# zhuye98/ICL

Hardware: AMD Instinct MI355X
Metric: 3D volumes/sec/node (fwd+bwd, 96^3 patch) (higher is better)
Workload: dtype f32; 1 GPU; 3D U-Net ICL BraTS-shape synthetic 96x96x96, num_classes=2, batch=2 per GPU (1 labeled + 1 unlabeled), full ICL step incl. SGD; global_batch=2, parallelism=dp1, launch=hipGraph replay

## Files before the change

icl_amd/_lib.py:

```python
from __future__ import annotations

import ctypes
import os
from ctypes import c_char_p, c_double, c_float, c_int, c_int64, c_void_p

import torch

_HERE = os.path.dirname(os.path.abspath(__file__))
DEFAULT_LIB = os.path.join(_HERE, "libicl_hip.so")

_lib = None
_lib_path = None
_host_pointers_ok = False

P, I, L, F = c_void_p, c_int, c_int64, c_float
D = c_double

_SIGNATURES = {
    "icl_abi_version": (c_int, []),
    "icl_last_error": (c_char_p, []),
    "icl_last_kernel_name": (c_char_p, []),
    "icl_conv3d_packed_elems": (c_int64, [I, I, I, I]),
    "icl_conv3d_pack_weights": (c_int, [P, P, I, I, I, I, P]),
    "icl_conv3d_pack_weights_both": (c_int, [P, P, P, I, I, I, P]),
    "icl_conv3d_pack_weights_multi": (c_int, [P, P, P, P, P, P, I, P]),
    "icl_conv3d_fwd_ws_bytes": (c_int64, [I, I, I, I, I, I, I]),
    "icl_conv3d_fwd": (c_int, [P, P, P, P, P, I, I, I, I, I, I, I, L, L, P]),
    "icl_scalar_combine": (c_int, [P, P, I, I, P, P]),
    "icl_conv3d_split_ws_bytes": (c_int64, [I, I]),
    "icl_conv3d_split_weights_multi": (c_int, [P, P, P, P, I, P]),
    "icl_conv3d_fwd_presplit": (c_int, [P, P, P, P, I, I, I, I, I, I, L, L, P]),
    "icl_conv3d_fwd_presplit_ws_bytes": (c_int64, [I, I, I, I, I, I]),
    "icl_conv3d_fwd_presplit_ws": (c_int, [P, P, P, P, P, I, I, I, I, I, I, L, L, P]),
    "icl_conv3d_fwd_stats_slots": (c_int, [I, I, I, I, I, I]),
    "icl_conv3d_fwd_presplit_stats": (c_int, [P, P, P, P, P, I, I, I, I, I, I, L, L, P]),
    "icl_norm_fwd_given_stats": (c_int, [P, P, P, P, P, P, P, P, P, I, I, L, I, I, F, F, P, I, P]),
    "icl_conv3d_wgrad_ws_bytes": (c_int64, [I, I, I, I]),
    "icl_conv3d_wgrad": (c_int, [P, P, P, P, P, I, I, I, I, I, I, I, L, L, P]),
    "icl_conv3d_wgrad_slabs": (c_int, [P, P, P, I, I, I, I, I, I, I, L, L, P, P]),
    "icl_conv3d_wgrad_reduce_multi": (c_int, [P, P, P, P, P, P, I, P]),
    "icl_norm_ws_bytes": (c_int64, [I, I, L]),
    "icl_norm_fwd": (c_int, [P, P, P, P, P, P, P, P, I, I, L, I, I, I, F, F, P, P]),
    "icl_norm_bwd": (c_int, [P, P, P, P, P, P, P, P, P, I, I, L, I, I, I, P, P]),
    "icl_norm_res_fwd": (c_int, [P, P, P, P, P, P, P, P, P, I, I, L, I, I, I, F, F, P, P]),
    "icl_norm_res_bwd": (c_int, [P, P, P, P, P, P, P, P, P, P, P, I, I, L, I, I, I, P, P]),
    "icl_rstd_from_var": (c_int, [P, P, I, F, P]),
    "icl_norm_finalize_stats": (c_int, [P, I, I, I, F, P, P, P, P]),
    "icl_norm_apply": (c_int, [P, P, P, I, I, L, P]),
    "icl_maxpool2_fwd_norm": (c_int, [P, P, P, P, L, I, I, I, I, P]),
    "icl_upsample2x_concat_norm": (c_int, [P, P, P, P, P, I, I, I, I, I, I, P]),
    "icl_conv1x1_dropout_norm": (c_int, [P, P, P, P, P, I, I, I, L, I, I, ctypes.c_uint32, F, P, P]),
    "icl_conv1x1_wgrad_dropout_norm": (c_int, [P, P, P, P, P, P, I, I, I, L, L, ctypes.c_uint32, F, P, P]),
    "icl_maxpool2_fwd": (c_int, [P, P, P, L, I, I, I, I, P]),
    "icl_maxpool2_bwd": (c_int, [P, P, P, L, I, I, I, I, P]),
    "icl_maxpool2_bwd_add": (c_int, [P, P, P, P, I, I, I, I, I, I, L, P]),
    "icl_trilinear_fwd": (c_int, [P, P, I, I, I, I, I, I, I, I, L, I, P]),
    "icl_trilinear_bwd_ws_bytes": (c_int64, [I, I, I, I, I, I, I, I]),
    "icl_trilinear_bwd": (c_int, [P, P, P, I, I, I, I, I, I, I, I, L, I, P]),
    "icl_copy_rows": (c_int, [P, P, L, L, L, L, P]),
    "icl_concat2": (c_int, [P, L, P, L, P, P]),
    "icl_dwconv3_fwd": (c_int, [P, P, P, I, I, I, I, I, I, P]),
    "icl_dwconv3_wgrad_ws_bytes": (c_int64, [I, I, I, I, I]),
    "icl_dwconv3_wgrad": (c_int, [P, P, P, P, I, I, I, I, I, P]),
    "icl_conv1x1_small": (c_int, [P, P, P, P, I, I, I, L, I, I, P]),
    "icl_conv1x1_dropout": (c_int, [P, P, P, P, I, I, I, L, I, I, I, ctypes.c_uint32, F, P, P]),
    "icl_conv1x1_wgrad_dropout": (c_int, [P, P, P, P, P, I, I, I, L, L, ctypes.c_uint32, F, P, P]),
    "icl_dropout": (c_int, [P, P, L, ctypes.c_uint32, F, P, P]),
    "icl_drop_path": (c_int, [P, P, L, L, ctypes.c_uint32, F, P, P]),
    "icl_drop_path_add": (c_int, [P, P, P, L, L, ctypes.c_uint32, F, P, P]),
    "icl_loss_fwd": (c_int, [P, P, P, P, P, P, I, I, L, I, I, P]),
    "icl_window_attn_bias_elems": (c_int64, [I, I]),
    "icl_depth_to_space2": (c_int, [P, P, I, I, I, I, I, L, P]),
    "icl_space_to_depth2": (c_int, [P, P, I, I, I, I, I, L, P]),
    "icl_colsum_multi": (c_int, [P, P, P, P, I, P]),
    "icl_gather_rows": (c_int, [P, P, P, L, L, L, I, P]),
    "icl_gather_rows_sum2": (c_int, [P, P, P, L, L, L, I, P]),
    "icl_im2col3": (c_int, [P, P, I, I, I, I, I, P]),
    "icl_im2col3_planes": (c_int, [P, P, I, I, I, I, I, P]),
    "icl_conv3d_cin1_fwd": (c_int, [P, P, P, P, I, I, I, I, I, L, L, P]),
    "icl_conv3d_cin1_wgrad_ws_bytes": (c_int64, [I, I, I]),
    "icl_conv3d_cin1_wgrad": (c_int, [P, P, P, P, I, I, I, I, I, L, L, P]),
    "icl_col2im3": (c_int, [P, P, I, I, I, I, I, P]),
    "icl_linear_ws_bytes": (c_int64, [L, I, I, I]),
    "icl_linear_fwd": (c_int, [P, P, P, P, P, L, I, I, I, P]),
    "icl_linear_dgrad": (c_int, [P, P, P, P, L, I, I, P]),
    "icl_linear_bwd_small": (c_int, [P, P, P, P, P, P, L, I, I, P]),
    "icl_linear_wgrad_small": (c_int, [P, P, P, P, L, I, I, P]),
    "icl_linear_dgrad_sgd": (c_int, [P, P, P, P, P, P, L, I, I, F, F, F, I, P, P]),
    "icl_gemm_ws_bytes": (c_int64, [L, I, I, I]),
    "icl_gemm": (c_int, [P, P, P, P, P, L, I, I, L, L, L, I, I, I, I, L, L, L, P]),
    "icl_linear_wgrad_ws_bytes": (c_int64, [L, I, I]),
    "icl_linear_wgrad": (c_int, [P, P, P, P, P, L, I, I, P]),
    "icl_conv1x1_wgrad_ws_bytes": (c_int64, [I, L, I, I]),
    "icl_conv1x1_wgrad": (c_int, [P, P, P, P, P, I, I, I, L, L, L, P]),
    "icl_relpos_bias_fwd": (c_int, [P, P, P, I, I, I, P]),
    "icl_window_attn_fwd": (c_int, [P, P, P, P, P, I, I, I, I, I, F, P]),
    "icl_window_attn_bwd": (c_int, [P, P, P, P, P, P, P, P, I, I, I, I, I, F, P]),
    "icl_window_attn_bwd_chunks": (c_int, [I, I, I, I, I]),
    "icl_window_attn_fwd_drop": (c_int, [P, P, P, P, P, I, I, I, I, I, F, ctypes.c_uint32, F, P, P]),
    "icl_window_attn_keep_probe": (c_int, [P, c_int64, I, ctypes.c_uint32, F, P, P]),
    "icl_window_attn_bwd_drop": (c_int, [P, P, P, P, P, P, P, P, I, I, I, I, I, F, ctypes.c_uint32, F, P, P]),
    "icl_relpos_bias_bwd_sum": (c_int, [P, I, P, P, P, L, I, I, P]),
    "icl_layernorm_fwd": (c_int, [P, P, P, P, P, P, L, I, F, P]),
    "icl_layernorm_bwd_ws_bytes": (c_int64, [L, I]),
    "icl_layernorm_bwd": (c_int, [P, P, P, P, P, P, P, P, P, L, I, P]),
    "icl_gelu_fwd": (c_int, [P, P, L, P]),
    "icl_gelu_bwd": (c_int, [P, P, P, L, P]),
    "icl_attn_fwd": (c_int, [P, P, P, P, P, I, I, I, I, I, F, P]),
    "icl_attn_bwd": (c_int, [P, P, P, P, P, P, P, P, P, I, I, I, I, I, F, P]),
    "icl_attn_bwd_ws_bytes": (c_int64, [I, I, I, I, I]),
    "icl_attn_bwd_ws": (c_int, [P, P, P, P, P, P, P, P, P, P, I, I, I, I, I, F, P]),
    "icl_crop_rotflip": (c_int, [P, P, P, I, P, P, I, I, I, P]),
    "icl_volume_feed": (c_int, [P, P, P, P, I, P, P, I, I, I, P]),
    "icl_rank_tile": (c_int, []),
    "icl_rank_index_build": (c_int, [P, P, I, I, I, F, P, P, P]),
    "icl_rank_select": (c_int, [P, P, P, P, P, F, I, P, P]),
    "icl_volume_feed_origins": (c_int, [P, P, P, P, I, P, P, P, I, I, I, P]),
    "icl_prefix_box": (c_int, [P, I, I, I, P, I, P, P, P]),
    "icl_prefix_resample": (c_int, [P, P, P, P, P, I, P, P, P]),
    "icl_prefix_restore": (c_int, [P, I, P, P, P, P]),
    "icl_slice_augment": (c_int, [P, P, P, P, I, P, P, I, I, P]),
    "icl_slice_resize": (c_int, [P, P, L, I, I, I, I, I, P]),
    "icl_sgd_step": (c_int, [P, P, P, L, F, F, F, I, P, P]),
    "icl_sgd_step_factored": (c_int, [P, P, P, P, I, I, I, F, F, F, I, P, P]),
    "icl_sgd_step_factored_narrow": (c_int, [P, P, P, P, I, I, I, F, F, F, I, P, I, P]),
    "icl_sgd_factored_split_ws_bytes": (c_int64, [I, I, I]),
    "icl_sgd_step_factored_split": (c_int, [P, P, P, P, P, I, I, I, F, F, F, I, P, P]),
    "icl_sgd_step_multi": (c_int, [P, P, P, P, I, F, F, F, I, P, P]),
    "icl_loss_bwd": (c_int, [P, P, P, P, P, P, P, P, I, I, L, I, I, P]),
    "icl_loss_fwd_multi": (c_int, [P, I, P]),
    "icl_loss_bwd_multi": (c_int, [P, I, P]),
    "icl_qchain_stage": (c_int, [P, P]),
    "icl_qchain_wgrad": (c_int, [P, P, P, P, P, P, P, P, I, P]),
    "icl_seg_metrics_ws_bytes": (c_int64, [I, I, I, I]),
    "icl_seg_metrics": (c_int, [P, I, P, I, I, I, I, I, I, P, P, P]),
    "icl_seg_surface_ws_bytes": (c_int64, [I, I, I, I]),
    "icl_seg_surface_metrics": (c_int, [P, I, P, I, I, I, I, I, D, D, D, D, P, P, P, P]),
    "icl_seg_components_ws_bytes": (c_int64, [I, I, I, I]),
    "icl_seg_components": (c_int, [P, I, I, I, I, I, I, P, P, P, P]),
    "icl_seg_filter_components": (c_int, [P, I, I, I, I, I, I, I, c_int64, P, P, P, P]),
    "icl_window_gather": (c_int, [P, P, P, I, I, I, I, I, I, I, I, I, I, I, I, I, I, P]),
    "icl_window_accumulate": (c_int, [P, P, P, P, P, I, I, I, I, I, I, I, I, I, P]),
    "icl_window_finalize": (c_int, [P, P, P, P, I, I, I, I, I, I, I, I, I, I, P]),
    "icl_window_gather_flipped": (c_int, [P, P, P, P, I, I, I, I, I, I, I, I, I, I, I, I, I, I, P]),
    "icl_window_accumulate_flipped": (c_int, [P, P, P, P, P, P, I, I, I, I, I, I, I, I, I, P]),
    "icl_last_live_fwd_kernel_name": (c_char_p, []),
    "icl_last_wgrad_grid": (None, [P, P]),
    "icl_conv3d_fwd_live_ok": (c_int, [I, I, I, I, I, I, I]),
    "icl_conv3d_fwd_presplit_live": (c_int, [P, P, P, P, I, I, I, I, I, I, I, L, L, P]),
    "icl_conv3d_fwd_presplit_ws_live": (c_int, [P, P, P, P, P, I, I, I, I, I, I, I, L, L, P]),
    "icl_conv3d_fwd_live": (c_int, [P, P, P, P, P, I, I, I, I, I, I, I, I, L, L, P]),
    "icl_conv3d_wgrad_ws_bytes_live": (c_int64, [I, I, I, I, I]),
    "icl_conv3d_wgrad_live": (c_int, [P, P, P, P, P, I, I, I, I, I, I, I, I, L, L, P]),
    "icl_conv3d_wgrad_slabs_live": (c_int, [P, P, P, I, I, I, I, I, I, I, I, L, L, P, P]),
    "icl_norm_bwd_live": (c_int, [P, P, P, P, P, P, P, P, P, I, I, I, L, I, I, I, P, P]),
    "icl_maxpool2_bwd_add_live": (c_int, [P, P, P, P, I, I, I, I, I, I, I, L, P]),
    "icl_trilinear_bwd_live": (c_int, [P, P, P, I, I, I, I, I, I, I, I, I, L, I, P]),
    "icl_conv1x1_small_live": (c_int, [P, P, P, P, I, I, I, I, L, I, I, P]),
    "icl_conv1x1_dropout_live": (c_int, [P, P, P, P, I, I, I, I, L, I, I, I, ctypes.c_uint32, F, P, P]),
    "icl_conv1x1_wgrad_live": (c_int, [P, P, P, P, P, I, I, I, I, L, L, L, P]),
    "icl_conv1x1_wgrad_dropout_live": (c_int, [P, P, P, P, P, I, I, I, I, L, L, ctypes.c_uint32, F, P, P]),
    "icl_conv1x1_wgrad_dropout_norm_live": (c_int, [P, P, P, P, P, P, I, I, I, I, L, L, ctypes.c_uint32, F, P, P]),
}

EXPORTS = tuple(_SIGNATURES)


def _load(path: str):
    if not os.path.exists(path):
        raise RuntimeError(
            f"icl_amd: HIP library {path} not found — build it with `python -m icl_amd.build` "
            "(hipcc --offload-arch=gfx950). There is no CPU fallback.")
    lib = ctypes.CDLL(path)
    for name, (res, args) in _SIGNATURES.items():
        fn = getattr(lib, name)
        fn.restype = res
        fn.argtypes = args
    return lib


def lib():
    global _lib, _lib_path
    if _lib is None:
        _lib_path = os.environ.get("ICL_HIP_LIB", DEFAULT_LIB)
        _lib = _load(_lib_path)
    return _lib


def lib_path():
    lib()
    return _lib_path


def host_pointers_ok() -> bool:
    return _host_pointers_ok


def _use_library_for_tests(path: str | None, host_pointers: bool = True):
    global _lib, _lib_path, _host_pointers_ok
    if path is None:
        _lib, _lib_path, _host_pointers_ok = None, None, False
        return
    _lib, _lib_path, _host_pointers_ok = _load(path), path, host_pointers


def check(rc: int, what: str = ""):
    if rc != 0:
        msg = lib().icl_last_error()
        raise RuntimeError(f"icl_hip {what} failed ({rc}): {msg.decode() if msg else ''}")
```

icl_amd/csrc/icl_abi.inc:

```

#include "kernels/common.h"
#include "kernels/norm.h"
#include "kernels/pool_resize.h"
#include "kernels/reduce.h"
#include "kernels/conv_mfma.h"
#include "kernels/conv_mfma_static.h"
#include "kernels/conv_mfma_flat.h"
#include "kernels/conv_bf16x3.h"
#include "kernels/conv_bf16x3_ws.h"
#include "kernels/conv_wgrad_tr.h"
#include "kernels/conv_wgrad_zs.h"
#include "kernels/conv_cin1.h"
#include "kernels/misc.h"
#include "kernels/loss.h"
#include "kernels/optim.h"
#include "kernels/winattn.h"
#include "kernels/linear_wgrad.h"
#include "kernels/token.h"
#include "kernels/gemm.h"
#include "kernels/datafeed.h"
#include "kernels/rankindex.h"
#include "kernels/prefix.h"
#include "kernels/qchain.h"
#include "kernels/metrics.h"
// ... 1181 lines not shown
  hipStream_t st = (hipStream_t)stream;
  const int R = n * c;
  const int nch = (int)((s + icl::kNormChunk - 1) / icl::kNormChunk);
  float* part = (float*)ws;
  if (mode == 0 && nch == 1) {
    part = nullptr;
  } else {
    ICL_LAUNCH(icl::norm_act_bwd_partial_kernel, dim3(nch, R), dim3(icl::kNormThreads), 0, st, gy, x, mean, rstd, gamma, beta, part,
               (long)s, c, nch, mode, act, res);
    if (int rc = check_launch("norm_bwd_partial")) return rc;
  }
  const float inv_count = 1.0f / (float)((mode ? (int64_t)n : 1) * s);
  ICL_LAUNCH(icl::norm_act_bwd_apply_kernel, dim3(nch, R), dim3(icl::kNormThreads), 0, st, gy, x, mean, rstd, gamma, beta,
             (const float*)part, gx, (long)s, c, mode, act, inv_count, use_batch_stats, res, gres, R, nch, dgamma, dbeta);
  return check_launch("norm_bwd_apply");
}

int icl_rstd_from_var(const float* var, float* rstd, int c, float eps, void* stream) {
  if (!var || !rstd || c < 1) return fail(-1, "rstd_from_var: bad argument");
  ICL_LAUNCH(icl::rstd_from_var_kernel, dim3((c + 63) / 64), dim3(64), 0, (hipStream_t)stream, var, rstd, c, eps);
  return check_launch("rstd_from_var");
}

namespace {
int maxpool2_fwd_run(const float* x, const float* ss, float* y, uint8_t* idx, int64_t nc, int dout, int hout, int wout, int pool_depth,
                     hipStream_t st, const char* what) {
  const long total = nc * dout * hout * wout;
  const char* e_x2 = getenv("ICL_MAXPOOL_BWD_X2");
  if ((wout & 1) == 0 && aligned16(x) && ((uintptr_t)y & 7) == 0 && (e_x2 ? atoi(e_x2) : 1)) {
    ICL_LAUNCH(icl::maxpool2_fwd_x2_kernel, dim3(grid_for(total / 2, 256)), dim3(256), 0, st, x, y, idx, (long)nc, dout, hout, wout, pool_depth, ss);
  } else {
    ICL_LAUNCH(icl::maxpool2_fwd_kernel, dim3(grid_for(total, 256)), dim3(256), 0, st, x, y, idx, (long)nc, dout, hout, wout, pool_depth, ss);
  }
  return check_launch(what);
}
}

int icl_maxpool2_fwd(const float* x, float* y, uint8_t* idx, int64_t nc, int dout, int hout, int wout, int pool_depth, void* stream) {
  if (!x || !y || !idx || nc < 1 || dout < 1 || hout < 1 || wout < 1 || (pool_depth != 1 && pool_depth != 2)) return fail(-1, "maxpool2_fwd: bad argument");
  return maxpool2_fwd_run(x, nullptr, y, idx, nc, dout, hout, wout, pool_depth, (hipStream_t)stream, "maxpool2_fwd");
}

int icl_norm_finalize_stats(const float* part, int n, int c, int nslots, float eps, float* mean, float* rstd, float* ss, void* stream) {
  if (!part || !mean || !rstd || !ss || n < 1 || c < 1 || nslots < 1) return fail(-1, "norm_finalize_stats: bad argument");
  ICL_LAUNCH(icl::norm_finalize_stats_kernel, dim3(n * c), dim3(64), 0, (hipStream_t)stream, part, n * c, c, nslots, eps, mean, rstd, ss);
  return check_launch("norm_finalize_stats");
}

int icl_norm_apply(const float* x, const float* ss, float* y, int n, int c, int64_t s, void* stream) {
  if (!x || !ss || !y || n < 1 || c < 1 || s < 4 || (s & 3) || !aligned16(x) || !aligned16(y)) return fail(-1, "norm_apply: bad argument (s %% 4 == 0)");
  ICL_LAUNCH(icl::copy_rows_norm_kernel, dim3(grid_for((long)n * c * (s >> 2), 256, 1 << 16)), dim3(256), 0, (hipStream_t)stream, x, y, n, c, (long)s,
             (long)c * s, ss);
  return check_launch("norm_apply");
}

int icl_maxpool2_fwd_norm(const float* x, const float* ss, float* y, uint8_t* idx, int64_t nc, int dout, int hout, int wout, int pool_depth,
                          void* stream) {
  if (!x || !ss || !y || !idx || nc < 1 || dout < 1 || hout < 1 || wout < 1 || (pool_depth != 1 && pool_depth != 2))
    return fail(-1, "maxpool2_fwd_norm: bad argument");
  return maxpool2_fwd_run(x, ss, y, idx, nc, dout, hout, wout, pool_depth, (hipStream_t)stream, "maxpool2_fwd_norm");
}

int icl_upsample2x_concat_norm(const float* skip, const float* skip_ss, const float* deep, const float* deep_ss, float* out, int n, int cs,
                               int cd, int d, int h, int w, void* stream) {
  if (!skip || !deep || !out || n < 1 || cs < 1 || cd < 1 || d < 2 || h < 2 || w < 4 || (d & 1) || (h & 1) || (w & 3))
    return fail(-1, "upsample2x_concat_norm: bad argument (even depth / height, width a multiple of 4)");
  if (!aligned16(skip) || !aligned16(deep) || !aligned16(out)) return fail(-1, "upsample2x_concat_norm: 16-byte alignment");
  hipStream_t st = (hipStream_t)stream;
  const long s = (long)d * h * w, obs = (long)(cs + cd) * s;
  if (skip_ss) {
    ICL_LAUNCH(icl::copy_rows_norm_kernel, dim3(grid_for((long)n * cs * (s >> 2), 256, 1 << 16)), dim3(256), 0, st, skip, out, n, cs, s, obs, skip_ss);
  } else {
    ICL_LAUNCH(icl::copy_rows_kernel, dim3(grid_for((long)n * cs * s, 256)), dim3(256), 0, st, skip, out, (long)n, (long)cs * s, (long)cs * s, obs);
  }
  if (int rc = check_launch("upsample2x_concat_norm: skip")) return rc;
  const long total = (long)n * cd * s;
  const int di = d / 2, hi = h / 2, wi = w / 2;
  if (wi % 4 == 0)
    ICL_LAUNCH(icl::upsample2x_fwd_x4_kernel, dim3(grid_for(total / 32, 256, 1 << 16)), dim3(256), 0, st, deep, out + (long)cs * s, n, cd, di, hi, wi, obs,
               deep_ss);
  else
    ICL_LAUNCH(icl::upsample2x_fwd_kernel, dim3(grid_for(total / 16, 256, 1 << 16)), dim3(256), 0, st, deep, out + (long)cs * s, n, cd, di, hi, wi, obs,
               deep_ss);
  return check_launch("upsample2x_concat_norm: deep");
}

int icl_maxpool2_bwd(const float* gy, const uint8_t* idx, float* gx, int64_t nc, int dout, int hout, int wout, int pool_depth, void* stream) {
  if (!gy || !gx || !idx || nc < 1 || dout < 1 || hout < 1 || wout < 1 || (pool_depth != 1 && pool_depth != 2)) return fail(-1, "maxpool2_bwd: bad argument");
  const long total = nc * dout * hout * wout;
  ICL_LAUNCH(icl::maxpool2_bwd_kernel, dim3(grid_for(total, 256)), dim3(256), 0, (hipStream_t)stream, gy, idx, gx, (long)nc, dout, hout, wout,
             pool_depth);
  return check_launch("maxpool2_bwd");
}

int icl_maxpool2_bwd_add(const float* gy, const uint8_t* idx, const float* add, float* gx, int n, int c, int dout, int hout, int wout,
                         int pool_depth, int64_t add_bstride, void* stream) {
  return icl_maxpool2_bwd_add_live(gy, idx, add, gx, n, n, c, dout, hout, wout, pool_depth, add_bstride, stream);
}

int icl_maxpool2_bwd_add_live(const float* gy, const uint8_t* idx, const float* add, float* gx, int n, int skip_live, int c, int dout, int hout,
                              int wout, int pool_depth, int64_t add_bstride, void* stream) {
  if (!gy || !gx || !idx || !add || n < 1 || c < 1 || dout < 1 || hout < 1 || wout < 1 || (pool_depth != 1 && pool_depth != 2) || (add_bstride & 1) ||
      ((uintptr_t)add & 7) || skip_live < 1 || skip_live > n)
    return fail(-1, "maxpool2_bwd_add: bad argument");
  const long ncskip = (long)skip_live * c;
  const long total = (long)n * c * dout * hout * wout;
  const char* e_x2 = getenv("ICL_MAXPOOL_BWD_X2");
  if ((wout & 1) == 0 && aligned16(add) && aligned16(gx) && ((uintptr_t)gy & 7) == 0 && (add_bstride & 3) == 0 && (e_x2 ? atoi(e_x2) : 1)) {
    ICL_LAUNCH(icl::maxpool2_bwd_add_x2_kernel, dim3(grid_for(total / 2, 256)), dim3(256), 0, (hipStream_t)stream, gy, idx, add, gx, (long)n * c, c,
               dout, hout, wout, pool_depth, (long)add_bstride, ncskip);
    return check_launch("maxpool2_bwd_add_x2");
  }
  ICL_LAUNCH(icl::maxpool2_bwd_add_kernel, dim3(grid_for(total, 256)), dim3(256), 0, (hipStream_t)stream, gy, idx, add, gx, (long)n * c, c, dout,
             hout, wout, pool_depth, (long)add_bstride, ncskip);
  return check_launch("maxpool2_bwd_add");
}

namespace {
inline float resize_scale(int in, int out, int align) {
  if (align) return out > 1 ? (float)(in - 1) / (float)(out - 1) : 0.f;
  return (float)in / (float)out;
}
}

int icl_trilinear_fwd(const float* x, float* y, int n, int c, int di, int hi, int wi, int dout, int hout, int wout,
                      int64_t y_bstride, int align_corners, void* stream) {
  if (!x || !y || n < 1 || c < 1 || di < 1 || hi < 1 || wi < 1 || dout < 1 || hout < 1 || wout < 1) return fail(-1, "trilinear_fwd: bad argument");
  const long total = (long)n * c * dout * hout * wout;
  const float rz = resize_scale(di, dout, align_corners), ry = resize_scale(hi, hout, align_corners), rx = resize_scale(wi, wout, align_corners);
  if (!align_corners && dout == 2 * di && hout == 2 * hi && wout == 2 * wi && wi % 2 == 0 && y_bstride % 4 == 0 && aligned16(y) &&
      total / 16 < (1L << 31)) {
    constexpr int x4 = 1;
    if (x4 && wi % 4 == 0 && aligned16(x))
      ICL_LAUNCH(icl::upsample2x_fwd_x4_kernel, dim3(grid_for(total / 32, 256, 1 << 16)), dim3(256), 0, (hipStream_t)stream, x, y, n, c, di, hi,
                 wi, (long)y_bstride, (const float*)nullptr);
    else
      ICL_LAUNCH(icl::upsample2x_fwd_kernel, dim3(grid_for(total / 16, 256, 1 << 16)), dim3(256), 0, (hipStream_t)stream, x, y, n, c, di, hi, wi,
                 (long)y_bstride, (const float*)nullptr);
  } else if (wout % 4 == 0 && y_bstride % 4 == 0 && aligned16(y) && total / 4 < (1L << 31)) {
    ICL_LAUNCH(icl::trilinear_fwd_quad_kernel, dim3(grid_for(total / 4, 256, 1 << 16)), dim3(256), 0, (hipStream_t)stream, x, y, n, c, di, hi,
               wi, dout, hout, wout, rz, ry, rx, (long)y_bstride, align_corners);
  } else {
    ICL_LAUNCH(icl::trilinear_fwd_kernel, dim3(grid_for(total, 256)), dim3(256), 0, (hipStream_t)stream, x, y, n, c, di, hi, wi, dout, hout,
               wout, rz, ry, rx, (long)y_bstride, align_corners);
  }
  return check_launch("trilinear_fwd");
}

int64_t icl_trilinear_bwd_ws_bytes(int n, int c, int di, int hi, int wi, int dout, int hout, int wout) {
  (void)di;
  return ((int64_t)n * c * dout * hout * wi + (int64_t)n * c * dout * hi * wi) * 4;
}

int icl_trilinear_bwd(const float* gy, float* gx, void* ws, int n, int c, int di, int hi, int wi, int dout, int hout, int wout,
                      int64_t gy_bstride, int align_corners, void* stream) {
  if (!gy || !gx || !ws || n < 1 || c < 1 || di < 1 || hi < 1 || wi < 1 || dout < 1 || hout < 1 || wout < 1) return fail(-1, "trilinear_bwd: bad argument");
  hipStream_t st = (hipStream_t)stream;
  const int al = align_corners;
  const float rz = resize_scale(di, dout, al), ry = resize_scale(hi, hout, al), rx = resize_scale(wi, wout, al);
  float* t1 = (float*)ws;
  float* t2 = t1 + (size_t)n * c * dout * hout * wi;
  int rc;
  if (!al && dout == 2 * di && hout == 2 * hi && wout == 2 * wi && wi % 4 == 0 && gy_bstride % 4 == 0 && aligned16(gy) && aligned16(gx) &&
      (long)n * c * di * hi * wi / 4 < (1L << 31)) {
    ICL_LAUNCH(icl::upsample2x_bwd_kernel, dim3(grid_for((long)n * c * ((di + icl::kUpSeg - 1) / icl::kUpSeg) * hi * wi / 4, 256, 1 << 16)),
               dim3(256), 0, st, gy, gx, n, c, di, hi,
               wi, (long)gy_bstride);
    return check_launch("upsample2x_bwd");
  }
  auto axis = [&](const float* src, float* dst, long rows, int li, int lo, long inner, float rs, long sbs, const char* what) -> int {
    const long total = (long)n * rows * li * inner;
    const bool small = total / 4 < (1L << 31) && rows < (1L << 31);
    if (small && inner % 4 == 0 && sbs % 4 == 0 && aligned16(src) && aligned16(dst)) {
      ICL_LAUNCH(icl::resize_bwd_axis_t4_kernel, dim3(grid_for(total / 4, 256, 1 << 16)), dim3(256), 0, st, src, dst, n, (unsigned)rows, li, lo,
                 (unsigned)(inner / 4), rs, sbs, al);
    } else if (inner == 1 && lo >= 4 * li && lo % 4 == 0 && lo <= 1024 && sbs % 4 == 0 && aligned16(src) && rows * li >= 4096) {
      const long nrows = (long)n * rows;
      ICL_LAUNCH(icl::resize_bwd_axis_x_lds_kernel, dim3((unsigned)cdivl(nrows, icl::kRbxRows)), dim3(256),
                 (size_t)icl::kRbxRows * (lo + 4) * 4, st, src, dst, n, rows, li, lo, rs, sbs, al);
    } else if (small && inner == 1 && li % 4 == 0 && aligned16(dst)) {
      ICL_LAUNCH(icl::resize_bwd_axis_i4_kernel, dim3(grid_for(total / 4, 256, 1 << 16)), dim3(256), 0, st, src, dst, n, (unsigned)rows, li, lo,
                 rs, sbs, al);
    } else {
      ICL_LAUNCH(icl::resize_bwd_axis_kernel, dim3(grid_for(total, 256)), dim3(256), 0, st, src, dst, n, rows, li, lo, inner, rs, sbs, al);
    }
    return check_launch(what);
  };
  if ((rc = axis(gy, t1, (long)c * dout * hout, wi, wout, 1L, rx, (long)gy_bstride, "resize_bwd_x"))) return rc;
  if ((rc = axis(t1, t2, (long)c * dout, hi, hout, (long)wi, ry, (long)c * dout * hout * wi, "resize_bwd_y"))) return rc;
  if ((rc = axis(t2, gx, (long)c, di, dout, (long)hi * wi, rz, (long)c * dout * hi * wi, "resize_bwd_z"))) return rc;
  return 0;
}

int icl_copy_rows(const float* src, float* dst, int64_t rows, int64_t row_elems, int64_t src_stride, int64_t dst_stride,
                  void* stream) {
  if (!src || !dst || rows < 1 || row_elems < 1) return fail(-1, "copy_rows: bad argument");
  ICL_LAUNCH(icl::copy_rows_kernel, dim3(grid_for(rows * row_elems, 256)), dim3(256), 0, (hipStream_t)stream, src, dst, (long)rows,
             (long)row_elems, (long)src_stride, (long)dst_stride);
  return check_launch("copy_rows");
}

int icl_concat2(const float* a, int64_t na, const float* b, int64_t nb, float* out, void* stream) {
  if (!out || na < 0 || nb < 0 || na + nb < 4 || (na & 3) || (nb & 3) || (!a && !b)) return fail(-1, "concat2: bad argument (float counts are multiples of 4)");
  if ((a && !aligned16(a)) || (b && !aligned16(b)) || !aligned16(out)) return fail(-1, "concat2: 16-byte alignment");
  ICL_LAUNCH(icl::concat2_kernel, dim3(grid_for((na + nb) >> 2, 256)), dim3(256), 0, (hipStream_t)stream, a, (long)na, b, (long)nb, out);
  return check_launch("concat2");
}

int icl_depth_to_space2(const float* yt, float* out, int n, int d, int h, int w, int cout, int64_t out_bstride, void* stream) {
  if (!yt || !out || n < 1 || d < 1 || h < 1 || w < 1 || cout < 1) return fail(-1, "depth_to_space2: bad argument");
  const size_t lds = (size_t)w * (cout * 8 + 2) * 4;
  if (lds > (size_t)kMaxDynLdsBig) return fail(-1, "depth_to_space2: token row does not fit LDS (w * cout too large)");
  if (lds > (size_t)kMaxDynLds) ICL_SET_MAX_DYN_LDS(icl::depth_to_space2_kernel, kMaxDynLdsBig);
  ICL_LAUNCH(icl::depth_to_space2_kernel, dim3(h, d, n), dim3(256), lds, (hipStream_t)stream, yt, out, d, h, w, cout, (long)out_bstride);
  return check_launch("depth_to_space2");
}

int icl_space_to_depth2(const float* g, float* gt, int n, int d, int h, int w, int cout, int64_t g_bstride, void* stream) {
  if (!g || !gt || n < 1 || d < 1 || h < 1 || w < 1 || cout < 1) return fail(-1, "space_to_depth2: bad argument");
  const size_t lds = (size_t)w * (cout * 8 + 2) * 4;
  if (lds > (size_t)kMaxDynLdsBig) return fail(-1, "space_to_depth2: token row does not fit LDS (w * cout too large)");
  if (lds > (size_t)kMaxDynLds) ICL_SET_MAX_DYN_LDS(icl::space_to_depth2_kernel, kMaxDynLdsBig);
  ICL_LAUNCH(icl::space_to_depth2_kernel, dim3(h, d, n), dim3(256), lds, (hipStream_t)stream, g, gt, d, h, w, cout, (long)g_bstride);
  return check_launch("space_to_depth2");
}

int icl_dwconv3_fwd(const float* x, const float* w, float* y, int n, int c, int d, int h, int wd, int flip, void* stream) {
  if (!x || !w || !y || n < 1 || c < 1 || d < 1 || h < 1 || wd < 1) return fail(-1, "dwconv3_fwd: bad argument");
  const long total = (long)n * c * d * h * wd;
  ICL_LAUNCH(icl::dwconv3_fwd_kernel, dim3(grid_for(total, 256)), dim3(256), 0, (hipStream_t)stream, x, w, y, (long)n * c, c, d, h, wd, flip);
  return check_launch("dwconv3_fwd");
}

static long dwconv3_wgrad_chunks(long total) {
  long chunks = cdivl(total, 1024);
  return chunks > 512 ? 512 : chunks;
}

int64_t icl_dwconv3_wgrad_ws_bytes(int n, int c, int d, int h, int wd) {
  return dwconv3_wgrad_chunks((long)n * d * h * wd) * c * 27 * 4;
}

int icl_dwconv3_wgrad(const float* x, const float* gy, float* gw, void* ws, int n, int c, int d, int h, int wd, void* stream) {
  if (!x || !gy || !gw || !ws || n < 1 || c < 1 || d < 1 || h < 1 || wd < 1) return fail(-1, "dwconv3_wgrad: bad argument");
  hipStream_t s = (hipStream_t)stream;
  const long total = (long)n * d * h * wd;
  const long chunks = dwconv3_wgrad_chunks(total);
  const long chunk = cdivl(total, chunks);
  ICL_LAUNCH(icl::dwconv3_wgrad_kernel, dim3((unsigned)chunks, c), dim3(256), 0, s, x, gy, (float*)ws, n, c, d, h, wd, chunk);
  if (int rc = check_launch("dwconv3_wgrad")) return rc;
  ICL_LAUNCH(icl::dwconv3_wgrad_reduce_kernel, dim3((unsigned)cdivl((long)c * 27, 16)), dim3(256), 0, s, (const float*)ws, gw, c * 27, (int)chunks);
  return check_launch("dwconv3_wgrad_reduce");
}

namespace {
icl::DropSpec drop_spec(int mode, uint32_t seed, float p, const uint32_t* seed_dev) {
  icl::DropSpec d{};
  d.mode = mode;
  d.seed = (unsigned)seed;
  d.thresh = (unsigned)((double)p * 4294967296.0);
  d.scale = 1.0f / (1.0f - p);
  d.seed_dev = (const unsigned*)seed_dev;
  return d;
}

int conv1x1_small_run(const float* x, const float* w, const float* bias, float* y, int n, int cin, int cout, int64_t s, int w_ostride,
                      int w_istride, const icl::DropSpec& dr, hipStream_t st, int n_plan = 0) {
  if ((long)(n_plan > n ? n_plan : n) * s >= 65536) {
    const long quads = (long)n * (s >> 2);
    const int ob = cout <= 1 ? 1 : cout <= 2 ? 2 : cout <= 4 ? 4 : cout <= 8 ? 8 : 16;
    const dim3 grid(grid_for(quads, 256, 1 << 16), (cout + ob - 1) / ob);
    switch (ob) {
      case 1: ICL_LAUNCH(icl::conv1x1_stream_kernel<1>, grid, dim3(256), 0, st, x, w, bias, y, n, cin, cout, (long)s, w_ostride, w_istride, dr); break;
      case 2: ICL_LAUNCH(icl::conv1x1_stream_kernel<2>, grid, dim3(256), 0, st, x, w, bias, y, n, cin, cout, (long)s, w_ostride, w_istride, dr); break;
      case 4: ICL_LAUNCH(icl::conv1x1_stream_kernel<4>, grid, dim3(256), 0, st, x, w, bias, y, n, cin, cout, (long)s, w_ostride, w_istride, dr); break;
      case 8: ICL_LAUNCH(icl::conv1x1_stream_kernel<8>, grid, dim3(256), 0, st, x, w, bias, y, n, cin, cout, (long)s, w_ostride, w_istride, dr); break;
      default: ICL_LAUNCH(icl::conv1x1_stream_kernel<16>, grid, dim3(256), 0, st, x, w, bias, y, n, cin, cout, (long)s, w_ostride, w_istride, dr); break;
    }
    return check_launch("conv1x1_stream");
  }
  if (dr.mode) return 1;
  const long total = (long)n * cout * (s >> 2);
  ICL_LAUNCH(icl::conv1x1_small_kernel, dim3(grid_for(total, 256)), dim3(256), 0, st, x, w, bias, y, n, cin, cout, (long)s,
             w_ostride, w_istride);
  return check_launch("conv1x1_small");
}
}

int icl_conv1x1_small(const float* x, const float* w, const float* bias, float* y, int n, int cin, int cout, int64_t s, int w_ostride,
                      int w_istride, void* stream) {
  if (!x || !w || !y || n < 1 || cin < 1 || cout < 1 || s < 4 || (s & 3)) return fail(-1, "conv1x1_small: bad argument (s %% 4 == 0)");
  return conv1x1_small_run(x, w, bias, y, n, cin, cout, s, w_ostride, w_istride, icl::DropSpec{}, (hipStream_t)stream);
}

int icl_conv1x1_dropout(const float* x, const float* w, const float* bias, float* y, int n, int cin, int cout, int64_t s, int w_ostride,
                        int w_istride, int mask_mode, uint32_t seed, float p, const uint32_t* seed_dev, void* stream) {
  if (!x || !w || !y || n < 1 || cin < 1 || cout < 1 || s < 4 || (s & 3) || (mask_mode != 1 && mask_mode != 2) || !(p >= 0.f && p < 1.f))
    return fail(-1, "conv1x1_dropout: bad argument");
  return conv1x1_small_run(x, w, bias, y, n, cin, cout, s, w_ostride, w_istride, drop_spec(mask_mode, seed, p, seed_dev), (hipStream_t)stream);
}

int icl_conv1x1_dropout_norm(const float* x, const float* ss, const float* w, const float* bias, float* y, int n, int cin, int cout, int64_t s,
                             int w_ostride, int w_istride, uint32_t seed, float p, const uint32_t* seed_dev, void* stream) {
  if (!x || !ss || !w || !y || n < 1 || cin < 1 || cout < 1 || s < 4 || (s & 3) || !(p >= 0.f && p < 1.f) || (long)n * s < 65536)
    return fail(-1, "conv1x1_dropout_norm: bad argument (big volumes only: n * s >= 65536)");
  icl::DropSpec dr = p > 0.f ? drop_spec(1, seed, p, seed_dev) : icl::DropSpec{};
  dr.ss = ss;
  return conv1x1_small_run(x, w, bias, y, n, cin, cout, s, w_ostride, w_istride, dr, (hipStream_t)stream);
}

int icl_scalar_combine(const void* const* in, const float* w, int n_in, int n_out, float* out, void* stream) {
  if (!in || !w || !out || n_in < 1 || n_out < 1 || n_in > icl::kScalarCombine || n_out > icl::kScalarCombine)
    return fail(-1, "scalar_combine: bad argument (<= %d scalars in and out)", icl::kScalarCombine);
  icl::ScalarCombine s{};
  s.n_in = n_in; s.n_out = n_out;
  for (int i = 0; i < n_in; ++i) {
    if (!in[i]) return fail(-1, "scalar_combine: null input %d", i);
    s.in[i] = (const float*)in[i];
  }
  for (int j = 0; j < n_out; ++j)
    for (int i = 0; i < n_in; ++i) s.w[j][i] = w[j * n_in + i];
  ICL_LAUNCH(icl::scalar_combine_kernel, dim3(1), dim3(64), 0, (hipStream_t)stream, s, out);
  return check_launch("scalar_combine");
}

int icl_colsum_multi(const void* const* g, void* const* out, const int32_t* rows, const int32_t* cols, int count, void* stream) {
  if (!g || !out || !rows || !cols || count < 1) return fail(-1, "colsum_multi: bad argument");
  for (int base = 0; base < count; base += icl::kColsumMulti) {
    icl::ColsumMulti m{};
    const int k = count - base < icl::kColsumMulti ? count - base : icl::kColsumMulti;
    int cmax = 1;
    for (int i = 0; i < k; ++i) {
      const int j = base + i;
      if (!g[j] || !out[j] || rows[j] < 1 || cols[j] < 1) return fail(-1, "colsum_multi: bad tensor %d", j);
      m.g[i] = (const float*)g[j]; m.out[i] = (float*)out[j]; m.rows[i] = rows[j]; m.cols[i] = cols[j];
      if (cols[j] > cmax) cmax = cols[j];
    }
    ICL_LAUNCH(icl::colsum_multi_kernel, dim3(grid_for(cmax, 16, 128), k), dim3(256), 0, (hipStream_t)stream, m);
    const int rc = check_launch("colsum_multi");
    if (rc) return rc;
  }
  return 0;
}

int icl_gather_rows(const float* src, const int32_t* idx, float* out, int64_t b, int64_t s, int64_t m, int c, void* stream) {
  if (!src || !idx || !out || b < 1 || s < 1 || m < 1 || c < 4 || (c & 3)) return fail(-1, "gather_rows: bad argument (c %% 4 == 0)");
  ICL_LAUNCH(icl::gather_rows_kernel, dim3(grid_for(b * m * (c / 4), 256)), dim3(256), 0, (hipStream_t)stream, src, (const int*)idx, out,
             (long)b, (long)s, (long)m, c / 4);
  return check_launch("gather_rows");
}

int icl_gather_rows_sum2(const float* src, const int32_t* idx2, float* out, int64_t b, int64_t s, int64_t m, int c, void* stream) {
  if (!src || !idx2 || !out || b < 1 || s < 1 || m < 1 || c < 4 || (c & 3)) return fail(-1, "gather_rows_sum2: bad argument (c %% 4 == 0)");
  ICL_LAUNCH(icl::gather_rows_sum2_kernel, dim3(grid_for(b * m * (c / 4), 256)), dim3(256), 0, (hipStream_t)stream, src, (const int*)idx2, out,
             (long)b, (long)s, (long)m, c / 4);
  return check_launch("gather_rows_sum2");
}

int icl_im2col3(const float* x, float* cols, int n, int c, int d, int h, int w, void* stream) {
  if (!x || !cols || n < 1 || c < 1 || d < 1 || h < 1 || w < 1) return fail(-1, "im2col3: bad argument");
  ICL_LAUNCH(icl::im2col3_kernel, dim3(grid_for((long)n * c * 27 * d * h * w, 256)), dim3(256), 0, (hipStream_t)stream, x, cols, n, c, d, h, w);
  return check_launch("im2col3");
}

int icl_im2col3_planes(const float* x, float* planes, int n, int c, int d, int h, int w, void* stream) {
  if (!x || !planes || n < 1 || c < 1 || d < 1 || h < 1 || w < 4 || (w & 3)) return fail(-1, "im2col3_planes: bad argument (w %% 4 == 0)");
  ICL_LAUNCH(icl::im2col3_planes_kernel, dim3(grid_for((long)n * c * 27 * d * h * (w / 4), 256, 1 << 16)), dim3(256), 0, (hipStream_t)stream, x,
             planes, n, c, d, h, w);
  return check_launch("im2col3_planes");
}

int icl_col2im3(const float* g, float* dx, int n, int c, int d, int h, int w, void* stream) {
  if (!g || !dx || n < 1 || c < 1 || d < 1 || h < 1 || w < 1) return fail(-1, "col2im3: bad argument");
  ICL_LAUNCH(icl::col2im3_kernel, dim3(grid_for((long)n * c * d * h * w, 256)), dim3(256), 0, (hipStream_t)stream, g, dx, n, c, d, h, w);
  return check_launch("col2im3");
}

int icl_drop_path_add(const float* x, const float* res, float* y, int64_t n, int64_t group, uint32_t seed, float p,
                      const uint32_t* seed_dev, void* stream) {
  if (!x || !y || n < 1 || group < 1 || !(p >= 0.f && p < 1.f)) return fail(-1, "dropout: bad argument");
  const unsigned thresh = (unsigned)((double)p * 4294967296.0);
  ICL_LAUNCH(icl::dropout_kernel, dim3(grid_for(n, 256)), dim3(256), 0, (hipStream_t)stream, x, res, y, (long)n, (unsigned)seed, thresh,
             1.0f / (1.0f - p), (const unsigned*)seed_dev, (long)group);
  return check_launch("dropout");
}

int icl_drop_path(const float* x, float* y, int64_t n, int64_t group, uint32_t seed, float p, const uint32_t* seed_dev, void* stream) {
  return icl_drop_path_add(x, nullptr, y, n, group, seed, p, seed_dev, stream);
}

int icl_dropout(const float* x, float* y, int64_t n, uint32_t seed, float p, const uint32_t* seed_dev, void* stream) {
  return icl_drop_path(x, y, n, 1, seed, p, seed_dev, stream);
}

static bool loss_force_generic() {
  const char* e = getenv("ICL_LOSS_GENERIC");
  return e && atoi(e) == 1;
}
static int loss_class_group(int nc) { return nc <= 4 ? 0 : (nc <= 16 ? 1 : 2); }

int icl_loss_fwd(const float* a, const float* b, const int64_t* labels, const float* weight, float* stats, float* out,
                 int batch, int nc, int64_t s, int mode, int a_is_prob, void* stream) {
  if (nc < 1 || nc > icl::kLossMaxNc) return fail(-1, "loss_fwd: %d classes (1 .. %d)", nc, icl::kLossMaxNc);
  if (!a || !stats || !out || batch < 1 || s < 1 || mode < 0 || mode > 3) return fail(-1, "loss_fwd: bad argument");
  if ((mode <= 1) != (labels != nullptr) || (mode >= 2) != (b != nullptr)) return fail(-1, "loss_fwd: target does not match mode");
  hipStream_t st = (hipStream_t)stream;
  const long total = (long)batch * s;
  const int nblk = grid_for(total, 256, ICL_LOSS_MAX_BLOCKS);
  float* part = stats + (3 * nc + 1);
  const dim3 grid(nblk), block(256);
  const long long* lab = (const long long*)labels;
  if (nc > 16 || loss_force_generic()) {
    ICL_LAUNCH(icl::loss_stats_generic_kernel, grid, block, 0, st, a, b, lab, part, batch, nc, (long)s, a_is_prob);
  } else if (nc <= 4) {
    ICL_LAUNCH((icl::loss_stats_kernel<4>), grid, block, 0, st, a, b, lab, part, batch, nc, (long)s, a_is_prob);
  } else {
    ICL_LAUNCH((icl::loss_stats_kernel<16>), grid, block, 0, st, a, b, lab, part, batch, nc, (long)s, a_is_prob);
  }
  int rc = check_launch("loss_stats");
  if (rc) return rc;
  ICL_LAUNCH(icl::loss_finalize_kernel, dim3(1), dim3(256), 0, st, (const float*)part, nblk, stats, weight, out, nc, 1.0f / (float)total,
             1.0f / ((float)total * (float)nc), mode);
  return check_launch("loss_finalize");
}

static int loss_multi_fill(const IclLossJob* jobs, int count, bool bwd, icl::LossMulti& m, int& most, int& group) {
  if (!jobs || count < 1 || count > icl::kLossMulti) return fail(-1, "loss_multi: 1 .. %d jobs", icl::kLossMulti);
  most = 1;
  group = loss_class_group(jobs[0].nc);
  for (int j = 0; j < count; ++j) {
    const IclLossJob& q = jobs[j];
    if (q.nc < 1 || q.nc > icl::kLossMaxNc) return fail(-1, "loss_multi: job %d has %d classes (1 .. %d)", j, q.nc, icl::kLossMaxNc);
    if (!q.a || !q.stats || q.batch < 1 || q.s < 1 || q.mode < 0 || q.mode > 3 || loss_class_group(q.nc) != group)
      return fail(-1, "loss_multi: bad job %d (all jobs of a call need nc <= 4, or all 5 .. 16, or all 17 .. %d)", j, icl::kLossMaxNc);
    if ((q.mode <= 1) != (q.labels != nullptr) || (q.mode >= 2) != (q.b != nullptr)) return fail(-1, "loss_multi: target of job %d does not match its mode", j);
    if (bwd ? !q.ga : !q.out) return fail(-1, "loss_multi: job %d has no output", j);
    const long total = (long)q.batch * q.s;
    m.a[j] = q.a; m.b[j] = q.b; m.lab[j] = (const long long*)q.labels; m.weight[j] = q.weight; m.stats[j] = q.stats; m.out[j] = q.out;
    m.g0[j] = q.gout0; m.g1[j] = q.gout1; m.ga[j] = q.ga;
    m.S[j] = (long)q.s; m.B[j] = q.batch; m.nc[j] = q.nc; m.mode[j] = q.mode; m.aip[j] = q.a_is_prob;
    m.nblk[j] = bwd ? grid_for(total, 256, 4096) : grid_for(total, 256, ICL_LOSS_MAX_BLOCKS);
    if (m.nblk[j] > most) most = m.nblk[j];
  }
  if (loss_force_generic()) group = 2;
  return 0;
}

int icl_loss_fwd_multi(const IclLossJob* jobs, int count, void* stream) {
  icl::LossMulti m{};
  int most = 1, group = 0;
  int rc = loss_multi_fill(jobs, count, false, m, most, group);
  if (rc) return rc;
  hipStream_t st = (hipStream_t)stream;
  if (group == 2) {
    ICL_LAUNCH(icl::loss_stats_generic_multi_kernel, dim3(most, count), dim3(256), 0, st, m);
  } else if (group == 0) {
    ICL_LAUNCH((icl::loss_stats_multi_kernel<4>), dim3(most, count), dim3(256), 0, st, m);
  } else {
    ICL_LAUNCH((icl::loss_stats_multi_kernel<16>), dim3(most, count), dim3(256), 0, st, m);
  }
  rc = check_launch("loss_stats_multi");
  if (rc) return rc;
  ICL_LAUNCH(icl::loss_finalize_multi_kernel, dim3(count), dim3(256), 0, st, m);
  return check_launch("loss_finalize_multi");
}

int icl_loss_bwd_multi(const IclLossJob* jobs, int count, void* stream) {
  icl::LossMulti m{};
  int most = 1, group = 0;
  int rc = loss_multi_fill(jobs, count, true, m, most, group);
  if (rc) return rc;
  if (group == 2) {
    ICL_LAUNCH(icl::loss_grad_generic_multi_kernel, dim3(most, count), dim3(256), 0, (hipStream_t)stream, m);
  } else if (group == 0) {
    ICL_LAUNCH((icl::loss_grad_multi_kernel<4>), dim3(most, count), dim3(256), 0, (hipStream_t)stream, m);
  } else {
    ICL_LAUNCH((icl::loss_grad_multi_kernel<16>), dim3(most, count), dim3(256), 0, (hipStream_t)stream, m);
  }
  return check_launch("loss_grad_multi");
}

int icl_loss_bwd(const float* a, const float* b, const int64_t* labels, const float* weight, const float* stats,
                 const float* gout0, const float* gout1, float* ga, int batch, int nc, int64_t s, int mode, int a_is_prob,
                 void* stream) {
  if (nc < 1 || nc > icl::kLossMaxNc) return fail(-1, "loss_bwd: %d classes (1 .. %d)", nc, icl::kLossMaxNc);
  if (!a || !stats || !ga || batch < 1 || s < 1) return fail(-1, "loss_bwd: bad argument");
  hipStream_t st = (hipStream_t)stream;
  const long total = (long)batch * s;
  const float inv_vox = 1.0f / (float)total, inv_elems = 1.0f / ((float)total * (float)nc);
  const dim3 grid(grid_for(total, 256, 4096)), block(256);
  const long long* lab = (const long long*)labels;
  if (nc > 16 || loss_force_generic()) {
    ICL_LAUNCH(icl::loss_grad_generic_kernel, grid, block, 0, st, a, b, lab, stats, weight, gout0, gout1, ga, batch, nc, (long)s, mode, inv_vox,
               inv_elems, a_is_prob);
  } else if (nc <= 4) {
    ICL_LAUNCH((icl::loss_grad_kernel<4>), grid, block, 0, st, a, b, lab, stats, weight, gout0, gout1, ga, batch, nc, (long)s, mode, inv_vox,
               inv_elems, a_is_prob);
  } else {
    ICL_LAUNCH((icl::loss_grad_kernel<16>), grid, block, 0, st, a, b, lab, stats, weight, gout0, gout1, ga, batch, nc, (long)s, mode, inv_vox,
               inv_elems, a_is_prob);
  }
  return check_launch("loss_grad");
}

int icl_layernorm_fwd(const float* x, const float* gamma, const float* beta, float* y, float* mean, float* rstd, int64_t rows,
                      int c, float eps, void* stream) {
  if (!x || (!gamma != !beta) || !y || !mean || !rstd || rows < 1 || c < 1) return fail(-1, "layernorm_fwd: bad argument");
  constexpr int longrow = 1;
  if (c >= 1024 && c <= 256 * 64 && longrow) {
    if (c <= 256 * 16) ICL_LAUNCH((icl::layernorm_fwd_longrow_kernel<16>), dim3((unsigned)rows), dim3(256), 0, (hipStream_t)stream, x, gamma, beta, y, mean, rstd, c, eps);
    else if (c <= 256 * 32) ICL_LAUNCH((icl::layernorm_fwd_longrow_kernel<32>), dim3((unsigned)rows), dim3(256), 0, (hipStream_t)stream, x, gamma, beta, y, mean, rstd, c, eps);
    else ICL_LAUNCH((icl::layernorm_fwd_longrow_kernel<64>), dim3((unsigned)rows), dim3(256), 0, (hipStream_t)stream, x, gamma, beta, y, mean, rstd, c, eps);
  } else if (c >= 1024) {
    ICL_LAUNCH((icl::layernorm_fwd_kernel<true>), dim3((unsigned)rows), dim3(256), 0, (hipStream_t)stream, x, gamma, beta, y, mean, rstd,
               (long)rows, c, eps);
  } else {
    ICL_LAUNCH((icl::layernorm_fwd_kernel<false>), dim3((unsigned)cdivl(rows, 4)), dim3(256), 0, (hipStream_t)stream, x, gamma, beta, y,
               mean, rstd, (long)rows, c, eps);
  }
  return check_launch("layernorm_fwd");
}

namespace {
long ln_rows_per_chunk(long rows) {
  long rpb = cdivl(rows, 512);
  return rpb < 32 ? 32 : rpb;
}
}

int64_t icl_layernorm_bwd_ws_bytes(int64_t rows, int c) {
  if (rows < 1 || c < 1) return 0;
  return (int64_t)2 * cdivl(rows, ln_rows_per_chunk(rows)) * c * 4;
}

int icl_layernorm_bwd(const float* gy, const float* x, const float* gamma, const float* mean, const float* rstd, float* gx,
                      float* dgamma, float* dbeta, void* ws, int64_t rows, int c, void* stream) {
  if (!gy || !x || !mean || !rstd || !gx || ((dgamma || ws) && !gamma) || rows < 1 || c < 1) return fail(-1, "layernorm_bwd: bad argument");
  hipStream_t st = (hipStream_t)stream;
  if (!dgamma != !dbeta) return fail(-1, "layernorm_bwd: dgamma and dbeta go together");
  if (dgamma && !ws) return fail(-1, "layernorm_bwd: parameter gradients need the workspace of icl_layernorm_bwd_ws_bytes");
  const long rpb = ln_rows_per_chunk(rows);
  const int chunks = (int)cdivl(rows, rpb);
  float* part_g = (float*)ws;
  float* part_b = part_g ? part_g + (long)chunks * c : nullptr;
  constexpr int fuse_on = 1;
  if (c < 1024 && ws && fuse_on) {
    const dim3 grid((unsigned)chunks);
#define ICL_LN_BW(CPL, RU) \
  ICL_LAUNCH((icl::layernorm_bwd_wgrad_kernel<CPL, RU>), grid, dim3(256), 0, st, gy, x, gamma, mean, rstd, gx, part_g, part_b, (long)rows, c, rpb)
    if (c <= 64) ICL_LN_BW(1, 4);
    else if (c <= 128) ICL_LN_BW(2, 4);
    else if (c <= 256) ICL_LN_BW(4, 2);
    else if (c <= 512) ICL_LN_BW(8, 1);
    else ICL_LN_BW(16, 1);
#undef ICL_LN_BW
    int rc = check_launch("layernorm_bwd_wgrad");
    if (rc || !dgamma) return rc;
    const void* g[2] = {part_g, part_b};
    void* out[2] = {dgamma, dbeta};
    const int32_t rr[2] = {chunks, chunks}, cc[2] = {c, c};
    return icl_colsum_multi(g, out, rr, cc, 2, stream);
  }
  constexpr int longrow = 1;
  if (c >= 1024 && c <= 256 * 64 && longrow) {
    if (c <= 256 * 16) ICL_LAUNCH((icl::layernorm_bwd_longrow_kernel<16>), dim3((unsigned)rows), dim3(256), 0, st, gy, x, gamma, mean, rstd, gx, c);
    else if (c <= 256 * 32) ICL_LAUNCH((icl::layernorm_bwd_longrow_kernel<32>), dim3((unsigned)rows), dim3(256), 0, st, gy, x, gamma, mean, rstd, gx, c);
    else ICL_LAUNCH((icl::layernorm_bwd_longrow_kernel<64>), dim3((unsigned)rows), dim3(256), 0, st, gy, x, gamma, mean, rstd, gx, c);
  } else if (c >= 1024) {
    ICL_LAUNCH((icl::layernorm_bwd_kernel<true>), dim3((unsigned)rows), dim3(256), 0, st, gy, x, gamma, mean, rstd, gx, (long)rows, c);
  } else {
    ICL_LAUNCH((icl::layernorm_bwd_kernel<false>), dim3((unsigned)cdivl(rows, 4)), dim3(256), 0, st, gy, x, gamma, mean, rstd, gx,
               (long)rows, c);
  }
  int rc = check_launch("layernorm_bwd");
  if (rc || !ws) return rc;
  int cols = 256;
  while (cols > c && cols > 16) cols >>= 1;
  if (cols < c && cols < 256) cols <<= 1;
  ICL_LAUNCH(icl::layernorm_wgrad_kernel, dim3((c + cols - 1) / cols, (unsigned)chunks), dim3(256), 0, st, gy, x, mean, rstd, part_g, part_b,
             (long)rows, c, rpb, cols);
  rc = check_launch("layernorm_wgrad");
  if (rc || !dgamma) return rc;
  const void* g[2] = {part_g, part_b};
  void* out[2] = {dgamma, dbeta};
  const int32_t rr[2] = {chunks, chunks}, cc[2] = {c, c};
  return icl_colsum_multi(g, out, rr, cc, 2, stream);
}

int icl_gelu_fwd(const float* x, float* y, int64_t n, void* stream) {
  if (!x || !y || n < 1) return fail(-1, "gelu_fwd: bad argument");
  ICL_LAUNCH(icl::gelu_fwd_kernel, dim3(grid_for(n, 256)), dim3(256), 0, (hipStream_t)stream, x, y, (long)n);
  return check_launch("gelu_fwd");
}

int icl_gelu_bwd(const float* gy, const float* x, float* gx, int64_t n, void* stream) {
  if (!gy || !x || !gx || n < 1) return fail(-1, "gelu_bwd: bad argument");
  ICL_LAUNCH(icl::gelu_bwd_kernel, dim3(grid_for(n, 256)), dim3(256), 0, (hipStream_t)stream, gy, x, gx, (long)n);
  return check_launch("gelu_bwd");
}

static bool attn_class_tiles(int nc) {
  const char* e = getenv("ICL_ATTN_TILED");
  return nc > icl::kAttnMaxNc || (e && atoi(e) == 1);
}

int icl_attn_fwd(const float* q, const float* kv, float* logits, float* out, float* stats, int b, int h, int nc, int n, int d,
                 float scale, void* stream) {
  if (nc < 1 || nc > icl::kAttnMaxClasses) return fail(-1, "attn_fwd: %d classes (1 .. %d)", nc, icl::kAttnMaxClasses);
  if (!q || !kv || !logits || !out || !stats || b < 1 || h < 1 || n < 1 || (d != 8 && d != 16))
    return fail(-1, "attn_fwd: bad argument (head dim 8 or 16)");
  hipStream_t st = (hipStream_t)stream;
  const dim3 g1((n + 255) / 256, b * h), g2(b * h * nc);
  const bool tiled = attn_class_tiles(nc);
  if (d == 16) {
    if (tiled) ICL_LAUNCH((icl::attn_logits_kernel<16, true>), g1, dim3(256), 0, st, q, kv, logits, b, h, nc, n, scale);
    else ICL_LAUNCH((icl::attn_logits_kernel<16, false>), g1, dim3(256), 0, st, q, kv, logits, b, h, nc, n, scale);
    ICL_LAUNCH((icl::attn_softmax_pv_kernel<16, 256>), g2, dim3(256), 0, st, (const float*)logits, kv, out, stats, b, h, nc, n);
  } else {
    if (tiled) ICL_LAUNCH((icl::attn_logits_kernel<8, true>), g1, dim3(256), 0, st, q, kv, logits, b, h, nc, n, scale);
    else ICL_LAUNCH((icl::attn_logits_kernel<8, false>), g1, dim3(256), 0, st, q, kv, logits, b, h, nc, n, scale);
    ICL_LAUNCH((icl::attn_softmax_pv_kernel<8, 256>), g2, dim3(256), 0, st, (const float*)logits, kv, out, stats, b, h, nc, n);
  }
  return check_launch("attn_fwd");
}

int64_t icl_attn_bwd_ws_bytes(int b, int h, int nc, int n, int d) {
  if (b < 1 || h < 1 || nc < 1 || n < 1 || d < 1) return 0;
  return (int64_t)((n + 255) / 256) * b * h * nc * d * 4;
}

int icl_attn_bwd(const float* q, const float* kv, const float* logits, const float* stats, const float* out, const float* gout,
                 const float* glog, float* gq, float* gkv, int b, int h, int nc, int n, int d, float scale, void* stream) {
// ... 1390 lines not shown
```

icl_amd/csrc/kernels/loss.h:

```cpp
#pragma once

namespace icl {

constexpr float kDiceEps = 1e-5f;

template <int NCMAX>
__device__ __forceinline__ void softmax_vec(float* v, int nc, float& lse) {
  float m = v[0];
#pragma unroll
  for (int c = 1; c < NCMAX; ++c)
    if (c < nc) m = fmaxf(m, v[c]);
  float s = 0.f;
#pragma unroll
  for (int c = 0; c < NCMAX; ++c)
    if (c < nc) { v[c] = expf(v[c] - m); s += v[c]; }
  const float inv = 1.0f / s;
#pragma unroll
  for (int c = 0; c < NCMAX; ++c)
    if (c < nc) v[c] *= inv;
  lse = m + logf(s);
}

template <int NCMAX>
__device__ __forceinline__ void loss_stats_body(const float* __restrict__ a, const float* __restrict__ b,
                                                const long long* __restrict__ labels, float* __restrict__ part,
                                                int B, int nc, long S, int a_is_prob, int bx, int nbx) {
  float s0[NCMAX], s1[NCMAX], s2[NCMAX];
  float sx = 0.f;
#pragma unroll
  for (int c = 0; c < NCMAX; ++c) { s0[c] = 0.f; s1[c] = 0.f; s2[c] = 0.f; }
  const long total = (long)B * S;
  for (long e = (long)bx * blockDim.x + threadIdx.x; e < total; e += (long)nbx * blockDim.x) {
    const long bi = e / S, s = e - bi * S;
    const float* ap = a + bi * nc * S + s;
    float p[NCMAX];
#pragma unroll
    for (int c = 0; c < NCMAX; ++c) p[c] = c < nc ? ap[(long)c * S] : 0.f;
    float lse = 0.f;
    if (labels) {
      const int y = (int)labels[e];
      float ay = 0.f;
#pragma unroll
      for (int c = 0; c < NCMAX; ++c)
        if (c == y) ay = p[c];
      if (!a_is_prob) { softmax_vec<NCMAX>(p, nc, lse); sx += lse - ay; }
#pragma unroll
      for (int c = 0; c < NCMAX; ++c) {
        if (c < nc) {
          const float t = (c == y) ? 1.f : 0.f;
          s0[c] += p[c] * t;
          s1[c] += p[c] * p[c];
          s2[c] += t;
        }
      }
    } else {
      const float* bp = b + bi * nc * S + s;
      float q[NCMAX];
#pragma unroll
      for (int c = 0; c < NCMAX; ++c) q[c] = c < nc ? bp[(long)c * S] : 0.f;
      float l2;
      if (!a_is_prob) softmax_vec<NCMAX>(p, nc, lse);
      softmax_vec<NCMAX>(q, nc, l2);
#pragma unroll
      for (int c = 0; c < NCMAX; ++c) {
        if (c < nc) {
          s0[c] += p[c] * q[c];
          s1[c] += p[c];
          s2[c] += q[c];
          const float d = p[c] - q[c];
          sx += d * d;
        }
      }
    }
  }
  __shared__ float red[4][3 * NCMAX + 1];
  const int lane = threadIdx.x & 63, wid = threadIdx.x >> 6;
#pragma unroll
  for (int c = 0; c < NCMAX; ++c) {
    const float r0 = wave_sum(s0[c]), r1 = wave_sum(s1[c]), r2 = wave_sum(s2[c]);
    if (lane == 0) { red[wid][c] = r0; red[wid][NCMAX + c] = r1; red[wid][2 * NCMAX + c] = r2; }
  }
  {
    const float rx = wave_sum(sx);
    if (lane == 0) red[wid][3 * NCMAX] = rx;
  }
  __syncthreads();
  const int t = threadIdx.x;
  if (t < 3 * NCMAX + 1) {
    const int grp = t / NCMAX, c = t - grp * NCMAX;
    if (t == 3 * NCMAX || c < nc) {
      const float v = red[0][t] + red[1][t] + red[2][t] + red[3][t];
      const int slot = (t == 3 * NCMAX) ? 3 * nc : grp * nc + c;
      part[(long)bx * (3 * nc + 1) + slot] = v;
    }
  }
}
template <int NCMAX>
__global__ __launch_bounds__(256) void loss_stats_kernel(const float* __restrict__ a, const float* __restrict__ b,
                                                         const long long* __restrict__ labels, float* __restrict__ part,
                                                         int B, int nc, long S, int a_is_prob) {
  loss_stats_body<NCMAX>(a, b, labels, part, B, nc, S, a_is_prob, blockIdx.x, gridDim.x);
}

__device__ __forceinline__ void loss_finalize_body(const float* __restrict__ part, int nblk, float* __restrict__ stats,
                                                   const float* __restrict__ weight, float* __restrict__ out, int nc,
                                                   float inv_vox, float inv_elems, int mode) {
  const int nslot = 3 * nc + 1;
  __shared__ float red[256];
  int S = 8;
  while (S < nslot && S < 64) S <<= 1;
  const int G = 256 / S;
  const int sl = threadIdx.x % S, grp = threadIdx.x / S;
  for (int s0 = 0; s0 < nslot; s0 += S) {
    const int slot = s0 + sl;
    float v = 0.f;
    if (slot < nslot) {
#pragma unroll 4
      for (int b = grp; b < nblk; b += G) v += part[(long)b * nslot + slot];
    }
    __syncthreads();
    red[grp * S + sl] = v;
    __syncthreads();
    if (grp == 0 && slot < nslot) {
      float t = red[sl];
      for (int k = 1; k < G; ++k) t += red[k * S + sl];
      stats[slot] = t;
    }
  }
  __syncthreads();
  if (threadIdx.x != 0) return;
  float dice = 0.f;
  for (int c = 0; c < nc; ++c) {
    const float num = 2.f * stats[c] + kDiceEps;
    const float den = stats[nc + c] + stats[2 * nc + c] + kDiceEps;
    dice += (weight ? weight[c] : 1.f) * (1.f - num / den);
  }
  out[1] = (mode == 3) ? 0.f : dice / (float)nc;
  out[0] = (mode == 1) ? stats[3 * nc] * inv_vox : (mode == 3 ? stats[3 * nc] * inv_elems : 0.f);
}
__global__ __launch_bounds__(256) void loss_finalize_kernel(const float* __restrict__ part, int nblk, float* __restrict__ stats,
                                                            const float* __restrict__ weight, float* __restrict__ out, int nc,
                                                            float inv_vox, float inv_elems, int mode) {
  loss_finalize_body(part, nblk, stats, weight, out, nc, inv_vox, inv_elems, mode);
}

template <int NCMAX>
__device__ __forceinline__ void loss_grad_body(const float* __restrict__ a, const float* __restrict__ b,
                                               const long long* __restrict__ labels, const float* __restrict__ stats,
                                               const float* __restrict__ weight, const float* __restrict__ gout0,
                                               const float* __restrict__ gout1, float* __restrict__ ga, int B, int nc,
                                               long S, int mode, float inv_vox, float inv_elems, int a_is_prob, int bx, int nbx) {
  float al[NCMAX], be[NCMAX], gm[NCMAX];
  const float g0 = gout0 ? gout0[0] : 0.f, g1 = gout1 ? gout1[0] : 0.f;
#pragma unroll
  for (int c = 0; c < NCMAX; ++c) {
    al[c] = be[c] = gm[c] = 0.f;
    if (c < nc) {
      const float num = 2.f * stats[c] + kDiceEps;
      const float den = stats[nc + c] + stats[2 * nc + c] + kDiceEps;
      const float w = (weight ? weight[c] : 1.f) * g1 / (float)nc;
      if (mode == 0 || mode == 1) { al[c] = -2.f * w / den; be[c] = 2.f * w * num / (den * den); }
      else if (mode == 2) { al[c] = -2.f * w / den; gm[c] = w * num / (den * den); }
      else { al[c] = -2.f * g0 * inv_elems; be[c] = 2.f * g0 * inv_elems; }
    }
  }
  const float kappa = (mode == 1) ? g0 * inv_vox : 0.f;
  const long total = (long)B * S;
  for (long e = (long)bx * blockDim.x + threadIdx.x; e < total; e += (long)nbx * blockDim.x) {
    const long bi = e / S, s = e - bi * S;
    const float* ap = a + bi * nc * S + s;
    float* gp = ga + bi * nc * S + s;
    float p[NCMAX], T[NCMAX];
#pragma unroll
    for (int c = 0; c < NCMAX; ++c) p[c] = c < nc ? ap[(long)c * S] : 0.f;
    float lse;
    if (!a_is_prob) softmax_vec<NCMAX>(p, nc, lse);
    if (labels) {
      const int y = (int)labels[e];
#pragma unroll
      for (int c = 0; c < NCMAX; ++c) T[c] = (c == y) ? 1.f : 0.f;
    } else {
      const float* bp = b + bi * nc * S + s;
#pragma unroll
      for (int c = 0; c < NCMAX; ++c) T[c] = c < nc ? bp[(long)c * S] : 0.f;
      softmax_vec<NCMAX>(T, nc, lse);
    }
    float d[NCMAX];
    float dot = 0.f;
#pragma unroll
    for (int c = 0; c < NCMAX; ++c) {
      d[c] = c < nc ? al[c] * T[c] + be[c] * p[c] + gm[c] : 0.f;
      dot += d[c] * p[c];
    }
#pragma unroll
    for (int c = 0; c < NCMAX; ++c) {
      if (c < nc) {
        float gv = a_is_prob ? d[c] : p[c] * (d[c] - dot);
        if (labels) gv += kappa * (p[c] - T[c]);
        gp[(long)c * S] = gv;
      }
    }
  }
}
template <int NCMAX>
__global__ __launch_bounds__(256) void loss_grad_kernel(const float* __restrict__ a, const float* __restrict__ b,
                                                        const long long* __restrict__ labels, const float* __restrict__ stats,
                                                        const float* __restrict__ weight, const float* __restrict__ gout0,
                                                        const float* __restrict__ gout1, float* __restrict__ ga, int B, int nc,
                                                        long S, int mode, float inv_vox, float inv_elems, int a_is_prob) {
  loss_grad_body<NCMAX>(a, b, labels, stats, weight, gout0, gout1, ga, B, nc, S, mode, inv_vox, inv_elems, a_is_prob, blockIdx.x, gridDim.x);
}

constexpr int kLossMaxNc = 256;

__device__ __forceinline__ void softmax_norm_strided(const float* __restrict__ p, int nc, long S, float& m, float& sum) {
  m = p[0];
  sum = 1.f;
  for (int c = 1; c < nc; ++c) {
    const float v = p[(long)c * S];
    const float e = expf(-fabsf(v - m));
    sum = v > m ? sum * e + 1.f : sum + e;
    m = fmaxf(m, v);
  }
}

__device__ __forceinline__ void loss_stats_generic_body(const float* __restrict__ a, const float* __restrict__ b,
                                                        const long long* __restrict__ labels, float* __restrict__ part,
                                                        int B, int nc, long S, int a_is_prob, int bx, int nbx) {
  __shared__ float acc[4][3 * kLossMaxNc + 1];
  const int lane = threadIdx.x & 63, wid = threadIdx.x >> 6;
  const int nslot = 3 * nc + 1;
  float* my = acc[wid];
  for (int i = lane; i < nslot; i += 64) my[i] = 0.f;
  __syncthreads();
  float sx = 0.f;
  const long total = (long)B * S;
  for (long e0 = (long)bx * 256; e0 < total; e0 += (long)nbx * 256) {
    const long e = e0 + threadIdx.x;
    const bool live = e < total;
    const long ec = live ? e : total - 1;
    const long bi = ec / S, s = ec - bi * S;
    const float* ap = a + bi * nc * S + s;
    float m = 0.f, inv = 1.f;
    if (!a_is_prob) {
      float sum;
      softmax_norm_strided(ap, nc, S, m, sum);
      inv = 1.0f / sum;
      if (labels) {
        const int y = (int)labels[ec];
        const float ay = (y >= 0 && y < nc) ? ap[(long)y * S] : 0.f;
        if (live) sx += (m + logf(sum)) - ay;
      }
    }
    if (labels) {
      const int y = (int)labels[ec];
      for (int c = 0; c < nc; ++c) {
        const float v = ap[(long)c * S];
        const float p = a_is_prob ? v : expf(v - m) * inv;
        const float t = (live && c == y) ? 1.f : 0.f;
        const float r0 = wave_sum(p * t), r1 = wave_sum(live ? p * p : 0.f), r2 = wave_sum(t);
        if (lane == 0) { my[c] += r0; my[nc + c] += r1; my[2 * nc + c] += r2; }
      }
    } else {
      const float* bp = b + bi * nc * S + s;
      float m2, sum2;
      softmax_norm_strided(bp, nc, S, m2, sum2);
      const float inv2 = 1.0f / sum2;
      for (int c = 0; c < nc; ++c) {
        const float v = ap[(long)c * S];
        const float p = live ? (a_is_prob ? v : expf(v - m) * inv) : 0.f;
        const float q = live ? expf(bp[(long)c * S] - m2) * inv2 : 0.f;
        const float d = p - q;
        sx += d * d;
        const float r0 = wave_sum(p * q), r1 = wave_sum(p), r2 = wave_sum(q);
        if (lane == 0) { my[c] += r0; my[nc + c] += r1; my[2 * nc + c] += r2; }
      }
    }
  }
  {
    const float rx = wave_sum(sx);
    if (lane == 0) my[3 * nc] = rx;
  }
  __syncthreads();
  for (int t = threadIdx.x; t < nslot; t += 256)
    part[(long)bx * nslot + t] = ((acc[0][t] + acc[1][t]) + acc[2][t]) + acc[3][t];
}
__global__ __launch_bounds__(256) void loss_stats_generic_kernel(const float* __restrict__ a, const float* __restrict__ b,
                                                                 const long long* __restrict__ labels, float* __restrict__ part,
                                                                 int B, int nc, long S, int a_is_prob) {
  loss_stats_generic_body(a, b, labels, part, B, nc, S, a_is_prob, blockIdx.x, gridDim.x);
}

__device__ __forceinline__ void loss_grad_generic_body(const float* __restrict__ a, const float* __restrict__ b,
                                                       const long long* __restrict__ labels, const float* __restrict__ stats,
                                                       const float* __restrict__ weight, const float* __restrict__ gout0,
                                                       const float* __restrict__ gout1, float* __restrict__ ga, int B, int nc,
                                                       long S, int mode, float inv_vox, float inv_elems, int a_is_prob, int bx, int nbx) {
  __shared__ float al[kLossMaxNc], be[kLossMaxNc], gm[kLossMaxNc];
  const float g0 = gout0 ? gout0[0] : 0.f, g1 = gout1 ? gout1[0] : 0.f;
  for (int c = threadIdx.x; c < nc; c += 256) {
    const float num = 2.f * stats[c] + kDiceEps;
    const float den = stats[nc + c] + stats[2 * nc + c] + kDiceEps;
    const float w = (weight ? weight[c] : 1.f) * g1 / (float)nc;
    float x = 0.f, y = 0.f, z = 0.f;
    if (mode == 0 || mode == 1) { x = -2.f * w / den; y = 2.f * w * num / (den * den); }
    else if (mode == 2) { x = -2.f * w / den; z = w * num / (den * den); }
    else { x = -2.f * g0 * inv_elems; y = 2.f * g0 * inv_elems; }
    al[c] = x; be[c] = y; gm[c] = z;
  }
  __syncthreads();
  const float kappa = (mode == 1) ? g0 * inv_vox : 0.f;
  const long total = (long)B * S;
  for (long e = (long)bx * 256 + threadIdx.x; e < total; e += (long)nbx * 256) {
    const long bi = e / S, s = e - bi * S;
    const float* ap = a + bi * nc * S + s;
    float* gp = ga + bi * nc * S + s;
    float m = 0.f, inv = 1.f;
    if (!a_is_prob) {
      float sum;
      softmax_norm_strided(ap, nc, S, m, sum);
      inv = 1.0f / sum;
    }
    if (labels) {
      const int y = (int)labels[e];
      float dot = 0.f;
      if (!a_is_prob) {
        for (int c = 0; c < nc; ++c) {
          const float p = expf(ap[(long)c * S] - m) * inv;
          dot += ((c == y ? al[c] : 0.f) + be[c] * p + gm[c]) * p;
        }
      }
      for (int c = 0; c < nc; ++c) {
        const float v = ap[(long)c * S];
        const float p = a_is_prob ? v : expf(v - m) * inv;
        const float T = (c == y) ? 1.f : 0.f;
        const float d = al[c] * T + be[c] * p + gm[c];
        gp[(long)c * S] = (a_is_prob ? d : p * (d - dot)) + kappa * (p - T);
      }
    } else {
      const float* bp = b + bi * nc * S + s;
      float m2, sum2;
      softmax_norm_strided(bp, nc, S, m2, sum2);
      const float inv2 = 1.0f / sum2;
      float dot = 0.f;
      if (!a_is_prob) {
        for (int c = 0; c < nc; ++c) {
          const float p = expf(ap[(long)c * S] - m) * inv;
          const float T = expf(bp[(long)c * S] - m2) * inv2;
          dot += (al[c] * T + be[c] * p + gm[c]) * p;
        }
      }
      for (int c = 0; c < nc; ++c) {
        const float v = ap[(long)c * S];
        const float p = a_is_prob ? v : expf(v - m) * inv;
        const float T = expf(bp[(long)c * S] - m2) * inv2;
        const float d = al[c] * T + be[c] * p + gm[c];
        gp[(long)c * S] = a_is_prob ? d : p * (d - dot);
      }
    }
  }
}
__global__ __launch_bounds__(256) void loss_grad_generic_kernel(const float* __restrict__ a, const float* __restrict__ b,
                                                                const long long* __restrict__ labels, const float* __restrict__ stats,
                                                                const float* __restrict__ weight, const float* __restrict__ gout0,
                                                                const float* __restrict__ gout1, float* __restrict__ ga, int B, int nc,
                                                                long S, int mode, float inv_vox, float inv_elems, int a_is_prob) {
  loss_grad_generic_body(a, b, labels, stats, weight, gout0, gout1, ga, B, nc, S, mode, inv_vox, inv_elems, a_is_prob, blockIdx.x, gridDim.x);
}

constexpr int kLossMulti = 12;
struct LossMulti {
  const float* a[kLossMulti]; const float* b[kLossMulti]; const long long* lab[kLossMulti]; const float* weight[kLossMulti];
  float* stats[kLossMulti]; float* out[kLossMulti];
  const float* g0[kLossMulti]; const float* g1[kLossMulti]; float* ga[kLossMulti];
  long S[kLossMulti];
  int B[kLossMulti], nc[kLossMulti], mode[kLossMulti], aip[kLossMulti], nblk[kLossMulti];
};
template <int NCMAX>
__global__ __launch_bounds__(256) void loss_stats_multi_kernel(LossMulti m) {
  const int j = blockIdx.y;
  if ((int)blockIdx.x >= m.nblk[j]) return;
  loss_stats_body<NCMAX>(m.a[j], m.b[j], m.lab[j], m.stats[j] + (3 * m.nc[j] + 1), m.B[j], m.nc[j], m.S[j], m.aip[j], blockIdx.x, m.nblk[j]);
}
__global__ __launch_bounds__(256) void loss_finalize_multi_kernel(LossMulti m) {
  const int j = blockIdx.x;
  const float total = (float)((long)m.B[j] * m.S[j]);
  loss_finalize_body(m.stats[j] + (3 * m.nc[j] + 1), m.nblk[j], m.stats[j], m.weight[j], m.out[j], m.nc[j], 1.0f / total,
                     1.0f / (total * (float)m.nc[j]), m.mode[j]);
}
template <int NCMAX>
__global__ __launch_bounds__(256) void loss_grad_multi_kernel(LossMulti m) {
  const int j = blockIdx.y;
  if ((int)blockIdx.x >= m.nblk[j]) return;
  const float total = (float)((long)m.B[j] * m.S[j]);
  loss_grad_body<NCMAX>(m.a[j], m.b[j], m.lab[j], m.stats[j], m.weight[j], m.g0[j], m.g1[j], m.ga[j], m.B[j], m.nc[j], m.S[j], m.mode[j],
                        1.0f / total, 1.0f / (total * (float)m.nc[j]), m.aip[j], blockIdx.x, m.nblk[j]);
}

__global__ __launch_bounds__(256) void loss_stats_generic_multi_kernel(LossMulti m) {
  const int j = blockIdx.y;
  if ((int)blockIdx.x >= m.nblk[j]) return;
  loss_stats_generic_body(m.a[j], m.b[j], m.lab[j], m.stats[j] + (3 * m.nc[j] + 1), m.B[j], m.nc[j], m.S[j], m.aip[j], blockIdx.x, m.nblk[j]);
}
__global__ __launch_bounds__(256) void loss_grad_generic_multi_kernel(LossMulti m) {
  const int j = blockIdx.y;
  if ((int)blockIdx.x >= m.nblk[j]) return;
  const float total = (float)((long)m.B[j] * m.S[j]);
  loss_grad_generic_body(m.a[j], m.b[j], m.lab[j], m.stats[j], m.weight[j], m.g0[j], m.g1[j], m.ga[j], m.B[j], m.nc[j], m.S[j], m.mode[j],
                         1.0f / total, 1.0f / (total * (float)m.nc[j]), m.aip[j], blockIdx.x, m.nblk[j]);
}

}
```

icl_amd/csrc/kernels/pool_resize.h:

```cpp
#pragma once

namespace icl {

__global__ __launch_bounds__(256) void maxpool2_fwd_kernel(const float* __restrict__ x, float* __restrict__ y,
                                                           unsigned char* __restrict__ idx, long NC, int Do, int Ho, int Wo, int pd,
                                                           const float* __restrict__ ss) {
  const long total = NC * Do * Ho * Wo;
  const int H = Ho * 2, W = Wo * 2;
  const int nk = 4 * pd;
  for (long o = (long)blockIdx.x * blockDim.x + threadIdx.x; o < total; o += (long)gridDim.x * blockDim.x) {
    const int ox = (int)(o % Wo);
    long t = o / Wo;
    const int oy = (int)(t % Ho);
    t /= Ho;
    const int oz = (int)(t % Do);
    const long nc = t / Do;
    const float* p = x + ((nc * (Do * pd) + oz * pd) * H + oy * 2) * (long)W + ox * 2;
    const float sc = ss ? ss[2 * nc] : 1.f, sh = ss ? ss[2 * nc + 1] : 0.f;
    float best = ss ? norm_relu1(p[0], sc, sh) : p[0];
    int bi = 0;
    for (int k = 1; k < nk; ++k) {
      float v = p[((k >> 2) * H + ((k >> 1) & 1)) * (long)W + (k & 1)];
      if (ss) v = norm_relu1(v, sc, sh);
      if (v > best) { best = v; bi = k; }
    }
    y[o] = best;
    idx[o] = (unsigned char)bi;
  }
}

__global__ __launch_bounds__(256) void maxpool2_fwd_x2_kernel(const float* __restrict__ x, float* __restrict__ y,
                                                              unsigned char* __restrict__ idx, long NC, int Do, int Ho, int Wo, int pd,
                                                              const float* __restrict__ ss) {
  const int Wo2 = Wo >> 1;
  const long total = NC * Do * Ho * Wo2;
  const int H = Ho * 2, W = Wo * 2;
  const int nk = 4 * pd;
  for (long o2 = (long)blockIdx.x * blockDim.x + threadIdx.x; o2 < total; o2 += (long)gridDim.x * blockDim.x) {
    const int ox = (int)(o2 % Wo2) * 2;
    long t = o2 / Wo2;
    const int oy = (int)(t % Ho);
    t /= Ho;
    const int oz = (int)(t % Do);
    const long nc = t / Do;
    const long o = ((nc * Do + oz) * Ho + oy) * (long)Wo + ox;
    const float* p = x + ((nc * (Do * pd) + oz * pd) * H + oy * 2) * (long)W + ox * 2;
    const float sc = ss ? ss[2 * nc] : 1.f, sh = ss ? ss[2 * nc + 1] : 0.f;
    float b0 = 0.f, b1 = 0.f;
    int i0 = 0, i1 = 0;
    for (int k = 0; k < nk; k += 2) {
      float4 v = *reinterpret_cast<const float4*>(p + ((k >> 2) * H + ((k >> 1) & 1)) * (long)W);
      if (ss) { v.x = norm_relu1(v.x, sc, sh); v.y = norm_relu1(v.y, sc, sh); v.z = norm_relu1(v.z, sc, sh); v.w = norm_relu1(v.w, sc, sh); }
      if (k == 0) { b0 = v.x; b1 = v.z; }
      else {
        if (v.x > b0) { b0 = v.x; i0 = k; }
        if (v.z > b1) { b1 = v.z; i1 = k; }
      }
      if (v.y > b0) { b0 = v.y; i0 = k + 1; }
      if (v.w > b1) { b1 = v.w; i1 = k + 1; }
    }
    *reinterpret_cast<float2*>(y + o) = make_float2(b0, b1);
    idx[o] = (unsigned char)i0;
    idx[o + 1] = (unsigned char)i1;
  }
}

__global__ __launch_bounds__(256) void maxpool2_bwd_kernel(const float* __restrict__ gy, const unsigned char* __restrict__ idx,
                                                           float* __restrict__ gx, long NC, int Do, int Ho, int Wo, int pd) {
  const long total = NC * Do * Ho * Wo;
  const int H = Ho * 2, W = Wo * 2;
  const int nk = 4 * pd;
  for (long o = (long)blockIdx.x * blockDim.x + threadIdx.x; o < total; o += (long)gridDim.x * blockDim.x) {
    const int ox = (int)(o % Wo);
    long t = o / Wo;
    const int oy = (int)(t % Ho);
    t /= Ho;
    const int oz = (int)(t % Do);
    const long nc = t / Do;
    float* p = gx + ((nc * (Do * pd) + oz * pd) * H + oy * 2) * (long)W + ox * 2;
    const float g = gy[o];
    const int bi = idx[o];
    for (int k = 0; k < nk; k += 2) {
      float2 v = make_float2(bi == k ? g : 0.f, bi == k + 1 ? g : 0.f);
      *reinterpret_cast<float2*>(p + ((k >> 2) * H + ((k >> 1) & 1)) * (long)W) = v;
    }
  }
}

__global__ __launch_bounds__(256) void maxpool2_bwd_add_kernel(const float* __restrict__ gy, const unsigned char* __restrict__ idx,
                                                               const float* __restrict__ add, float* __restrict__ gx, long NC, int C, int Do,
                                                               int Ho, int Wo, int pd, long add_bstride, long NCskip) {
  const long total = NC * Do * Ho * Wo;
  const int H = Ho * 2, W = Wo * 2;
  const long plane = (long)Do * pd * H * W;
  const int nk = 4 * pd;
  for (long o = (long)blockIdx.x * blockDim.x + threadIdx.x; o < total; o += (long)gridDim.x * blockDim.x) {
    const int ox = (int)(o % Wo);
    long t = o / Wo;
    const int oy = (int)(t % Ho);
    t /= Ho;
    const int oz = (int)(t % Do);
    const long nc = t / Do;
    const long in_plane = ((long)(oz * pd) * H + oy * 2) * (long)W + ox * 2;
    float* p = gx + nc * plane + in_plane;
    const float* a = add + (nc / C) * add_bstride + (nc % C) * plane + in_plane;
    const float g = gy[o];
    const int bi = idx[o];
    for (int k = 0; k < nk; k += 2) {
      const long off = ((k >> 2) * H + ((k >> 1) & 1)) * (long)W;
      const float2 s = nc < NCskip ? *reinterpret_cast<const float2*>(a + off) : make_float2(0.f, 0.f);
      *reinterpret_cast<float2*>(p + off) = make_float2(s.x + (bi == k ? g : 0.f), s.y + (bi == k + 1 ? g : 0.f));
    }
  }
}

__global__ __launch_bounds__(256) void maxpool2_bwd_add_x2_kernel(const float* __restrict__ gy, const unsigned char* __restrict__ idx,
                                                                  const float* __restrict__ add, float* __restrict__ gx, long NC, int C, int Do,
                                                                  int Ho, int Wo, int pd, long add_bstride, long NCskip) {
  const int Wo2 = Wo >> 1;
  const long total = NC * Do * Ho * Wo2;
  const int H = Ho * 2, W = Wo * 2;
  const long plane = (long)Do * pd * H * W;
  const int nk = 4 * pd;
  for (long o2 = (long)blockIdx.x * blockDim.x + threadIdx.x; o2 < total; o2 += (long)gridDim.x * blockDim.x) {
    const int ox = (int)(o2 % Wo2) * 2;
    long t = o2 / Wo2;
    const int oy = (int)(t % Ho);
    t /= Ho;
    const int oz = (int)(t % Do);
    const long nc = t / Do;
    const long o = ((nc * Do + oz) * Ho + oy) * (long)Wo + ox;
    const long in_plane = ((long)(oz * pd) * H + oy * 2) * (long)W + ox * 2;
    float* p = gx + nc * plane + in_plane;
    const float* a = add + (nc / C) * add_bstride + (nc % C) * plane + in_plane;
    const float2 g = *reinterpret_cast<const float2*>(gy + o);
    const int b0 = idx[o], b1 = idx[o + 1];
    for (int k = 0; k < nk; k += 2) {
      const long off = ((k >> 2) * H + ((k >> 1) & 1)) * (long)W;
      const float4 s = nc < NCskip ? *reinterpret_cast<const float4*>(a + off) : make_float4(0.f, 0.f, 0.f, 0.f);
      *reinterpret_cast<float4*>(p + off) = make_float4(s.x + (b0 == k ? g.x : 0.f), s.y + (b0 == k + 1 ? g.x : 0.f),
                                                        s.z + (b1 == k ? g.y : 0.f), s.w + (b1 == k + 1 ? g.y : 0.f));
    }
  }
}

struct LinTap { int i0, i1; float l0, l1; };
__device__ __forceinline__ LinTap lin_tap(int dst, float rscale, int in_size, int align) {
  float src = align ? rscale * (float)dst : rscale * ((float)dst + 0.5f) - 0.5f;
  if (src < 0.f) src = 0.f;
  LinTap t;
  t.i0 = (int)src;
  if (t.i0 > in_size - 1) t.i0 = in_size - 1;
  t.i1 = t.i0 + (t.i0 < in_size - 1 ? 1 : 0);
  t.l1 = src - (float)t.i0;
  t.l0 = 1.f - t.l1;
  return t;
}

__global__ __launch_bounds__(256) void trilinear_fwd_kernel(const float* __restrict__ x, float* __restrict__ y, int N, int C,
                                                            int Di, int Hi, int Wi, int Do, int Ho, int Wo,
                                                            float rz, float ry, float rx, long y_bstride, int align) {
  const long per_n = (long)C * Do * Ho * Wo;
  const long total = (long)N * per_n;
  for (long o = (long)blockIdx.x * blockDim.x + threadIdx.x; o < total; o += (long)gridDim.x * blockDim.x) {
    const int ox = (int)(o % Wo);
    long t = o / Wo;
    const int oy = (int)(t % Ho);
    t /= Ho;
    const int oz = (int)(t % Do);
    t /= Do;
    const int c = (int)(t % C);
    const int n = (int)(t / C);
    const LinTap tz = lin_tap(oz, rz, Di, align), ty = lin_tap(oy, ry, Hi, align), tx = lin_tap(ox, rx, Wi, align);
    const float* p = x + ((long)n * C + c) * Di * Hi * Wi;
    const long z0 = (long)tz.i0 * Hi * Wi, z1 = (long)tz.i1 * Hi * Wi;
    const long y0 = (long)ty.i0 * Wi, y1 = (long)ty.i1 * Wi;
    const float v =
        tz.l0 * (ty.l0 * (tx.l0 * p[z0 + y0 + tx.i0] + tx.l1 * p[z0 + y0 + tx.i1]) +
                 ty.l1 * (tx.l0 * p[z0 + y1 + tx.i0] + tx.l1 * p[z0 + y1 + tx.i1])) +
        tz.l1 * (ty.l0 * (tx.l0 * p[z1 + y0 + tx.i0] + tx.l1 * p[z1 + y0 + tx.i1]) +
                 ty.l1 * (tx.l0 * p[z1 + y1 + tx.i0] + tx.l1 * p[z1 + y1 + tx.i1]));
    y[(long)n * y_bstride + (((long)c * Do + oz) * Ho + oy) * Wo + ox] = v;
  }
}

__global__ __launch_bounds__(256) void trilinear_fwd_quad_kernel(const float* __restrict__ x, float* __restrict__ y, int N, int C,
                                                                 int Di, int Hi, int Wi, int Do, int Ho, int Wo,
                                                                 float rz, float ry, float rx, long y_bstride, int align) {
  const unsigned wq = (unsigned)Wo >> 2;
  const unsigned total = (unsigned)N * C * Do * Ho * wq;
  for (unsigned e = blockIdx.x * blockDim.x + threadIdx.x; e < total; e += gridDim.x * blockDim.x) {
    const unsigned xq = e % wq;
    unsigned t = e / wq;
    const int oy = (int)(t % (unsigned)Ho);
    t /= (unsigned)Ho;
    const int oz = (int)(t % (unsigned)Do);
    t /= (unsigned)Do;
    const int c = (int)(t % (unsigned)C);
    const int n = (int)(t / (unsigned)C);
    const LinTap tz = lin_tap(oz, rz, Di, align), ty = lin_tap(oy, ry, Hi, align);
    const float* p = x + ((long)n * C + c) * Di * Hi * Wi;
    const float* p00 = p + (long)tz.i0 * Hi * Wi + (long)ty.i0 * Wi;
    const float* p01 = p + (long)tz.i0 * Hi * Wi + (long)ty.i1 * Wi;
    const float* p10 = p + (long)tz.i1 * Hi * Wi + (long)ty.i0 * Wi;
    const float* p11 = p + (long)tz.i1 * Hi * Wi + (long)ty.i1 * Wi;
    float v[4];
#pragma unroll
    for (int k = 0; k < 4; ++k) {
      const LinTap tx = lin_tap((int)(xq * 4) + k, rx, Wi, align);
      v[k] = tz.l0 * (ty.l0 * (tx.l0 * p00[tx.i0] + tx.l1 * p00[tx.i1]) + ty.l1 * (tx.l0 * p01[tx.i0] + tx.l1 * p01[tx.i1])) +
             tz.l1 * (ty.l0 * (tx.l0 * p10[tx.i0] + tx.l1 * p10[tx.i1]) + ty.l1 * (tx.l0 * p11[tx.i0] + tx.l1 * p11[tx.i1]));
    }
    *reinterpret_cast<float4*>(y + (long)n * y_bstride + (((long)c * Do + oz) * Ho + oy) * Wo + xq * 4) = make_float4(v[0], v[1], v[2], v[3]);
  }
}

__device__ __forceinline__ float up2_even(float prev, float cur, bool first) { return first ? cur : 0.25f * prev + 0.75f * cur; }
__device__ __forceinline__ float up2_odd(float cur, float next) { return 0.75f * cur + 0.25f * next; }

__global__ __launch_bounds__(256) void upsample2x_fwd_kernel(const float* __restrict__ x, float* __restrict__ y, int N, int C, int Di,
                                                             int Hi, int Wi, long y_bstride, const float* __restrict__ ss) {
  const unsigned wq = (unsigned)Wi >> 1;
  const unsigned total = (unsigned)N * C * Di * Hi * wq;
  const int Ho = 2 * Hi, Wo = 2 * Wi;
  for (unsigned e = blockIdx.x * blockDim.x + threadIdx.x; e < total; e += gridDim.x * blockDim.x) {
    const unsigned xq = e % wq;
    unsigned t = e / wq;
    const int iy = (int)(t % (unsigned)Hi);
    t /= (unsigned)Hi;
    const int iz = (int)(t % (unsigned)Di);
    t /= (unsigned)Di;
    const int c = (int)(t % (unsigned)C);
    const int n = (int)(t / (unsigned)C);
    const float* p = x + ((long)n * C + c) * Di * Hi * Wi;
    const float sc = ss ? ss[2 * (n * C + c)] : 1.f, sh = ss ? ss[2 * (n * C + c) + 1] : 0.f;
    const int ix = (int)xq * 2;
    const int xa = ix > 0 ? ix - 1 : 0, xd = ix + 2 < Wi ? ix + 2 : Wi - 1;
    float r[3][3][4];
#pragma unroll
    for (int dz = 0; dz < 3; ++dz) {
      int z = iz + dz - 1;
      z = z < 0 ? 0 : (z > Di - 1 ? Di - 1 : z);
#pragma unroll
      for (int dy = 0; dy < 3; ++dy) {
        int yy = iy + dy - 1;
        yy = yy < 0 ? 0 : (yy > Hi - 1 ? Hi - 1 : yy);
        const float* row = p + ((long)z * Hi + yy) * Wi;
        float a = row[xa], b = row[ix], cc = row[ix + 1], d = row[xd];
        if (ss) { a = norm_relu1(a, sc, sh); b = norm_relu1(b, sc, sh); cc = norm_relu1(cc, sc, sh); d = norm_relu1(d, sc, sh); }
        r[dz][dy][0] = up2_even(a, b, ix == 0);
        r[dz][dy][1] = up2_odd(b, cc);
        r[dz][dy][2] = up2_even(b, cc, false);
        r[dz][dy][3] = up2_odd(cc, d);
      }
    }
    float u[3][2][4];
#pragma unroll
    for (int dz = 0; dz < 3; ++dz)
#pragma unroll
      for (int k = 0; k < 4; ++k) {
        u[dz][0][k] = up2_even(r[dz][0][k], r[dz][1][k], iy == 0);
        u[dz][1][k] = up2_odd(r[dz][1][k], r[dz][2][k]);
      }
    float* yo = y + (long)n * y_bstride + (((long)c * (2 * Di) + 2 * iz) * Ho + 2 * iy) * Wo + ix * 2;
#pragma unroll
    for (int py = 0; py < 2; ++py) {
      float ev[4], od[4];
#pragma unroll
      for (int k = 0; k < 4; ++k) {
        ev[k] = up2_even(u[0][py][k], u[1][py][k], iz == 0);
        od[k] = up2_odd(u[1][py][k], u[2][py][k]);
      }
      *reinterpret_cast<float4*>(yo + (long)py * Wo) = make_float4(ev[0], ev[1], ev[2], ev[3]);
      *reinterpret_cast<float4*>(yo + ((long)Ho + py) * Wo) = make_float4(od[0], od[1], od[2], od[3]);
    }
  }
}

__device__ __forceinline__ void up2_adj_weights(int i, int n, float w[4]) {
  w[0] = i > 0 ? 0.25f : 0.f;
  w[1] = i > 0 ? 0.75f : 1.f;
  w[2] = i < n - 1 ? 0.75f : 1.f;
  w[3] = i < n - 1 ? 0.25f : 0.f;
}

__global__ __launch_bounds__(256) void upsample2x_fwd_x4_kernel(const float* __restrict__ x, float* __restrict__ y, int N, int C, int Di,
                                                                int Hi, int Wi, long y_bstride, const float* __restrict__ ss) {
  const unsigned wq = (unsigned)Wi >> 2;
  const unsigned total = (unsigned)N * C * Di * Hi * wq;
  const int Ho = 2 * Hi, Wo = 2 * Wi;
  for (unsigned e = blockIdx.x * blockDim.x + threadIdx.x; e < total; e += gridDim.x * blockDim.x) {
    const unsigned xq = e % wq;
    unsigned t = e / wq;
    const int iy = (int)(t % (unsigned)Hi);
    t /= (unsigned)Hi;
    const int iz = (int)(t % (unsigned)Di);
    t /= (unsigned)Di;
    const int c = (int)(t % (unsigned)C);
    const int n = (int)(t / (unsigned)C);
    const float* p = x + ((long)n * C + c) * Di * Hi * Wi;
    const float sc = ss ? ss[2 * (n * C + c)] : 1.f, sh = ss ? ss[2 * (n * C + c) + 1] : 0.f;
    const int ix = (int)xq * 4;
    const int xa = ix > 0 ? ix - 1 : 0, xd = ix + 4 < Wi ? ix + 4 : Wi - 1;
    float r[3][3][8];
#pragma unroll
    for (int dz = 0; dz < 3; ++dz) {
      int z = iz + dz - 1;
      z = z < 0 ? 0 : (z > Di - 1 ? Di - 1 : z);
#pragma unroll
      for (int dy = 0; dy < 3; ++dy) {
        int yy = iy + dy - 1;
        yy = yy < 0 ? 0 : (yy > Hi - 1 ? Hi - 1 : yy);
        const float* row = p + ((long)z * Hi + yy) * Wi;
        const float4 q = *reinterpret_cast<const float4*>(row + ix);
        float v[6] = {row[xa], q.x, q.y, q.z, q.w, row[xd]};
        if (ss) {
#pragma unroll
          for (int k = 0; k < 6; ++k) v[k] = norm_relu1(v[k], sc, sh);
        }
#pragma unroll
        for (int k = 0; k < 4; ++k) {
          r[dz][dy][2 * k] = up2_even(v[k], v[k + 1], ix + k == 0);
          r[dz][dy][2 * k + 1] = up2_odd(v[k + 1], v[k + 2]);
        }
      }
    }
    float u[3][2][8];
#pragma unroll
    for (int dz = 0; dz < 3; ++dz)
#pragma unroll
      for (int k = 0; k < 8; ++k) {
        u[dz][0][k] = up2_even(r[dz][0][k], r[dz][1][k], iy == 0);
        u[dz][1][k] = up2_odd(r[dz][1][k], r[dz][2][k]);
      }
    float* yo = y + (long)n * y_bstride + (((long)c * (2 * Di) + 2 * iz) * Ho + 2 * iy) * Wo + ix * 2;
#pragma unroll
    for (int py = 0; py < 2; ++py) {
      float ev[8], od[8];
#pragma unroll
      for (int k = 0; k < 8; ++k) {
        ev[k] = up2_even(u[0][py][k], u[1][py][k], iz == 0);
        od[k] = up2_odd(u[1][py][k], u[2][py][k]);
      }
      float* e0 = yo + (long)py * Wo;
      float* o0 = yo + ((long)Ho + py) * Wo;
      *reinterpret_cast<float4*>(e0) = make_float4(ev[0], ev[1], ev[2], ev[3]);
      *reinterpret_cast<float4*>(e0 + 4) = make_float4(ev[4], ev[5], ev[6], ev[7]);
      *reinterpret_cast<float4*>(o0) = make_float4(od[0], od[1], od[2], od[3]);
      *reinterpret_cast<float4*>(o0 + 4) = make_float4(od[4], od[5], od[6], od[7]);
    }
  }
}

constexpr int kUpSeg = 8;
__global__ __launch_bounds__(256) void upsample2x_bwd_kernel(const float* __restrict__ gy, float* __restrict__ gx, int N, int C, int Di,
                                                             int Hi, int Wi, long gy_bstride) {
  const unsigned wq = (unsigned)Wi >> 2;
  const unsigned nseg = ((unsigned)Di + kUpSeg - 1) / kUpSeg;
  const unsigned total = (unsigned)N * C * nseg * Hi * wq;
  const int Do = 2 * Di, Ho = 2 * Hi, Wo = 2 * Wi;
  for (unsigned e = blockIdx.x * blockDim.x + threadIdx.x; e < total; e += gridDim.x * blockDim.x) {
    const unsigned xq = e % wq;
    unsigned t = e / wq;
    const int iy = (int)(t % (unsigned)Hi);
// ... 261 lines not shown
```

icl_amd/ops.py:

```python
from __future__ import annotations

import ctypes
import functools
import math
import os
from typing import NamedTuple, Optional, Sequence

import torch

from . import _lib
from .step_scope import BackwardEnd, DeferredBiasGrads, DeferredWgradReduce, FactoredGrads, ScopeField, StepScope, WgradLane

_vp = ctypes.c_void_p


def _ptr(t: Optional[torch.Tensor]):
    return None if t is None else _vp(t.data_ptr())


def _stream(t: torch.Tensor):
    if t.is_cuda:
        return _vp(torch.cuda.current_stream(t.device).cuda_stream)
    return None

# ... 2047 lines not shown
        if bcast and R <= QC_ROWS_PER_PASS:
            gqin = new(1, nc, C)
            _qc_stage(kv, dp, y=gqin, R=R, K=C, trans=2, nc=nc, x=dn1, pro=QC_PRO_LNBWD, pa=xhat1, pb=rstd1, pc=n1w, epi=QC_EPI_SUMB)
        else:
            gqin = new(B, nc, C)
            _qc_stage(kv, dp, y=gqin, R=R, K=C, trans=2, nc=nc, x=dn1, pro=QC_PRO_LNBWD, pa=xhat1, pb=rstd1, pc=n1w)
            if bcast:
                gqin = gqin.sum(0, keepdim=True)
        gn1w, gn1b, gfqw, gfqb = new(C), new(C), new(C, C), new(C)
        jobs += [(dn1, xhat1, gn1w, gn1b, R, C, C, 1), (gq, n1, gfqw, gfqb, R, C, C, 0)]
        grads[0:4] = [gn1w, gn1b, gfqw, gfqb]
        _qc_wgrad(kv, jobs)
        return (gqin, gkv, None, *grads)


def query_attend(q_in, kv, heads, scale, ba, eps, dp, full, params):
    cfg = dict(heads=int(heads), scale=float(scale), ba=int(ba), eps=float(eps), dp=dp, full=bool(full))
    return _QueryAttend.apply(q_in, kv, cfg, *params)


def drop_path_site(like, p: float, training: bool):
    if p == 0.0 or not training:
        return (0, 0, 1.0), None
    seed, seed_dev = _step_seed(like, None)
    return (seed, int(p * 4294967296.0) & 0xFFFFFFFF, 1.0 / (1.0 - p)), seed_dev



LOSS_MAX_BLOCKS = 1024


class _FusedLoss(torch.autograd.Function):

    @staticmethod
    def forward(ctx, a, target, weight, mode, a_is_prob):
        _require(a, target, weight)
        L = _lib.lib()
        a = a.contiguous()
        target = target.contiguous()
        B, nc = a.shape[0], a.shape[1]
        _check_classes(nc, "loss")
        S = a.numel() // (B * nc)
        hard = mode <= 1
        if hard:
            assert target.dtype == torch.int64 and target.numel() == B * S, "labels must be int64 [B, ...]"
        else:
            assert target.shape == a.shape and target.dtype == torch.float32
        stats = torch.empty((3 * nc + 1) * (1 + LOSS_MAX_BLOCKS), dtype=torch.float32, device=a.device)
        out = torch.empty(2, dtype=torch.float32, device=a.device)
        _lib.check(L.icl_loss_fwd(_ptr(a), None if hard else _ptr(target), _ptr(target) if hard else None, _ptr(weight),
                                  _ptr(stats), _ptr(out), B, nc, S, mode, int(a_is_prob), _stream(a)), "loss_fwd")
        ctx.save_for_backward(a, target, stats, weight)
        ctx.cfg = (mode, int(a_is_prob))
        ctx.set_materialize_grads(False)
        return out[0], out[1]

    @staticmethod
    def backward(ctx, g0, g1):
        a, target, stats, weight = ctx.saved_tensors
        mode, aip = ctx.cfg
        L = _lib.lib()
        B, nc = a.shape[0], a.shape[1]
        S = a.numel() // (B * nc)
        hard = mode <= 1
        g0 = g0.contiguous() if g0 is not None else None
        g1 = g1.contiguous() if g1 is not None else None
        ga = torch.empty_like(a)
        _lib.check(L.icl_loss_bwd(_ptr(a), None if hard else _ptr(target), _ptr(target) if hard else None, _ptr(weight),
                                  _ptr(stats), _ptr(g0), _ptr(g1), _ptr(ga), B, nc, S, mode, aip, _stream(a)), "loss_bwd")
        return ga, None, None, None, None


class _LossJob(ctypes.Structure):
    _fields_ = [("a", _vp), ("b", _vp), ("labels", _vp), ("weight", _vp), ("stats", _vp), ("out", _vp), ("gout0", _vp), ("gout1", _vp),
                ("ga", _vp), ("s", ctypes.c_int64), ("batch", ctypes.c_int), ("nc", ctypes.c_int), ("mode", ctypes.c_int),
                ("a_is_prob", ctypes.c_int)]


LOSS_MULTI_MAX = 12
LOSS_MULTI = os.environ.get("ICL_LOSS_MULTI", "1") != "0"


class _FusedLossMulti(torch.autograd.Function):

    @staticmethod
    def forward(ctx, modes, *tensors):
        L = _lib.lib()
        n = len(modes)
        assert 1 <= n <= LOSS_MULTI_MAX and len(tensors) == 2 * n
        a_s = [tensors[2 * j].contiguous() for j in range(n)]
        t_s = [tensors[2 * j + 1].contiguous() for j in range(n)]
        _require(*a_s, *t_s)
        dev = a_s[0].device
        nc = a_s[0].shape[1]
        _check_classes(nc, "loss")
        per = (3 * nc + 1) * (1 + LOSS_MAX_BLOCKS)
        stats = torch.empty((n, per), dtype=torch.float32, device=dev)
        out = torch.empty((n, 2), dtype=torch.float32, device=dev)
        jobs = (_LossJob * n)()
        for j in range(n):
            a, t, mode = a_s[j], t_s[j], modes[j]
            B = a.shape[0]
            S = a.numel() // (B * nc)
            hard = mode <= 1
            assert a.shape[1] == nc
            if hard:
                assert t.dtype == torch.int64 and t.numel() == B * S, "labels must be int64 [B, ...]"
            else:
                assert t.shape == a.shape and t.dtype == torch.float32
            q = jobs[j]
            q.a, q.b, q.labels, q.weight = a.data_ptr(), (None if hard else t.data_ptr()), (t.data_ptr() if hard else None), None
            q.stats, q.out = stats[j].data_ptr(), out[j].data_ptr()
            q.s, q.batch, q.nc, q.mode, q.a_is_prob = S, B, nc, mode, 0
        _lib.check(L.icl_loss_fwd_multi(jobs, n, _stream(a_s[0])), "loss_fwd_multi")
        ctx.save_for_backward(stats, *a_s, *t_s)
        ctx.modes = tuple(modes)
        ctx.set_materialize_grads(False)
        return tuple(out[j, k] for j in range(n) for k in (0, 1))

    @staticmethod
    def backward(ctx, *gs):
        L = _lib.lib()
        modes = ctx.modes
        n = len(modes)
        stats = ctx.saved_tensors[0]
        a_s, t_s = ctx.saved_tensors[1:1 + n], ctx.saved_tensors[1 + n:1 + 2 * n]
        nc = a_s[0].shape[1]
        gas = [None] * n
        keep = []
        live = [j for j in range(n) if ctx.needs_input_grad[1 + 2 * j] and (gs[2 * j] is not None or gs[2 * j + 1] is not None)]
        jobs = (_LossJob * max(len(live), 1))()
        for i, j in enumerate(live):
            a, t, mode = a_s[j], t_s[j], modes[j]
            B = a.shape[0]
            S = a.numel() // (B * nc)
            hard = mode <= 1
            g0 = gs[2 * j].contiguous() if gs[2 * j] is not None else None
            g1 = gs[2 * j + 1].contiguous() if gs[2 * j + 1] is not None else None
            keep += [g0, g1]
            gas[j] = torch.empty_like(a)
            q = jobs[i]
            q.a, q.b, q.labels, q.weight = a.data_ptr(), (None if hard else t.data_ptr()), (t.data_ptr() if hard else None), None
            q.stats, q.out = stats[j].data_ptr(), None
            q.gout0, q.gout1, q.ga = _ptr(g0), _ptr(g1), gas[j].data_ptr()
            q.s, q.batch, q.nc, q.mode, q.a_is_prob = S, B, nc, mode, 0
        if live:
            _lib.check(L.icl_loss_bwd_multi(jobs, len(live), _stream(a_s[0])), "loss_bwd_multi")
        res = [None]
        for j in range(n):
            res += [gas[j], None]
        return tuple(res)


def fused_losses(terms):
    if not terms:
        return []
    ncs = {t[0].shape[1] for t in terms}
    if not LOSS_MULTI or len(terms) > LOSS_MULTI_MAX or len(ncs) != 1:
        return [_FusedLoss.apply(a, (t.long() if m <= 1 else t.detach()), None, m, False) for a, t, m in terms]
    flat = []
    for a, t, m in terms:
        flat += [a, (t.long() if m <= 1 else t.detach())]
    out = _FusedLossMulti.apply(tuple(m for _, _, m in terms), *flat)
    return [(out[2 * j], out[2 * j + 1]) for j in range(len(terms))]


class _CombineScalars(torch.autograd.Function):

    @staticmethod
    def forward(ctx, W, *terms):
        n, m = len(terms), len(W)
        ts = [t if (t.dtype == torch.float32 and t.dim() == 0) else t.float().reshape(()) for t in terms]
        _require(*ts)
        out = torch.empty(m, dtype=torch.float32, device=ts[0].device)
        arr = (ctypes.c_void_p * n)(*[t.data_ptr() for t in ts])
        flat = (ctypes.c_float * (m * n))(*[float(W[j][i]) for j in range(m) for i in range(n)])
        _lib.check(_lib.lib().icl_scalar_combine(arr, flat, n, m, _ptr(out), _stream(out)), "scalar_combine")
        ctx.W = W
        ctx.n = n
        return out

    @staticmethod
    def backward(ctx, gout):
        W, n = ctx.W, ctx.n
        m = len(W)
        gout = gout.contiguous()
        gin = torch.empty(n, dtype=torch.float32, device=gout.device)
        arr = (ctypes.c_void_p * m)(*[gout.data_ptr() + 4 * j for j in range(m)])
        flat = (ctypes.c_float * (n * m))(*[float(W[j][i]) for i in range(n) for j in range(m)])
        _lib.check(_lib.lib().icl_scalar_combine(arr, flat, m, n, _ptr(gin), _stream(gin)), "scalar_combine_bwd")
        return (None,) + tuple(gin[i] for i in range(n))


def combine_scalars(terms, W) -> torch.Tensor:
    return _CombineScalars.apply(tuple(tuple(float(v) for v in row) for row in W), *terms)


def _weight_tensor(weight, like):
    if weight is None:
        return None
    return torch.as_tensor(weight, dtype=torch.float32, device=like.device)


def dice_loss(inputs: torch.Tensor, labels: torch.Tensor, n_classes: int, softmax: bool = False, weight=None):
    assert inputs.shape[1] == n_classes
    return _FusedLoss.apply(inputs, labels.long(), _weight_tensor(weight, inputs), 0, not softmax)[1]


def cross_entropy_dice_parts(logits: torch.Tensor, labels: torch.Tensor, n_classes: int):
    assert logits.shape[1] == n_classes
    return _FusedLoss.apply(logits, labels.long(), None, 1, False)


def cross_entropy_dice(logits: torch.Tensor, labels: torch.Tensor, n_classes: int):
    ce, dc = cross_entropy_dice_parts(logits, labels, n_classes)
    return ce + dc


def soft_dice_loss(a: torch.Tensor, b: torch.Tensor):
    return _FusedLoss.apply(a, b.detach(), None, 2, False)[1]


def softmax_mse(a: torch.Tensor, b: torch.Tensor):
    return _FusedLoss.apply(a, b.detach(), None, 3, False)[0]



_SEG_DTYPES = {torch.uint8: 1, torch.bool: 1, torch.int64: 8}


def seg_metrics_shape(t: torch.Tensor):
    shape = tuple(t.shape)
    if len(shape) < 3 or any(s != 1 for s in shape[:-3]):
        return None
    return shape[-3], shape[-2], shape[-1], int(len(shape) > 3)


def _seg_label_maps(who, *maps, exactly_3d=False):
    first = maps[0]
    if len(maps) == 2 and first.shape != maps[1].shape:
        raise ValueError(f"{who}: shapes differ {tuple(first.shape)} vs {tuple(maps[1].shape)}")
    geo = seg_metrics_shape(first)
    if exactly_3d and first.dim() != 3:
        raise ValueError(f"{who}: needs a 3-D label map, got {tuple(first.shape)}")
    if geo is None:
        raise ValueError(f"{who}: needs a 3-D label map (leading axes of length 1 allowed), got {tuple(first.shape)}")
    for t in maps:
        if t.dtype not in _SEG_DTYPES:
            raise TypeError(f"{who}: unsupported label dtype {t.dtype}")
        if not t.is_cuda and not _lib.host_pointers_ok():
            raise RuntimeError("icl_amd: HIP kernels need device tensors (no CPU fallback)")
    if len(maps) == 2 and first.device != maps[1].device:
        raise ValueError(f"{who}: pred and gt on different devices")
    return [t.contiguous() for t in maps], geo


def _seg_workspace(who, ws_bytes, geo, num_classes, device):
    nbytes = ws_bytes(*geo[:3], int(num_classes))
    if nbytes < 0:
        raise ValueError(f"{who}: shape {geo[:3]} / num_classes {num_classes} not supported (2 <= num_classes <= 256)")
    return torch.empty(nbytes, dtype=torch.uint8, device=device)


def seg_metrics(pred: torch.Tensor, gt: torch.Tensor, num_classes: int) -> torch.Tensor:
    L = _lib.lib()
    (pred, gt), geo = _seg_label_maps("seg_metrics", pred, gt)
    ws = _seg_workspace("seg_metrics", L.icl_seg_metrics_ws_bytes, geo, num_classes, pred.device)
    out = torch.empty((int(num_classes) - 1, 6), dtype=torch.int64, device=pred.device)
    _lib.check(L.icl_seg_metrics(_ptr(pred), _SEG_DTYPES[pred.dtype], _ptr(gt), _SEG_DTYPES[gt.dtype], *geo[:3], int(num_classes), geo[3],
                                 _ptr(out), _ptr(ws), _stream(pred)), "seg_metrics")
    return out


def seg_surface_metrics(pred: torch.Tensor, gt: torch.Tensor, num_classes: int, spacing, tolerance: float = 1.0):
    (pred, gt), (n0, n1, n2, _) = _seg_label_maps("seg_surface_metrics", pred, gt, exactly_3d=True)
    try:
        sp = [float(v) for v in spacing]
    except TypeError:
        raise ValueError(f"seg_surface_metrics: spacing must be three numbers, got {spacing!r}") from None
    if len(sp) != 3 or not all(math.isfinite(v) and v > 0 for v in sp):
        raise ValueError(f"seg_surface_metrics: spacing must be three finite positive numbers, got {spacing!r}")
    tol = float(tolerance)
    if not (math.isfinite(tol) and tol >= 0):
        raise ValueError(f"seg_surface_metrics: tolerance must be finite and not negative, got {tolerance!r}")
    L = _lib.lib()
    ws = _seg_workspace("seg_surface_metrics", L.icl_seg_surface_ws_bytes, (n0, n1, n2), num_classes, pred.device)
    counts = torch.empty((int(num_classes) - 1, 7), dtype=torch.int64, device=pred.device)
    values = torch.empty((int(num_classes) - 1, 6), dtype=torch.float64, device=pred.device)
    _lib.check(L.icl_seg_surface_metrics(_ptr(pred), _SEG_DTYPES[pred.dtype], _ptr(gt), _SEG_DTYPES[gt.dtype], n0, n1, n2, int(num_classes),
                                         sp[0], sp[1], sp[2], tol, _ptr(counts), _ptr(values), _ptr(ws), _stream(pred)), "seg_surface_metrics")
    return counts, values


def _seg_components_args(who, label_map, num_classes, connectivity):
    (m,), (n0, n1, n2, _) = _seg_label_maps(who, label_map)
    if isinstance(connectivity, bool) or not isinstance(connectivity, int) or connectivity not in (1, 2, 3):
        raise ValueError(f"{who}: connectivity must be 1, 2 or 3, got {connectivity!r}")
    return m, n0, n1, n2, _seg_workspace(who, _lib.lib().icl_seg_components_ws_bytes, (n0, n1, n2), num_classes, m.device)


def seg_components(label_map: torch.Tensor, num_classes: int, connectivity: int = 1):
    m, n0, n1, n2, ws = _seg_components_args("seg_components", label_map, num_classes, connectivity)
    labels = torch.empty(label_map.shape, dtype=torch.int32, device=m.device)
    counts = torch.empty((int(num_classes) - 1, 3), dtype=torch.int64, device=m.device)
    _lib.check(_lib.lib().icl_seg_components(_ptr(m), _SEG_DTYPES[m.dtype], n0, n1, n2, int(num_classes), connectivity, _ptr(labels),
                                             _ptr(counts), _ptr(ws), _stream(m)), "seg_components")
    return labels, counts


def seg_filter_components(label_map: torch.Tensor, num_classes: int, connectivity: int = 1, keep_largest: bool = True, min_size: int = 0,
# ... 100 lines not shown
```

icl_amd/utils/losses.py:

```python
from __future__ import annotations

import torch
import torch.nn as nn
from torch.nn.modules.loss import CrossEntropyLoss

from .. import ops


def dice_loss1(score, target):
    target = target.float()
    smooth = 1e-5
    intersect = torch.sum(score * target)
    return 1 - (2 * intersect + smooth) / (torch.sum(score) + torch.sum(target) + smooth)


def softmax_dice_loss(input_logits, target_logits):
    assert input_logits.size() == target_logits.size()
    return ops.soft_dice_loss(input_logits, target_logits)


def _mean_of(leaves):
    if len(leaves) == 1:
        return leaves[0]
    return ops.combine_scalars(leaves, [[1.0 / len(leaves)] * len(leaves)])[0]


def softmax_mse_leaves(input_logits, target_logits):
    return [ops.softmax_mse(a, b.detach()) for a, b in zip(input_logits, target_logits)]


def softmax_mse_loss(input_logits, target_logits, sigmoid=False):
    if sigmoid:
        raise NotImplementedError("the ICL trainers never pass sigmoid=True")
    return _mean_of(softmax_mse_leaves(input_logits, target_logits))


class DiceLoss(nn.Module):

    def __init__(self, n_classes):
        super().__init__()
        self.n_classes = n_classes

    def forward(self, inputs, target, weight=None, softmax=False):
        assert inputs.shape[1] == self.n_classes and inputs.shape[0] == target.shape[0] \
            and inputs.shape[2:] == target.shape[2:], \
            "predict {} & target {} shape do not match".format(inputs.size(), target.size())
        return ops.dice_loss(inputs, target[:, 0], self.n_classes, softmax, weight)


def _resize(t, size):
    return ops.trilinear_resize(t.float(), size)


def _resize2d(t, size):
    return ops.bilinear_resize(t.float(), size)


class AuxLoss(nn.Module):

    def __init__(self, n_classes, resize=(224, 224)):
        super().__init__()
        self.n_classes = n_classes
        self.ce_loss = CrossEntropyLoss()
        self.dice_loss = DiceLoss(n_classes)
        self.resize = tuple(resize)

    def leaves(self, feat_maps, labels):
        out = []
        for fm in feat_maps:
            out += list(ops.cross_entropy_dice_parts(_resize2d(fm, self.resize), labels.long(), self.n_classes))
        return out

    def forward(self, feat_maps, labels):
        lv = self.leaves(feat_maps, labels)
        return ops.combine_scalars(lv, [[1.0 / len(feat_maps)] * len(lv)])[0]


class PseudoSoftLoss(nn.Module):

    def __init__(self, n_classes, resize=(224, 224)):
        super().__init__()
        self.resize = tuple(resize)

    def leaves(self, feat_maps, predicts):
        tgt = predicts.detach()
        return [softmax_dice_loss(_resize2d(fm, self.resize), tgt) for fm in feat_maps]

    def forward(self, feat_maps, predicts):
        return _mean_of(self.leaves(feat_maps, predicts))


class AuxLoss3D(nn.Module):

    def __init__(self, n_classes, resize=(96, 96, 96)):
        super().__init__()
        self.n_classes = n_classes
        self.ce_loss = CrossEntropyLoss()
        self.dice_loss = DiceLoss(n_classes)
        self.resize = tuple(resize)

    def leaves(self, feat_maps, labels):
        out = []
        for fm in feat_maps:
            out += list(ops.cross_entropy_dice_parts(_resize(fm, self.resize), labels.long(), self.n_classes))
        return out

    def terms(self, feat_maps, labels):
        return [(_resize(fm, self.resize), labels, 1) for fm in feat_maps]

    def forward(self, feat_maps, labels):
        lv = self.leaves(feat_maps, labels)
        return ops.combine_scalars(lv, [[1.0 / len(feat_maps)] * len(lv)])[0]


class PseudoSoftLoss3D(nn.Module):

    def __init__(self, n_classes, resize=(96, 96, 96)):
        super().__init__()
        self.resize = tuple(resize)

    def leaves(self, feat_maps, predicts):
        tgt = predicts.detach()
        return [softmax_dice_loss(_resize(fm, self.resize), tgt) for fm in feat_maps]

    def terms(self, feat_maps, predicts):
        tgt = predicts.detach()
        return [(_resize(fm, self.resize), tgt, 2) for fm in feat_maps]

    def forward(self, feat_maps, predicts):
        return _mean_of(self.leaves(feat_maps, predicts))
```

include/icl_hip.h:

```cpp
#ifndef ICL_HIP_H
#define ICL_HIP_H
#include <stdint.h>
#ifdef __cplusplus
extern "C" {
#endif

int icl_abi_version(void);
const char* icl_last_error(void);
const char* icl_last_kernel_name(void);

int64_t icl_conv3d_packed_elems(int cout, int cin, int ks, int mode);
int icl_conv3d_pack_weights(const float* w, float* wp, int cout, int cin, int ks, int mode, void* stream);
int icl_conv3d_pack_weights_both(const float* w, float* wp_fwd, float* wp_dgrad, int cout, int cin, int ks, void* stream);
int icl_conv3d_pack_weights_multi(const void* const* w, void* const* wp_fwd, void* const* wp_dgrad, const int32_t* cout, const int32_t* cin,
                                  const int32_t* ks, int count, void* stream);
int64_t icl_conv3d_fwd_ws_bytes(int n, int cin, int cout, int d, int h, int w, int ks);
int64_t icl_conv3d_split_ws_bytes(int cin, int cout);
int icl_conv3d_split_weights_multi(const void* const* wp, void* const* wsplit, const int32_t* cin, const int32_t* cout, int count,
                                   void* stream);
int icl_conv3d_fwd_presplit(const float* x, const void* wsplit, const float* bias, float* y, int n, int cin, int cout, int d, int h, int w,
                            int64_t x_bstride, int64_t y_bstride, void* stream);
int64_t icl_conv3d_fwd_presplit_ws_bytes(int n, int cin, int cout, int d, int h, int w);
int icl_conv3d_fwd_presplit_ws(const float* x, const void* wsplit, const float* bias, float* y, void* ws, int n, int cin, int cout, int d,
                               int h, int w, int64_t x_bstride, int64_t y_bstride, void* stream);
int icl_conv3d_fwd_stats_slots(int n, int cin, int cout, int d, int h, int w);
int icl_conv3d_fwd_presplit_stats(const float* x, const void* wsplit, const float* bias, float* y, float* stats, int n, int cin, int cout,
                                  int d, int h, int w, int64_t x_bstride, int64_t y_bstride, void* stream);
int icl_conv3d_fwd(const float* x, const float* wp, const float* bias, float* y, void* ws, int n, int cin, int cout, int d, int h,
                   int w, int ks, int64_t x_bstride, int64_t y_bstride, void* stream);
int64_t icl_conv3d_wgrad_ws_bytes(int n, int cin, int cout, int ks);
int icl_conv3d_wgrad(const float* x, const float* gy, float* gw, float* gbias, void* ws, int n, int cin, int cout, int d,
                     int h, int w, int ks, int64_t x_bstride, int64_t gy_bstride, void* stream);
int icl_conv3d_wgrad_slabs(const float* x, const float* gy, void* ws, int n, int cin, int cout, int d, int h, int w, int ks,
                           int64_t x_bstride, int64_t gy_bstride, int32_t* nslabs, void* stream);
int icl_conv3d_wgrad_reduce_multi(const void* const* ws, void* const* gw, const int32_t* cout, const int32_t* cin, const int32_t* ks,
                                  const int32_t* nslabs, int count, void* stream);

int icl_conv3d_fwd_live_ok(int n, int n_live, int cin, int cout, int d, int h, int w);
const char* icl_last_live_fwd_kernel_name(void);
void icl_last_wgrad_grid(int32_t* launched, int32_t* planned);
int icl_conv3d_fwd_presplit_live(const float* x, const void* wsplit, const float* bias, float* y, int n, int n_live, int cin, int cout, int d,
                                 int h, int w, int64_t x_bstride, int64_t y_bstride, void* stream);
int icl_conv3d_fwd_presplit_ws_live(const float* x, const void* wsplit, const float* bias, float* y, void* ws, int n, int n_live, int cin,
                                    int cout, int d, int h, int w, int64_t x_bstride, int64_t y_bstride, void* stream);
int icl_conv3d_fwd_live(const float* x, const float* wp, const float* bias, float* y, void* ws, int n, int n_live, int cin, int cout, int d,
                        int h, int w, int ks, int64_t x_bstride, int64_t y_bstride, void* stream);
int64_t icl_conv3d_wgrad_ws_bytes_live(int n, int n_live, int cin, int cout, int ks);
int icl_conv3d_wgrad_live(const float* x, const float* gy, float* gw, float* gbias, void* ws, int n, int n_live, int cin, int cout, int d,
                          int h, int w, int ks, int64_t x_bstride, int64_t gy_bstride, void* stream);
int icl_conv3d_wgrad_slabs_live(const float* x, const float* gy, void* ws, int n, int n_live, int cin, int cout, int d, int h, int w, int ks,
                                int64_t x_bstride, int64_t gy_bstride, int32_t* nslabs, void* stream);

int64_t icl_norm_ws_bytes(int n, int c, int64_t s);
int icl_norm_fwd(const float* x, float* y, float* mean, float* rstd, const float* gamma, const float* beta,
                 float* running_mean, float* running_var, int n, int c, int64_t s, int mode, int use_batch_stats,
                 int act, float eps, float momentum, void* ws, void* stream);
int icl_norm_bwd(const float* gy, const float* x, const float* mean, const float* rstd, const float* gamma,
                 const float* beta, float* gx, float* dgamma, float* dbeta, int n, int c, int64_t s, int mode,
                 int use_batch_stats, int act, void* ws, void* stream);
int icl_norm_bwd_live(const float* gy, const float* x, const float* mean, const float* rstd, const float* gamma, const float* beta, float* gx,
                      float* dgamma, float* dbeta, int n, int n_live, int c, int64_t s, int mode, int use_batch_stats, int act, void* ws,
                      void* stream);
int icl_norm_fwd_given_stats(const float* x, const float* res, float* y, float* mean, float* rstd, const float* gamma, const float* beta,
                             float* running_mean, float* running_var, int n, int c, int64_t s, int mode, int act, float eps,
                             float momentum, const float* part, int nslots, void* stream);
int icl_norm_res_fwd(const float* x, const float* res, float* y, float* mean, float* rstd, const float* gamma, const float* beta,
                     float* running_mean, float* running_var, int n, int c, int64_t s, int mode, int use_batch_stats,
                     int act, float eps, float momentum, void* ws, void* stream);
int icl_norm_res_bwd(const float* gy, const float* x, const float* res, const float* mean, const float* rstd, const float* gamma,
                     const float* beta, float* gx, float* gres, float* dgamma, float* dbeta, int n, int c, int64_t s, int mode,
                     int use_batch_stats, int act, void* ws, void* stream);
int icl_rstd_from_var(const float* var, float* rstd, int c, float eps, void* stream);

int icl_norm_finalize_stats(const float* part, int n, int c, int nslots, float eps, float* mean, float* rstd, float* ss, void* stream);
int icl_norm_apply(const float* x, const float* ss, float* y, int n, int c, int64_t s, void* stream);
int icl_maxpool2_fwd_norm(const float* x, const float* ss, float* y, uint8_t* idx, int64_t nc, int dout, int hout, int wout, int pool_depth,
                          void* stream);
int icl_upsample2x_concat_norm(const float* skip, const float* skip_ss, const float* deep, const float* deep_ss, float* out, int n, int cs,
                               int cd, int d, int h, int w, void* stream);

int icl_maxpool2_fwd(const float* x, float* y, uint8_t* idx, int64_t nc, int dout, int hout, int wout, int pool_depth, void* stream);
int icl_maxpool2_bwd(const float* gy, const uint8_t* idx, float* gx, int64_t nc, int dout, int hout, int wout, int pool_depth, void* stream);
int icl_maxpool2_bwd_add(const float* gy, const uint8_t* idx, const float* add, float* gx, int n, int c, int dout, int hout, int wout,
                         int pool_depth, int64_t add_bstride, void* stream);
int icl_maxpool2_bwd_add_live(const float* gy, const uint8_t* idx, const float* add, float* gx, int n, int skip_live, int c, int dout, int hout,
                              int wout, int pool_depth, int64_t add_bstride, void* stream);

int icl_trilinear_fwd(const float* x, float* y, int n, int c, int di, int hi, int wi, int dout, int hout, int wout,
                      int64_t y_bstride, int align_corners, void* stream);
int64_t icl_trilinear_bwd_ws_bytes(int n, int c, int di, int hi, int wi, int dout, int hout, int wout);
int icl_trilinear_bwd(const float* gy, float* gx, void* ws, int n, int c, int di, int hi, int wi, int dout, int hout, int wout,
                      int64_t gy_bstride, int align_corners, void* stream);
int icl_trilinear_bwd_live(const float* gy, float* gx, void* ws, int n, int n_live, int c, int di, int hi, int wi, int dout, int hout, int wout,
                           int64_t gy_bstride, int align_corners, void* stream);

int icl_copy_rows(const float* src, float* dst, int64_t rows, int64_t row_elems, int64_t src_stride, int64_t dst_stride,
                  void* stream);

int icl_concat2(const float* a, int64_t na, const float* b, int64_t nb, float* out, void* stream);

int icl_dwconv3_fwd(const float* x, const float* w, float* y, int n, int c, int d, int h, int wd, int flip, void* stream);
int64_t icl_dwconv3_wgrad_ws_bytes(int n, int c, int d, int h, int wd);
int icl_dwconv3_wgrad(const float* x, const float* gy, float* gw, void* ws, int n, int c, int d, int h, int wd, void* stream);

int icl_conv1x1_small(const float* x, const float* w, const float* bias, float* y, int n, int cin, int cout, int64_t s, int w_ostride,
                      int w_istride, void* stream);
int icl_conv1x1_dropout(const float* x, const float* w, const float* bias, float* y, int n, int cin, int cout, int64_t s, int w_ostride,
                        int w_istride, int mask_mode, uint32_t seed, float p, const uint32_t* seed_dev, void* stream);
int icl_conv1x1_wgrad_dropout(const float* x, const float* gy, float* gw, float* gbias, void* ws, int n, int cin, int cout, int64_t s,
                              int64_t gy_bstride, uint32_t seed, float p, const uint32_t* seed_dev, void* stream);
int icl_conv1x1_dropout_norm(const float* x, const float* ss, const float* w, const float* bias, float* y, int n, int cin, int cout, int64_t s,
                             int w_ostride, int w_istride, uint32_t seed, float p, const uint32_t* seed_dev, void* stream);
int icl_conv1x1_wgrad_dropout_norm(const float* x, const float* ss, const float* gy, float* gw, float* gbias, void* ws, int n, int cin,
                                   int cout, int64_t s, int64_t gy_bstride, uint32_t seed, float p, const uint32_t* seed_dev, void* stream);
int icl_conv1x1_small_live(const float* x, const float* w, const float* bias, float* y, int n, int n_live, int cin, int cout, int64_t s,
                           int w_ostride, int w_istride, void* stream);
int icl_conv1x1_dropout_live(const float* x, const float* w, const float* bias, float* y, int n, int n_live, int cin, int cout, int64_t s,
                             int w_ostride, int w_istride, int mask_mode, uint32_t seed, float p, const uint32_t* seed_dev, void* stream);
int icl_conv1x1_wgrad_dropout_live(const float* x, const float* gy, float* gw, float* gbias, void* ws, int n, int n_live, int cin, int cout,
                                   int64_t s, int64_t gy_bstride, uint32_t seed, float p, const uint32_t* seed_dev, void* stream);
int icl_conv1x1_wgrad_dropout_norm_live(const float* x, const float* ss, const float* gy, float* gw, float* gbias, void* ws, int n, int n_live,
                                        int cin, int cout, int64_t s, int64_t gy_bstride, uint32_t seed, float p, const uint32_t* seed_dev,
                                        void* stream);

int icl_dropout(const float* x, float* y, int64_t n, uint32_t seed, float p, const uint32_t* seed_dev, void* stream);
int icl_drop_path(const float* x, float* y, int64_t n, int64_t group, uint32_t seed, float p, const uint32_t* seed_dev, void* stream);
int icl_drop_path_add(const float* x, const float* res, float* y, int64_t n, int64_t group, uint32_t seed, float p,
                      const uint32_t* seed_dev, void* stream);

#define ICL_LOSS_MAX_BLOCKS 1024
#define ICL_LOSS_STATS_FLOATS(nc) ((3 * (nc) + 1) * (1 + ICL_LOSS_MAX_BLOCKS))
int icl_loss_fwd(const float* a, const float* b, const int64_t* labels, const float* weight, float* stats, float* out,
                 int batch, int nc, int64_t s, int mode, int a_is_prob, void* stream);
int icl_loss_bwd(const float* a, const float* b, const int64_t* labels, const float* weight, const float* stats,
                 const float* gout0, const float* gout1, float* ga, int batch, int nc, int64_t s, int mode, int a_is_prob,
                 void* stream);
typedef struct IclLossJob {
  const float* a; const float* b; const int64_t* labels; const float* weight;
  float* stats; float* out;
  const float* gout0; const float* gout1; float* ga;
  int64_t s;
  int batch, nc, mode, a_is_prob;
} IclLossJob;
int icl_loss_fwd_multi(const IclLossJob* jobs, int count, void* stream);
int icl_loss_bwd_multi(const IclLossJob* jobs, int count, void* stream);

int icl_layernorm_fwd(const float* x, const float* gamma, const float* beta, float* y, float* mean, float* rstd, int64_t rows,
                      int c, float eps, void* stream);
int64_t icl_layernorm_bwd_ws_bytes(int64_t rows, int c);
int icl_layernorm_bwd(const float* gy, const float* x, const float* gamma, const float* mean, const float* rstd, float* gx,
                      float* dgamma, float* dbeta, void* ws, int64_t rows, int c, void* stream);
int icl_gelu_fwd(const float* x, float* y, int64_t n, void* stream);
int icl_gelu_bwd(const float* gy, const float* x, float* gx, int64_t n, void* stream);
int icl_attn_fwd(const float* q, const float* kv, float* logits, float* out, float* stats, int b, int h, int nc, int n, int d,
                 float scale, void* stream);
int icl_attn_bwd(const float* q, const float* kv, const float* logits, const float* stats, const float* out, const float* gout,
                 const float* glog, float* gq, float* gkv, int b, int h, int nc, int n, int d, float scale, void* stream);
int64_t icl_attn_bwd_ws_bytes(int b, int h, int nc, int n, int d);
int icl_attn_bwd_ws(const float* q, const float* kv, const float* logits, const float* stats, const float* out, const float* gout,
                    const float* glog, float* gq, float* gkv, void* ws, int b, int h, int nc, int n, int d, float scale, void* stream);

int icl_colsum_multi(const void* const* g, void* const* out, const int32_t* rows, const int32_t* cols, int count, void* stream);
int icl_scalar_combine(const void* const* in, const float* w, int n_in, int n_out, float* out, void* stream);

int icl_gather_rows(const float* src, const int32_t* idx, float* out, int64_t b, int64_t s, int64_t m, int c, void* stream);
int icl_gather_rows_sum2(const float* src, const int32_t* idx2, float* out, int64_t b, int64_t s, int64_t m, int c, void* stream);

int icl_im2col3(const float* x, float* cols, int n, int c, int d, int h, int w, void* stream);
int icl_im2col3_planes(const float* x, float* planes, int n, int c, int d, int h, int w, void* stream);

int icl_conv3d_cin1_fwd(const float* x, const float* w, const float* bias, float* y, int n, int cout, int d, int h, int wd, int64_t x_bstride,
                        int64_t y_bstride, void* stream);
int64_t icl_conv3d_cin1_wgrad_ws_bytes(int n, int d, int h);
int icl_conv3d_cin1_wgrad(const float* x, const float* gy, float* gw, void* ws, int n, int cout, int d, int h, int wd, int64_t x_bstride,
                          int64_t gy_bstride, void* stream);
int icl_col2im3(const float* g, float* dx, int n, int c, int d, int h, int w, void* stream);

int icl_depth_to_space2(const float* yt, float* out, int n, int d, int h, int w, int cout, int64_t out_bstride, void* stream);
int icl_space_to_depth2(const float* g, float* gt, int n, int d, int h, int w, int cout, int64_t g_bstride, void* stream);

int64_t icl_linear_ws_bytes(int64_t rows, int in, int out, int kind);
int icl_linear_fwd(const float* x, const float* w, const float* bias, float* y, void* ws, int64_t rows, int in, int out, int act,
                   void* stream);
int icl_linear_dgrad(const float* gy, const float* w, float* gx, void* ws, int64_t rows, int in, int out, void* stream);
int icl_linear_bwd_small(const float* gy, const float* w, const float* x, float* gx, float* dw, void* ws, int64_t rows, int in, int out,
                         void* stream);
int icl_linear_wgrad_small(const float* gy, const float* x, float* dw, void* ws, int64_t rows, int in, int out, void* stream);
int icl_linear_dgrad_sgd(const float* gy, const float* x, float* w, float* mom, float* gx, void* ws, int64_t rows, int in, int out,
                         float lr, float momentum, float weight_decay, int first, const float* lr_dev, void* stream);
int64_t icl_gemm_ws_bytes(int64_t m, int n, int k, int batch);
int icl_gemm(const float* a, const float* b, float* c, const float* bias, void* ws, int64_t m, int n, int k, int64_t lda, int64_t ldb,
             int64_t ldc, int a_kcontig, int b_kcontig, int act, int batch, int64_t a_bstride, int64_t b_bstride, int64_t c_bstride,
             void* stream);

int64_t icl_linear_wgrad_ws_bytes(int64_t rows, int o, int i);
int icl_linear_wgrad(const float* gy, const float* x, float* dw, float* db, void* ws, int64_t rows, int o, int i, void* stream);

int64_t icl_conv1x1_wgrad_ws_bytes(int n, int64_t s, int cin, int cout);
int icl_conv1x1_wgrad(const float* x, const float* gy, float* gw, float* gbias, void* ws, int n, int cin, int cout, int64_t s,
                      int64_t x_bstride, int64_t gy_bstride, void* stream);
int icl_conv1x1_wgrad_live(const float* x, const float* gy, float* gw, float* gbias, void* ws, int n, int n_live, int cin, int cout, int64_t s,
                           int64_t x_bstride, int64_t gy_bstride, void* stream);

int64_t icl_window_attn_bias_elems(int n, int heads);
int icl_relpos_bias_fwd(const float* table, const int64_t* index, float* bias, int n, int heads, int idx_stride, void* stream);
int icl_window_attn_fwd(const float* qkv, const float* bias, const int32_t* regions, float* out, float* lse, int b_, int n, int heads,
                        int nw, int head_dim, float scale, void* stream);
int icl_window_attn_bwd(const float* qkv, const float* bias, const int32_t* regions, const float* out, const float* lse,
                        const float* dout, float* dqkv, float* dbias, int b_, int n, int heads, int nw, int head_dim, float scale,
                        void* stream);
int icl_window_attn_fwd_drop(const float* qkv, const float* bias, const int32_t* regions, float* out, float* lse, int b_, int n, int heads,
                             int nw, int head_dim, float scale, uint32_t seed, float p, const uint32_t* seed_dev, void* stream);
int icl_window_attn_bwd_drop(const float* qkv, const float* bias, const int32_t* regions, const float* out, const float* lse,
                             const float* dout, float* dqkv, float* dbias, int b_, int n, int heads, int nw, int head_dim, float scale,
                             uint32_t seed, float p, const uint32_t* seed_dev, void* stream);
int icl_window_attn_keep_probe(int32_t* out, int64_t base, int count, uint32_t seed, float p, const uint32_t* seed_dev, void* stream);
int icl_window_attn_bwd_chunks(int b_, int n, int heads, int nw, int head_dim);
int icl_relpos_bias_bwd_sum(float* dbias, int chunks, const int32_t* inv, const int32_t* offs, float* dtable, int64_t table_rows, int n,
                            int heads, void* stream);

int icl_crop_rotflip(const void* const* images, const void* const* labels, const int32_t* params, int batch, float* image_out,
                     int64_t* label_out, int o0, int o1, int o2, void* stream);

int icl_volume_feed(const void* const* images, const void* const* labels, const int32_t* int_params, const float* float_params, int batch,
                    float* image_out, int64_t* label_out, int R0, int R1, int R2, void* stream);

int icl_rank_tile(void);
int icl_rank_index_build(const float* image, const uint8_t* label, int n0, int n1, int n2, float threshold, uint32_t* fg_index,
                         uint32_t* bg_index, void* stream);
int icl_rank_select(const void* const* images, const void* const* labels, const void* const* fg_indices, const void* const* bg_indices,
                    const int32_t* int_params, float threshold, int batch, int32_t* origins, void* stream);
int icl_volume_feed_origins(const void* const* images, const void* const* labels, const int32_t* int_params, const float* float_params,
                            int batch, const int32_t* origins, float* image_out, int64_t* label_out, int R0, int R1, int R2, void* stream);

int icl_prefix_box(const float* image, int n0, int n1, int n2, const float* window, int clip, int32_t* box, int32_t* ws, void* stream);
int icl_prefix_resample(const float* image, const uint8_t* label, const int32_t* int_params, const double* double_params, const float* window,
                        int clip, float* image_out, uint8_t* label_out, void* stream);
int icl_prefix_restore(const void* prediction, int elem_kind, const int32_t* int_params, const double* double_params, uint8_t* out,
                       void* stream);

int icl_slice_augment(const void* const* images, const void* const* labels, const int32_t* int_params, const double* double_params,
                      int batch, float* image_out, uint8_t* label_out, int o0, int o1, void* stream);
int icl_slice_resize(const void* src, void* dst, int64_t batch, int n0, int n1, int o0, int o1, int elem_kind, void* stream);

int icl_sgd_step(float* p, const float* g, float* m, int64_t n, float lr, float momentum, float weight_decay, int first,
                 const float* lr_dev, void* stream);
int icl_sgd_step_factored(float* p, float* m, const float* g, const float* x, int rows, int n, int k, float lr, float momentum,
                          float weight_decay, int first, const float* lr_dev, void* stream);
int64_t icl_sgd_factored_split_ws_bytes(int rows, int n, int k);
int icl_sgd_step_factored_split(float* p, float* m, const float* g, const float* x, void* ws, int rows, int n, int k, float lr,
                                float momentum, float weight_decay, int first, const float* lr_dev, void* stream);
int icl_sgd_step_factored_narrow(float* p, float* m, const float* g, const float* x, int rows, int n, int k, float lr, float momentum,
                                 float weight_decay, int first, const float* lr_dev, int workgroups, void* stream);
int icl_sgd_step_multi(void* const* p, const void* const* g, void* const* m, const int64_t* n, int count, float lr,
                       float momentum, float weight_decay, int first, const float* lr_dev, void* stream);

typedef struct IclQcStage {
  const float* x; int x_rows;
  const float* w; const float* bias; float* y;
  int R, K, N, trans, nc, npw;
  int pro, epi;
  const float* pa; const float* pb; const float* pc; const float* pd; int pro_dp;
  float* so0; float* so1; float* so2;
  const float* ea; const float* eb; int ea_r0, ea_r1, eb_r0, eb_r1;
  uint32_t dp_seed[2], dp_thresh[2]; float dp_scale[2]; const uint32_t* dp_seed_dev;
  float eps;
} IclQcStage;
int icl_qchain_stage(const IclQcStage* stage, void* stream);
int icl_qchain_wgrad(const void* const* g, const void* const* x, void* const* dw, void* const* db, const int32_t* rows, const int32_t* n,
                     const int32_t* k, const int32_t* kind, int count, void* stream);

int64_t icl_seg_metrics_ws_bytes(int n0, int n1, int n2, int num_classes);
int icl_seg_metrics(const void* pred, int pred_dtype, const void* gt, int gt_dtype, int n0, int n1, int n2, int num_classes, int all_border,
                    int64_t* out, void* ws, void* stream);

int64_t icl_seg_surface_ws_bytes(int n0, int n1, int n2, int num_classes);
int icl_seg_surface_metrics(const void* pred, int pred_dtype, const void* gt, int gt_dtype, int n0, int n1, int n2, int num_classes, double s0,
                            double s1, double s2, double tolerance, int64_t* counts, double* values, void* ws, void* stream);

int64_t icl_seg_components_ws_bytes(int n0, int n1, int n2, int num_classes);
int icl_seg_components(const void* map, int dtype, int n0, int n1, int n2, int num_classes, int connectivity, int32_t* labels, int64_t* counts,
                       void* ws, void* stream);
int icl_seg_filter_components(const void* map, int dtype, int n0, int n1, int n2, int num_classes, int connectivity, int keep_largest,
                              int64_t min_size, void* out, int64_t* counts , void* ws, void* stream);

int icl_window_gather(const float* vol, float* out, const int32_t* origins, int n, int cin, int s0, int s1, int s2, int a0, int a1, int a2,
                      int p0, int p1, int p2, int r0, int r1, int r2, void* stream);
int icl_window_gather_flipped(const float* vol, float* out, const int32_t* origins, const int32_t* flips, int n, int cin, int s0, int s1,
                              int s2, int a0, int a1, int a2, int p0, int p1, int p2, int r0, int r1, int r2, void* stream);
int icl_window_accumulate(const float* logits, const float* importance, float* score, float* weight, const int32_t* origins, int n, int c,
                          int p0, int p1, int p2, int r0, int r1, int r2, int softmax, void* stream);
int icl_window_accumulate_flipped(const float* logits, const float* importance, float* score, float* weight, const int32_t* origins,
                                  const int32_t* flips, int n, int c, int p0, int p1, int p2, int r0, int r1, int r2, int softmax,
                                  void* stream);
int icl_window_finalize(const float* score, const float* weight, int64_t* label, float* quotients, int c, int p0, int p1, int p2, int a0,
                        int a1, int a2, int s0, int s1, int s2, void* stream);

#ifdef __cplusplus
// ... 4 lines not shown
```

Measured before the change: 206.4 volumes/s.

## Fuse trilinear resize of deep-supervision maps into the multi-loss kernels

The deep-supervision losses no longer materialise each upsampled feature map. The loss stats and grad kernels sample the low-resolution source trilinearly on the fly. The backward pass fuses the x-axis resize adjoint into the loss-grad kernel, writing a partially reduced gradient, and then runs only the y and z adjoint passes. This removes full-resolution resize writes and reads and several launches, at the cost of redundant interpolation arithmetic per voxel and more complex kernels with extra indexing.

Result: no change. 207.5 volumes/s (median of 6 runs) (+0.6%).

```diff
diff --git a/icl_amd/_lib.py b/icl_amd/_lib.py
--- a/icl_amd/_lib.py
+++ b/icl_amd/_lib.py
@@ -130,6 +130,10 @@
     "icl_loss_bwd": (c_int, [P, P, P, P, P, P, P, P, I, I, L, I, I, P]),
     "icl_loss_fwd_multi": (c_int, [P, I, P]),
     "icl_loss_bwd_multi": (c_int, [P, I, P]),
+    "icl_loss_resized_bwd_ws_bytes": (c_int64, [I, I, I, I, I, I, I, I]),
+    "icl_loss_fwd_multi_resized": (c_int, [P, I, P]),
+    "icl_loss_bwd_multi_resized": (c_int, [P, I, P]),
+    "icl_loss_resized_bwd_yz": (c_int, [P, P, P, I, I, I, I, I, I, I, I, P]),
     "icl_qchain_stage": (c_int, [P, P]),
     "icl_qchain_wgrad": (c_int, [P, P, P, P, P, P, P, P, I, P]),
     "icl_seg_metrics_ws_bytes": (c_int64, [I, I, I, I]),
diff --git a/icl_amd/csrc/icl_abi.inc b/icl_amd/csrc/icl_abi.inc
--- a/icl_amd/csrc/icl_abi.inc
+++ b/icl_amd/csrc/icl_abi.inc
@@ -1357,12 +1357,38 @@
   return ((int64_t)n * c * dout * hout * wi + (int64_t)n * c * dout * hi * wi) * 4;
 }
 
+static int resize_bwd_axis(hipStream_t st, int n, int al, const float* src, float* dst, long rows, int li, int lo, long inner, float rs, long sbs,
+                           const char* what) {
+  const long total = (long)n * rows * li * inner;
+  const bool small = total / 4 < (1L << 31) && rows < (1L << 31);
+  if (small && inner % 4 == 0 && sbs % 4 == 0 && aligned16(src) && aligned16(dst)) {
+    ICL_LAUNCH(icl::resize_bwd_axis_t4_kernel, dim3(grid_for(total / 4, 256, 1 << 16)), dim3(256), 0, st, src, dst, n, (unsigned)rows, li, lo,
+               (unsigned)(inner / 4), rs, sbs, al);
+  } else if (inner == 1 && lo >= 4 * li && lo % 4 == 0 && lo <= 1024 && sbs % 4 == 0 && aligned16(src) && rows * li >= 4096) {
+    const long nrows = (long)n * rows;
+    ICL_LAUNCH(icl::resize_bwd_axis_x_lds_kernel, dim3((unsigned)cdivl(nrows, icl::kRbxRows)), dim3(256),
+               (size_t)icl::kRbxRows * (lo + 4) * 4, st, src, dst, n, rows, li, lo, rs, sbs, al);
+  } else if (small && inner == 1 && li % 4 == 0 && aligned16(dst)) {
+    ICL_LAUNCH(icl::resize_bwd_axis_i4_kernel, dim3(grid_for(total / 4, 256, 1 << 16)), dim3(256), 0, st, src, dst, n, (unsigned)rows, li, lo,
+               rs, sbs, al);
+  } else {
+    ICL_LAUNCH(icl::resize_bwd_axis_kernel, dim3(grid_for(total, 256)), dim3(256), 0, st, src, dst, n, rows, li, lo, inner, rs, sbs, al);
+  }
+  return check_launch(what);
+}
+static int resize_bwd_yz(hipStream_t st, int n, int c, int al, const float* t1, float* t2, float* gx, int di, int hi, int wi, int dout, int hout) {
+  const float rz = resize_scale(di, dout, al), ry = resize_scale(hi, hout, al);
+  int rc;
+  if ((rc = resize_bwd_axis(st, n, al, t1, t2, (long)c * dout, hi, hout, (long)wi, ry, (long)c * dout * hout * wi, "resize_bwd_y"))) return rc;
+  return resize_bwd_axis(st, n, al, t2, gx, (long)c, di, dout, (long)hi * wi, rz, (long)c * dout * hi * wi, "resize_bwd_z");
+}
+
 int icl_trilinear_bwd(const float* gy, float* gx, void* ws, int n, int c, int di, int hi, int wi, int dout, int hout, int wout,
                       int64_t gy_bstride, int align_corners, void* stream) {
   if (!gy || !gx || !ws || n < 1 || c < 1 || di < 1 || hi < 1 || wi < 1 || dout < 1 || hout < 1 || wout < 1) return fail(-1, "trilinear_bwd: bad argument");
   hipStream_t st = (hipStream_t)stream;
   const int al = align_corners;
-  const float rz = resize_scale(di, dout, al), ry = resize_scale(hi, hout, al), rx = resize_scale(wi, wout, al);
+  const float rx = resize_scale(wi, wout, al);
   float* t1 = (float*)ws;
   float* t2 = t1 + (size_t)n * c * dout * hout * wi;
   int rc;
@@ -1373,28 +1399,8 @@
                wi, (long)gy_bstride);
     return check_launch("upsample2x_bwd");
   }
-  auto axis = [&](const float* src, float* dst, long rows, int li, int lo, long inner, float rs, long sbs, const char* what) -> int {
-    const long total = (long)n * rows * li * inner;
-    const bool small = total / 4 < (1L << 31) && rows < (1L << 31);
-    if (small && inner % 4 == 0 && sbs % 4 == 0 && aligned16(src) && aligned16(dst)) {
-      ICL_LAUNCH(icl::resize_bwd_axis_t4_kernel, dim3(grid_for(total / 4, 256, 1 << 16)), dim3(256), 0, st, src, dst, n, (unsigned)rows, li, lo,
-                 (unsigned)(inner / 4), rs, sbs, al);
-    } else if (inner == 1 && lo >= 4 * li && lo % 4 == 0 && lo <= 1024 && sbs % 4 == 0 && aligned16(src) && rows * li >= 4096) {
-      const long nrows = (long)n * rows;
-      ICL_LAUNCH(icl::resize_bwd_axis_x_lds_kernel, dim3((unsigned)cdivl(nrows, icl::kRbxRows)), dim3(256),
-                 (size_t)icl::kRbxRows * (lo + 4) * 4, st, src, dst, n, rows, li, lo, rs, sbs, al);
-    } else if (small && inner == 1 && li % 4 == 0 && aligned16(dst)) {
-      ICL_LAUNCH(icl::resize_bwd_axis_i4_kernel, dim3(grid_for(total / 4, 256, 1 << 16)), dim3(256), 0, st, src, dst, n, (unsigned)rows, li, lo,
-                 rs, sbs, al);
-    } else {
-      ICL_LAUNCH(icl::resize_bwd_axis_kernel, dim3(grid_for(total, 256)), dim3(256), 0, st, src, dst, n, rows, li, lo, inner, rs, sbs, al);
-    }
-    return check_launch(what);
-  };
-  if ((rc = axis(gy, t1, (long)c * dout * hout, wi, wout, 1L, rx, (long)gy_bstride, "resize_bwd_x"))) return rc;
-  if ((rc = axis(t1, t2, (long)c * dout, hi, hout, (long)wi, ry, (long)c * dout * hout * wi, "resize_bwd_y"))) return rc;
-  if ((rc = axis(t2, gx, (long)c, di, dout, (long)hi * wi, rz, (long)c * dout * hi * wi, "resize_bwd_z"))) return rc;
-  return 0;
+  if ((rc = resize_bwd_axis(st, n, al, gy, t1, (long)c * dout * hout, wi, wout, 1L, rx, (long)gy_bstride, "resize_bwd_x"))) return rc;
+  return resize_bwd_yz(st, n, c, al, t1, t2, gx, di, hi, wi, dout, hout);
 }
 
 int icl_copy_rows(const float* src, float* dst, int64_t rows, int64_t row_elems, int64_t src_stride, int64_t dst_stride,
@@ -1683,6 +1689,87 @@
     ICL_LAUNCH((icl::loss_grad_multi_kernel<16>), dim3(most, count), dim3(256), 0, (hipStream_t)stream, m);
   }
   return check_launch("loss_grad_multi");
+}
+
+int64_t icl_loss_resized_bwd_ws_bytes(int batch, int nc, int di, int hi, int wi, int dout, int hout, int wout) {
+  (void)di; (void)hout; (void)wout;
+  return (int64_t)batch * nc * dout * hi * wi * 4;
+}
+
+static int loss_multi_resized_fill(const IclLossJobR* jobs, int count, bool bwd, icl::LossMultiR& r, int& most, int& group) {
+  if (!jobs || count < 1 || count > icl::kLossMulti) return fail(-1, "loss_multi_resized: 1 .. %d jobs", icl::kLossMulti);
+  if (loss_force_generic()) return fail(-1, "loss_multi_resized: the generic-class kernels take materialised operands only");
+  icl::LossMulti& m = r.m;
+  most = 1;
+  group = loss_class_group(jobs[0].job.nc);
+  for (int j = 0; j < count; ++j) {
+    const IclLossJobR& qr = jobs[j];
+    const IclLossJob& q = qr.job;
+    if (q.nc < 1 || q.nc > 16) return fail(-1, "loss_multi_resized: job %d has %d classes (1 .. 16)", j, q.nc);
+    if (!q.stats || q.batch < 1 || q.s < 1 || q.mode < 0 || q.mode > 3 || loss_class_group(q.nc) != group)
+      return fail(-1, "loss_multi_resized: bad job %d (all jobs of a call need nc <= 4, or all 5 .. 16)", j);
+    if ((q.mode <= 1) != (q.labels != nullptr) || (q.mode >= 2) != (q.b != nullptr))
+      return fail(-1, "loss_multi_resized: target of job %d does not match its mode", j);
+    if (bwd ? (qr.src ? !qr.gx : !q.ga) : !q.out) return fail(-1, "loss_multi_resized: job %d has no output", j);
+    if ((q.a != nullptr) == (qr.src != nullptr)) return fail(-1, "loss_multi_resized: job %d needs exactly one of a and src", j);
+    const long total = (long)q.batch * q.s;
+    m.a[j] = q.a; m.b[j] = q.b; m.lab[j] = (const long long*)q.labels; m.weight[j] = q.weight; m.stats[j] = q.stats; m.out[j] = q.out;
+    m.g0[j] = q.gout0; m.g1[j] = q.gout1; m.ga[j] = q.ga;
+    m.S[j] = (long)q.s; m.B[j] = q.batch; m.nc[j] = q.nc; m.mode[j] = q.mode; m.aip[j] = q.a_is_prob;
+    m.nblk[j] = bwd ? grid_for(total, 256, 4096) : grid_for(total, 256, ICL_LOSS_MAX_BLOCKS);
+    int blocks = m.nblk[j];
+    if (qr.src) {
+      if (qr.di < 1 || qr.hi < 1 || qr.wi < 1 || qr.dout < 1 || qr.hout < 1 || qr.wout < 1 || (long)qr.dout * qr.hout * qr.wout != (long)q.s ||
+          q.s >= (1L << 31) || (long)qr.di * qr.hi * qr.wi >= (1L << 31))
+        return fail(-1, "loss_multi_resized: extents of job %d (s = dout * hout * wout < 2^31)", j);
+      const int al = qr.align_corners ? 1 : 0;
+      r.src[j] = qr.src; r.gx[j] = qr.gx;
+      r.Di[j] = qr.di; r.Hi[j] = qr.hi; r.Wi[j] = qr.wi; r.Do[j] = qr.dout; r.Ho[j] = qr.hout; r.Wo[j] = qr.wout;
+      r.rz[j] = resize_scale(qr.di, qr.dout, al); r.ry[j] = resize_scale(qr.hi, qr.hout, al); r.rx[j] = resize_scale(qr.wi, qr.wout, al);
+      r.align[j] = al;
+      r.nblk_x[j] = grid_for((long)q.batch * qr.dout * qr.hout * qr.wi, 256, 4096);
+      if (bwd) blocks = r.nblk_x[j];
+    }
+    if (blocks > most) most = blocks;
+  }
+  return 0;
+}
+
+int icl_loss_fwd_multi_resized(const IclLossJobR* jobs, int count, void* stream) {
+  icl::LossMultiR r{};
+  int most = 1, group = 0;
+  int rc = loss_multi_resized_fill(jobs, count, false, r, most, group);
+  if (rc) return rc;
+  hipStream_t st = (hipStream_t)stream;
+  if (group == 0) {
+    ICL_LAUNCH((icl::loss_stats_multi_resized_kernel<4>), dim3(most, count), dim3(256), 0, st, r);
+  } else {
+    ICL_LAUNCH((icl::loss_stats_multi_resized_kernel<16>), dim3(most, count), dim3(256), 0, st, r);
+  }
+  rc = check_launch("loss_stats_multi_resized");
+  if (rc) return rc;
+  ICL_LAUNCH(icl::loss_finalize_multi_kernel, dim3(count), dim3(256), 0, st, r.m);
+  return check_launch("loss_finalize_multi");
+}
+
+int icl_loss_bwd_multi_resized(const IclLossJobR* jobs, int count, void* stream) {
+  icl::LossMultiR r{};
+  int most = 1, group = 0;
+  int rc = loss_multi_resized_fill(jobs, count, true, r, most, group);
+  if (rc) return rc;
+  hipStream_t st = (hipStream_t)stream;
+  if (group == 0) {
+    ICL_LAUNCH((icl::loss_grad_multi_resized_kernel<4>), dim3(most, count), dim3(256), 0, st, r);
+  } else {
+    ICL_LAUNCH((icl::loss_grad_multi_resized_kernel<16>), dim3(most, count), dim3(256), 0, st, r);
+  }
+  return check_launch("loss_grad_multi_resized");
+}
+
+int icl_loss_resized_bwd_yz(const float* gx, void* ws, float* gsrc, int batch, int nc, int di, int hi, int wi, int dout, int hout,
+                            int align_corners, void* stream) {
+  if (!gx || !ws || !gsrc || batch < 1 || nc < 1 || di < 1 || hi < 1 || wi < 1 || dout < 1 || hout < 1) return fail(-1, "loss_resized_bwd_yz: bad argument");
+  return resize_bwd_yz((hipStream_t)stream, batch, nc, align_corners ? 1 : 0, gx, (float*)ws, gsrc, di, hi, wi, dout, hout);
 }
 
 int icl_loss_bwd(const float* a, const float* b, const int64_t* labels, const float* weight, const float* stats,
diff --git a/icl_amd/csrc/kernels/loss.h b/icl_amd/csrc/kernels/loss.h
--- a/icl_amd/csrc/kernels/loss.h
+++ b/icl_amd/csrc/kernels/loss.h
@@ -21,10 +21,46 @@
   lse = m + logf(s);
 }
 
-template <int NCMAX>
-__device__ __forceinline__ void loss_stats_body(const float* __restrict__ a, const float* __restrict__ b,
-                                                const long long* __restrict__ labels, float* __restrict__ part,
-                                                int B, int nc, long S, int a_is_prob, int bx, int nbx) {
+struct LossSrcPlain {
+  const float* __restrict__ a;
+  template <int NCMAX>
+  __device__ __forceinline__ void load(float* p, long bi, long s, int nc, long S) const {
+    const float* ap = a + bi * nc * S + s;
+#pragma unroll
+    for (int c = 0; c < NCMAX; ++c) p[c] = c < nc ? ap[(long)c * S] : 0.f;
+  }
+};
+struct LossSrcResized {
+  const float* __restrict__ src;
+  int Di, Hi, Wi, Do, Ho, Wo;
+  float rz, ry, rx;
+  int align;
+  template <int NCMAX>
+  __device__ __forceinline__ void sample(float* p, long bi, int nc, const LinTap& tz, const LinTap& ty, const LinTap& tx) const {
+    const long plane = (long)Di * Hi * Wi;
+    const float* q = src + bi * nc * plane;
+    const long o00 = ((long)tz.i0 * Hi + ty.i0) * Wi, o01 = ((long)tz.i0 * Hi + ty.i1) * Wi;
+    const long o10 = ((long)tz.i1 * Hi + ty.i0) * Wi, o11 = ((long)tz.i1 * Hi + ty.i1) * Wi;
+#pragma unroll
+    for (int c = 0; c < NCMAX; ++c) {
+      const float* qc = q + (long)c * plane;
+      p[c] = c < nc ? trilinear_sample(qc + o00, qc + o01, qc + o10, qc + o11, tz, ty, tx) : 0.f;
+    }
+  }
+  template <int NCMAX>
+  __device__ __forceinline__ void load(float* p, long bi, long s, int nc, long) const {
+    const unsigned v = (unsigned)s;
+    const int ox = (int)(v % (unsigned)Wo);
+    const unsigned t = v / (unsigned)Wo;
+    const int oy = (int)(t % (unsigned)Ho), oz = (int)(t / (unsigned)Ho);
+    sample<NCMAX>(p, bi, nc, lin_tap(oz, rz, Di, align), lin_tap(oy, ry, Hi, align), lin_tap(ox, rx, Wi, align));
+  }
+};
+
+template <int NCMAX, class Src>
+__device__ __forceinline__ void loss_stats_body_src(const Src& a, const float* __restrict__ b,
+                                                    const long long* __restrict__ labels, float* __restrict__ part,
+                                                    int B, int nc, long S, int a_is_prob, int bx, int nbx) {
   float s0[NCMAX], s1[NCMAX], s2[NCMAX];
   float sx = 0.f;
 #pragma unroll
@@ -32,10 +68,8 @@
   const long total = (long)B * S;
   for (long e = (long)bx * blockDim.x + threadIdx.x; e < total; e += (long)nbx * blockDim.x) {
     const long bi = e / S, s = e - bi * S;
-    const float* ap = a + bi * nc * S + s;
     float p[NCMAX];
-#pragma unroll
-    for (int c = 0; c < NCMAX; ++c) p[c] = c < nc ? ap[(long)c * S] : 0.f;
+    a.template load<NCMAX>(p, bi, s, nc, S);
     float lse = 0.f;
     if (labels) {
       const int y = (int)labels[e];
@@ -94,6 +128,12 @@
       part[(long)bx * (3 * nc + 1) + slot] = v;
     }
   }
+}
+template <int NCMAX>
+__device__ __forceinline__ void loss_stats_body(const float* __restrict__ a, const float* __restrict__ b,
+                                                const long long* __restrict__ labels, float* __restrict__ part,
+                                                int B, int nc, long S, int a_is_prob, int bx, int nbx) {
+  loss_stats_body_src<NCMAX>(LossSrcPlain{a}, b, labels, part, B, nc, S, a_is_prob, bx, nbx);
 }
 template <int NCMAX>
 __global__ __launch_bounds__(256) void loss_stats_kernel(const float* __restrict__ a, const float* __restrict__ b,
@@ -145,13 +185,8 @@
 }
 
 template <int NCMAX>
-__device__ __forceinline__ void loss_grad_body(const float* __restrict__ a, const float* __restrict__ b,
-                                               const long long* __restrict__ labels, const float* __restrict__ stats,
-                                               const float* __restrict__ weight, const float* __restrict__ gout0,
-                                               const float* __restrict__ gout1, float* __restrict__ ga, int B, int nc,
-                                               long S, int mode, float inv_vox, float inv_elems, int a_is_prob, int bx, int nbx) {
-  float al[NCMAX], be[NCMAX], gm[NCMAX];
-  const float g0 = gout0 ? gout0[0] : 0.f, g1 = gout1 ? gout1[0] : 0.f;
+__device__ __forceinline__ void loss_grad_coeffs(const float* __restrict__ stats, const float* __restrict__ weight, float g0, float g1,
+                                                 int nc, int mode, float inv_elems, float* al, float* be, float* gm) {
 #pragma unroll
   for (int c = 0; c < NCMAX; ++c) {
     al[c] = be[c] = gm[c] = 0.f;
@@ -164,42 +199,119 @@
       else { al[c] = -2.f * g0 * inv_elems; be[c] = 2.f * g0 * inv_elems; }
     }
   }
+}
+template <int NCMAX>
+__device__ __forceinline__ void loss_grad_voxel(float* p, float* T, int y, bool hard, const float* al, const float* be, const float* gm,
+                                                float kappa, int nc, int a_is_prob, float* gv) {
+  float lse;
+  if (!a_is_prob) softmax_vec<NCMAX>(p, nc, lse);
+  if (hard) {
+#pragma unroll
+    for (int c = 0; c < NCMAX; ++c) T[c] = (c == y) ? 1.f : 0.f;
+  } else {
+    softmax_vec<NCMAX>(T, nc, lse);
+  }
+  float d[NCMAX];
+  float dot = 0.f;
+#pragma unroll
+  for (int c = 0; c < NCMAX; ++c) {
+    d[c] = c < nc ? al[c] * T[c] + be[c] * p[c] + gm[c] : 0.f;
+    dot += d[c] * p[c];
+  }
+#pragma unroll
+  for (int c = 0; c < NCMAX; ++c) {
+    float g = a_is_prob ? d[c] : p[c] * (d[c] - dot);
+    if (hard) g += kappa * (p[c] - T[c]);
+    gv[c] = g;
+  }
+}
+template <int NCMAX, class Src>
+__device__ __forceinline__ void loss_grad_body_src(const Src& a, const float* __restrict__ b,
+                                                   const long long* __restrict__ labels, const float* __restrict__ stats,
+                                                   const float* __restrict__ weight, const float* __restrict__ gout0,
+                                                   const float* __restrict__ gout1, float* __restrict__ ga, int B, int nc,
+                                                   long S, int mode, float inv_vox, float inv_elems, int a_is_prob, int bx, int nbx) {
+  float al[NCMAX], be[NCMAX], gm[NCMAX];
+  const float g0 = gout0 ? gout0[0] : 0.f, g1 = gout1 ? gout1[0] : 0.f;
+  loss_grad_coeffs<NCMAX>(stats, weight, g0, g1, nc, mode, inv_elems, al, be, gm);
   const float kappa = (mode == 1) ? g0 * inv_vox : 0.f;
   const long total = (long)B * S;
   for (long e = (long)bx * blockDim.x + threadIdx.x; e < total; e += (long)nbx * blockDim.x) {
     const long bi = e / S, s = e - bi * S;
-    const float* ap = a + bi * nc * S + s;
     float* gp = ga + bi * nc * S + s;
-    float p[NCMAX], T[NCMAX];
-#pragma unroll
-    for (int c = 0; c < NCMAX; ++c) p[c] = c < nc ? ap[(long)c * S] : 0.f;
-    float lse;
-    if (!a_is_prob) softmax_vec<NCMAX>(p, nc, lse);
+    float p[NCMAX], T[NCMAX], gv[NCMAX];
+    a.template load<NCMAX>(p, bi, s, nc, S);
+    int y = 0;
     if (labels) {
-      const int y = (int)labels[e];
-#pragma unroll
-      for (int c = 0; c < NCMAX; ++c) T[c] = (c == y) ? 1.f : 0.f;
+      y = (int)labels[e];
     } else {
       const float* bp = b + bi * nc * S + s;
 #pragma unroll
       for (int c = 0; c < NCMAX; ++c) T[c] = c < nc ? bp[(long)c * S] : 0.f;
-      softmax_vec<NCMAX>(T, nc, lse);
-    }
-    float d[NCMAX];
-    float dot = 0.f;
-#pragma unroll
-    for (int c = 0; c < NCMAX; ++c) {
-      d[c] = c < nc ? al[c] * T[c] + be[c] * p[c] + gm[c] : 0.f;
-      dot += d[c] * p[c];
-    }
-#pragma unroll
-    for (int c = 0; c < NCMAX; ++c) {
-      if (c < nc) {
-        float gv = a_is_prob ? d[c] : p[c] * (d[c] - dot);
-        if (labels) gv += kappa * (p[c] - T[c]);
-        gp[(long)c * S] = gv;
-      }
-    }
+    }
+    loss_grad_voxel<NCMAX>(p, T, y, labels != nullptr, al, be, gm, kappa, nc, a_is_prob, gv);
+#pragma unroll
+    for (int c = 0; c < NCMAX; ++c)
+      if (c < nc) gp[(long)c * S] = gv[c];
+  }
+}
+template <int NCMAX>
+__device__ __forceinline__ void loss_grad_body(const float* __restrict__ a, const float* __restrict__ b,
+                                               const long long* __restrict__ labels, const float* __restrict__ stats,
+                                               const float* __restrict__ weight, const float* __restrict__ gout0,
+                                               const float* __restrict__ gout1, float* __restrict__ ga, int B, int nc,
+                                               long S, int mode, float inv_vox, float inv_elems, int a_is_prob, int bx, int nbx) {
+  loss_grad_body_src<NCMAX>(LossSrcPlain{a}, b, labels, stats, weight, gout0, gout1, ga, B, nc, S, mode, inv_vox, inv_elems, a_is_prob, bx, nbx);
+}
+
+template <int NCMAX>
+__device__ __forceinline__ void loss_grad_resized_x_body(const LossSrcResized& a, const float* __restrict__ b,
+                                                         const long long* __restrict__ labels, const float* __restrict__ stats,
+                                                         const float* __restrict__ weight, const float* __restrict__ gout0,
+                                                         const float* __restrict__ gout1, float* __restrict__ gx, int B, int nc,
+                                                         int mode, float inv_vox, float inv_elems, int a_is_prob, int bx, int nbx) {
+  float al[NCMAX], be[NCMAX], gm[NCMAX];
+  const float g0 = gout0 ? gout0[0] : 0.f, g1 = gout1 ? gout1[0] : 0.f;
+  loss_grad_coeffs<NCMAX>(stats, weight, g0, g1, nc, mode, inv_elems, al, be, gm);
+  const float kappa = (mode == 1) ? g0 * inv_vox : 0.f;
+  const long S = (long)a.Do * a.Ho * a.Wo;
+  const long rowsx = (long)a.Do * a.Ho;
+  const long total = (long)B * rowsx * a.Wi;
+  for (long e = (long)bx * blockDim.x + threadIdx.x; e < total; e += (long)nbx * blockDim.x) {
+    const int xi = (int)(e % a.Wi);
+    const long r = e / a.Wi;
+    const long bi = r / rowsx, row = r - bi * rowsx;
+    const int oz = (int)(row / a.Ho), oy = (int)(row - (long)oz * a.Ho);
+    const LinTap tz = lin_tap(oz, a.rz, a.Di, a.align), ty = lin_tap(oy, a.ry, a.Hi, a.align);
+    int lo, hi;
+    lin_range(xi, a.rx, a.Wo, a.align, lo, hi);
+    const long v0 = bi * S + row * a.Wo;
+    const float* bp = b ? b + bi * nc * S + row * a.Wo : nullptr;
+    float acc[NCMAX];
+#pragma unroll
+    for (int c = 0; c < NCMAX; ++c) acc[c] = 0.f;
+    for (int o = lo; o <= hi; ++o) {
+      const LinTap tx = lin_tap(o, a.rx, a.Wi, a.align);
+      const float w = (tx.i0 == xi ? tx.l0 : 0.f) + (tx.i1 == xi ? tx.l1 : 0.f);
+      if (w != 0.f) {
+        float p[NCMAX], T[NCMAX], gv[NCMAX];
+        a.template sample<NCMAX>(p, bi, nc, tz, ty, tx);
+        int y = 0;
+        if (labels) {
+          y = (int)labels[v0 + o];
+        } else {
+#pragma unroll
+          for (int c = 0; c < NCMAX; ++c) T[c] = c < nc ? bp[(long)c * S + o] : 0.f;
+        }
+        loss_grad_voxel<NCMAX>(p, T, y, labels != nullptr, al, be, gm, kappa, nc, a_is_prob, gv);
+#pragma unroll
+        for (int c = 0; c < NCMAX; ++c) acc[c] += w * gv[c];
+      }
+    }
+    float* gp = gx + (bi * nc * rowsx + row) * a.Wi + xi;
+#pragma unroll
+    for (int c = 0; c < NCMAX; ++c)
+      if (c < nc) gp[(long)c * rowsx * a.Wi] = acc[c];
   }
 }
 template <int NCMAX>
@@ -397,6 +509,45 @@
                         1.0f / total, 1.0f / (total * (float)m.nc[j]), m.aip[j], blockIdx.x, m.nblk[j]);
 }
 
+struct LossMultiR {
+  LossMulti m;
+  const float* src[kLossMulti];
+  float* gx[kLossMulti];
+  int Di[kLossMulti], Hi[kLossMulti], Wi[kLossMulti], Do[kLossMulti], Ho[kLossMulti], Wo[kLossMulti];
+  float rz[kLossMulti], ry[kLossMulti], rx[kLossMulti];
+  int align[kLossMulti], nblk_x[kLossMulti];
+};
+__device__ __forceinline__ LossSrcResized loss_multi_source(const LossMultiR& r, int j) {
+  return LossSrcResized{r.src[j], r.Di[j], r.Hi[j], r.Wi[j], r.Do[j], r.Ho[j], r.Wo[j], r.rz[j], r.ry[j], r.rx[j], r.align[j]};
+}
+template <int NCMAX>
+__global__ __launch_bounds__(256) void loss_stats_multi_resized_kernel(LossMultiR r) {
+  const LossMulti& m = r.m;
+  const int j = blockIdx.y;
+  if ((int)blockIdx.x >= m.nblk[j]) return;
+  float* part = m.stats[j] + (3 * m.nc[j] + 1);
+  if (r.src[j])
+    loss_stats_body_src<NCMAX>(loss_multi_source(r, j), m.b[j], m.lab[j], part, m.B[j], m.nc[j], m.S[j], m.aip[j], blockIdx.x, m.nblk[j]);
+  else
+    loss_stats_body<NCMAX>(m.a[j], m.b[j], m.lab[j], part, m.B[j], m.nc[j], m.S[j], m.aip[j], blockIdx.x, m.nblk[j]);
+}
+template <int NCMAX>
+__global__ __launch_bounds__(256) void loss_grad_multi_resized_kernel(LossMultiR r) {
+  const LossMulti& m = r.m;
+  const int j = blockIdx.y;
+  const float total = (float)((long)m.B[j] * m.S[j]);
+  const float inv_vox = 1.0f / total, inv_elems = 1.0f / (total * (float)m.nc[j]);
+  if (r.src[j]) {
+    if ((int)blockIdx.x >= r.nblk_x[j]) return;
+    loss_grad_resized_x_body<NCMAX>(loss_multi_source(r, j), m.b[j], m.lab[j], m.stats[j], m.weight[j], m.g0[j], m.g1[j], r.gx[j], m.B[j],
+                                    m.nc[j], m.mode[j], inv_vox, inv_elems, m.aip[j], blockIdx.x, r.nblk_x[j]);
+  } else {
+    if ((int)blockIdx.x >= m.nblk[j]) return;
+    loss_grad_body<NCMAX>(m.a[j], m.b[j], m.lab[j], m.stats[j], m.weight[j], m.g0[j], m.g1[j], m.ga[j], m.B[j], m.nc[j], m.S[j], m.mode[j],
+                          inv_vox, inv_elems, m.aip[j], blockIdx.x, m.nblk[j]);
+  }
+}
+
 __global__ __launch_bounds__(256) void loss_stats_generic_multi_kernel(LossMulti m) {
   const int j = blockIdx.y;
   if ((int)blockIdx.x >= m.nblk[j]) return;
diff --git a/icl_amd/csrc/kernels/pool_resize.h b/icl_amd/csrc/kernels/pool_resize.h
--- a/icl_amd/csrc/kernels/pool_resize.h
+++ b/icl_amd/csrc/kernels/pool_resize.h
@@ -157,6 +157,12 @@
   return t;
 }
 
+__device__ __forceinline__ float trilinear_sample(const float* p00, const float* p01, const float* p10, const float* p11,
+                                                  const LinTap& tz, const LinTap& ty, const LinTap& tx) {
+  return tz.l0 * (ty.l0 * (tx.l0 * p00[tx.i0] + tx.l1 * p00[tx.i1]) + ty.l1 * (tx.l0 * p01[tx.i0] + tx.l1 * p01[tx.i1])) +
+         tz.l1 * (ty.l0 * (tx.l0 * p10[tx.i0] + tx.l1 * p10[tx.i1]) + ty.l1 * (tx.l0 * p11[tx.i0] + tx.l1 * p11[tx.i1]));
+}
+
 __global__ __launch_bounds__(256) void trilinear_fwd_kernel(const float* __restrict__ x, float* __restrict__ y, int N, int C,
                                                             int Di, int Hi, int Wi, int Do, int Ho, int Wo,
                                                             float rz, float ry, float rx, long y_bstride, int align) {
@@ -175,11 +181,7 @@
     const float* p = x + ((long)n * C + c) * Di * Hi * Wi;
     const long z0 = (long)tz.i0 * Hi * Wi, z1 = (long)tz.i1 * Hi * Wi;
     const long y0 = (long)ty.i0 * Wi, y1 = (long)ty.i1 * Wi;
-    const float v =
-        tz.l0 * (ty.l0 * (tx.l0 * p[z0 + y0 + tx.i0] + tx.l1 * p[z0 + y0 + tx.i1]) +
-                 ty.l1 * (tx.l0 * p[z0 + y1 + tx.i0] + tx.l1 * p[z0 + y1 + tx.i1])) +
-        tz.l1 * (ty.l0 * (tx.l0 * p[z1 + y0 + tx.i0] + tx.l1 * p[z1 + y0 + tx.i1]) +
-                 ty.l1 * (tx.l0 * p[z1 + y1 + tx.i0] + tx.l1 * p[z1 + y1 + tx.i1]));
+    const float v = trilinear_sample(p + z0 + y0, p + z0 + y1, p + z1 + y0, p + z1 + y1, tz, ty, tx);
     y[(long)n * y_bstride + (((long)c * Do + oz) * Ho + oy) * Wo + ox] = v;
   }
 }
@@ -208,8 +210,7 @@
 #pragma unroll
     for (int k = 0; k < 4; ++k) {
       const LinTap tx = lin_tap((int)(xq * 4) + k, rx, Wi, align);
-      v[k] = tz.l0 * (ty.l0 * (tx.l0 * p00[tx.i0] + tx.l1 * p00[tx.i1]) + ty.l1 * (tx.l0 * p01[tx.i0] + tx.l1 * p01[tx.i1])) +
-             tz.l1 * (ty.l0 * (tx.l0 * p10[tx.i0] + tx.l1 * p10[tx.i1]) + ty.l1 * (tx.l0 * p11[tx.i0] + tx.l1 * p11[tx.i1]));
+      v[k] = trilinear_sample(p00, p01, p10, p11, tz, ty, tx);
     }
     *reinterpret_cast<float4*>(y + (long)n * y_bstride + (((long)c * Do + oz) * Ho + oy) * Wo + xq * 4) = make_float4(v[0], v[1], v[2], v[3]);
   }
diff --git a/icl_amd/ops.py b/icl_amd/ops.py
--- a/icl_amd/ops.py
+++ b/icl_amd/ops.py
@@ -2223,10 +2223,167 @@
         return tuple(res)
 
 
+class _LossJobR(ctypes.Structure):
+    _fields_ = [("job", _LossJob), ("src", _vp), ("gx", _vp), ("di", ctypes.c_int), ("hi", ctypes.c_int), ("wi", ctypes.c_int),
+                ("dout", ctypes.c_int), ("hout", ctypes.c_int), ("wout", ctypes.c_int), ("align_corners", ctypes.c_int)]
+
+
+LOSS_RESIZE_MAX_NC = 16
+
+
+LOSS_RESIZE_DEFAULT_NC = 4
+
+
+def loss_resize_fused(nc: int) -> bool:
+    if os.environ.get("ICL_LOSS_GENERIC", "0") == "1":
+        return False
+    sw = os.environ.get("ICL_LOSS_RESIZE_FUSED")
+    return sw != "0" and nc <= (LOSS_RESIZE_MAX_NC if sw is not None else LOSS_RESIZE_DEFAULT_NC)
+
+
+class ResizedMap:
+    __slots__ = ("fm", "size", "align_corners")
+
+    def __init__(self, fm: torch.Tensor, size: Sequence[int], align_corners: bool = False):
+        assert fm.dim() == 5 and len(size) == 3
+        self.fm, self.size, self.align_corners = fm, tuple(int(v) for v in size), bool(align_corners)
+
+    @property
+    def shape(self):
+        return tuple(self.fm.shape[:2]) + self.size
+
+    def materialize(self) -> torch.Tensor:
+        return trilinear_resize(self.fm.float(), self.size, self.align_corners)
+
+
+class _ResizeAdjointYZ(torch.autograd.Function):
+
+    @staticmethod
+    def forward(ctx, fm, size, align):
+        n, c, di, hi, wi = fm.shape
+        ctx.geom = (n, c, di, hi, wi, size[0], size[1], align)
+        ctx.set_materialize_grads(False)
+        return torch.empty((n, c, size[0], size[1], wi), dtype=torch.float32, device=fm.device)
+
+    @staticmethod
+    def backward(ctx, gx):
+        L = _lib.lib()
+        if gx is None:
+            return None, None, None
+        n, c, di, hi, wi, do, ho, align = ctx.geom
+        gx = gx.contiguous()
+        gsrc = torch.empty((n, c, di, hi, wi), dtype=torch.float32, device=gx.device)
+        ws = _ws(L.icl_loss_resized_bwd_ws_bytes(n, c, di, hi, wi, do, ho, 1), gx)
+        _lib.check(L.icl_loss_resized_bwd_yz(_ptr(gx), _ptr(ws), _ptr(gsrc), n, c, di, hi, wi, do, ho, align, _stream(gx)),
+                   "loss_resized_bwd_yz")
+        return gsrc, None, None
+
+
+class _FusedLossMultiR(torch.autograd.Function):
+
+    @staticmethod
+    def _fill(q, a, src, t, mode, size, nc):
+        j = q.job
+        if size is None:
+            B = a.shape[0]
+            S = a.numel() // (B * nc)
+            j.a, q.src = a.data_ptr(), None
+            assert a.shape[1] == nc and a.dtype == torch.float32
+        else:
+            B = src.shape[0]
+            S = size[0] * size[1] * size[2]
+            j.a, q.src = None, src.data_ptr()
+            q.di, q.hi, q.wi = src.shape[2:]
+            q.dout, q.hout, q.wout, q.align_corners = size
+            assert src.shape[1] == nc and src.dtype == torch.float32 and tuple(a.shape) == (B, nc, size[0], size[1], src.shape[4])
+        hard = mode <= 1
+        if hard:
+            assert t.dtype == torch.int64 and t.numel() == B * S, "labels must be int64 [B, ...]"
+        else:
+            assert t.dtype == torch.float32 and t.shape[:2] == (B, nc) and t.numel() == B * nc * S
+        j.b, j.labels, j.weight = (None if hard else t.data_ptr()), (t.data_ptr() if hard else None), None
+        j.s, j.batch, j.nc, j.mode, j.a_is_prob = S, B, nc, mode, 0
+
+    @staticmethod
+    def forward(ctx, modes, sizes, srcs, *tensors):
+        L = _lib.lib()
+        n = len(modes)
+        assert 1 <= n <= LOSS_MULTI_MAX and len(tensors) == 2 * n and len(sizes) == n and len(srcs) == n
+        a_s = [tensors[2 * j] if sizes[j] is not None else tensors[2 * j].contiguous() for j in range(n)]
+        t_s = [tensors[2 * j + 1].contiguous() for j in range(n)]
+        srcs = [None if s is None else s.contiguous() for s in srcs]
+        _require(*a_s, *t_s)
+        dev = a_s[0].device
+        nc = a_s[0].shape[1]
+        assert nc <= LOSS_RESIZE_MAX_NC
+        per = (3 * nc + 1) * (1 + LOSS_MAX_BLOCKS)
+        stats = torch.empty((n, per), dtype=torch.float32, device=dev)
+        out = torch.empty((n, 2), dtype=torch.float32, device=dev)
+        jobs = (_LossJobR * n)()
+        for j in range(n):
+            _FusedLossMultiR._fill(jobs[j], a_s[j], srcs[j], t_s[j], modes[j], sizes[j], nc)
+            jobs[j].job.stats, jobs[j].job.out = stats[j].data_ptr(), out[j].data_ptr()
+        _lib.check(L.icl_loss_fwd_multi_resized(jobs, n, _stream(a_s[0])), "loss_fwd_multi_resized")
+        ctx.save_for_backward(stats, *[a if s is None else s for a, s in zip(a_s, srcs)], *t_s)
+        ctx.modes, ctx.sizes = tuple(modes), tuple(sizes)
+        ctx.gx_shapes = [None if sizes[j] is None else tuple(a_s[j].shape) for j in range(n)]
+        ctx.set_materialize_grads(False)
+        return tuple(out[j, k] for j in range(n) for k in (0, 1))
+
+    @staticmethod
+    def backward(ctx, *gs):
+        L = _lib.lib()
+        modes, sizes = ctx.modes, ctx.sizes
+        n = len(modes)
+        stats = ctx.saved_tensors[0]
+        a_s, t_s = ctx.saved_tensors[1:1 + n], ctx.saved_tensors[1 + n:1 + 2 * n]
+        nc = a_s[0].shape[1]
+        gas = [None] * n
+        keep = []
+        live = [j for j in range(n) if ctx.needs_input_grad[3 + 2 * j] and (gs[2 * j] is not None or gs[2 * j + 1] is not None)]
+        jobs = (_LossJobR * max(len(live), 1))()
+        for i, j in enumerate(live):
+            resized = sizes[j] is not None
+            g0 = gs[2 * j].contiguous() if gs[2 * j] is not None else None
+            g1 = gs[2 * j + 1].contiguous() if gs[2 * j + 1] is not None else None
+            q = jobs[i]
+            if resized:
+                gas[j] = torch.empty(ctx.gx_shapes[j], dtype=torch.float32, device=stats.device)
+                _FusedLossMultiR._fill(q, gas[j], a_s[j], t_s[j], modes[j], sizes[j], nc)
+                q.gx, q.job.ga = gas[j].data_ptr(), None
+            else:
+                gas[j] = torch.empty_like(a_s[j])
+                _FusedLossMultiR._fill(q, a_s[j], None, t_s[j], modes[j], None, nc)
+                q.job.ga = gas[j].data_ptr()
+            q.job.stats, q.job.out = stats[j].data_ptr(), None
+            q.job.gout0, q.job.gout1 = _ptr(g0), _ptr(g1)
+            keep += [g0, g1]
+        if live:
+            _lib.check(L.icl_loss_bwd_multi_resized(jobs, len(live), _stream(stats)), "loss_bwd_multi_resized")
+        res = [None, None, None]
+        for j in range(n):
+            res += [gas[j], None]
+        return tuple(res)
+
+
 def fused_losses(terms):
     if not terms:
         return []
     ncs = {t[0].shape[1] for t in terms}
+    if any(isinstance(t[0], ResizedMap) for t in terms):
+        fused = (LOSS_MULTI and len(terms) <= LOSS_MULTI_MAX and len(ncs) == 1 and loss_resize_fused(max(ncs))
+                 and all((t[0].fm if isinstance(t[0], ResizedMap) else t[0]).dtype == torch.float32 for t in terms))
+        if fused:
+            flat, sizes, srcs = [], [], []
+            for a, t, m in terms:
+                r = isinstance(a, ResizedMap)
+                al = int(a.align_corners) if r else 0
+                flat += [_ResizeAdjointYZ.apply(a.fm, a.size, al) if r else a, (t.long() if m <= 1 else t.detach())]
+                sizes.append(a.size + (al,) if r else None)
+                srcs.append(a.fm.detach() if r else None)
+            out = _FusedLossMultiR.apply(tuple(m for _, _, m in terms), tuple(sizes), tuple(srcs), *flat)
+            return [(out[2 * j], out[2 * j + 1]) for j in range(len(terms))]
+        terms = [((a.materialize() if isinstance(a, ResizedMap) else a), t, m) for a, t, m in terms]
     if not LOSS_MULTI or len(terms) > LOSS_MULTI_MAX or len(ncs) != 1:
         return [_FusedLoss.apply(a, (t.long() if m <= 1 else t.detach()), None, m, False) for a, t, m in terms]
     flat = []
diff --git a/icl_amd/utils/losses.py b/icl_amd/utils/losses.py
--- a/icl_amd/utils/losses.py
+++ b/icl_amd/utils/losses.py
@@ -50,6 +50,12 @@
 
 def _resize(t, size):
     return ops.trilinear_resize(t.float(), size)
+
+
+def _resized_operand(feat_maps, size):
+    fused = (0 < len(feat_maps) <= ops.LOSS_MULTI_MAX and all(fm.dtype == torch.float32 and fm.dim() == 5 for fm in feat_maps)
+             and len({fm.shape[1] for fm in feat_maps}) == 1 and ops.loss_resize_fused(feat_maps[0].shape[1]))
+    return [ops.ResizedMap(fm, size) if fused else _resize(fm, size) for fm in feat_maps]
 
 
 def _resize2d(t, size):
@@ -106,7 +112,7 @@
         return out
 
     def terms(self, feat_maps, labels):
-        return [(_resize(fm, self.resize), labels, 1) for fm in feat_maps]
+        return [(a, labels, 1) for a in _resized_operand(feat_maps, self.resize)]
 
     def forward(self, feat_maps, labels):
         lv = self.leaves(feat_maps, labels)
@@ -125,7 +131,7 @@
 
     def terms(self, feat_maps, predicts):
         tgt = predicts.detach()
-        return [(_resize(fm, self.resize), tgt, 2) for fm in feat_maps]
+        return [(a, tgt, 2) for a in _resized_operand(feat_maps, self.resize)]
 
     def forward(self, feat_maps, predicts):
         return _mean_of(self.leaves(feat_maps, predicts))
diff --git a/include/icl_hip.h b/include/icl_hip.h
--- a/include/icl_hip.h
+++ b/include/icl_hip.h
@@ -144,6 +144,16 @@
 } IclLossJob;
 int icl_loss_fwd_multi(const IclLossJob* jobs, int count, void* stream);
 int icl_loss_bwd_multi(const IclLossJob* jobs, int count, void* stream);
+typedef struct IclLossJobR {
+  IclLossJob job;
+  const float* src; float* gx;
+  int di, hi, wi, dout, hout, wout, align_corners;
+} IclLossJobR;
+int64_t icl_loss_resized_bwd_ws_bytes(int batch, int nc, int di, int hi, int wi, int dout, int hout, int wout);
+int icl_loss_fwd_multi_resized(const IclLossJobR* jobs, int count, void* stream);
+int icl_loss_bwd_multi_resized(const IclLossJobR* jobs, int count, void* stream);
+int icl_loss_resized_bwd_yz(const float* gx, void* ws, float* gsrc, int batch, int nc, int di, int hi, int wi, int dout, int hout,
+                            int align_corners, void* stream);
 
 int icl_layernorm_fwd(const float* x, const float* gamma, const float* beta, float* y, float* mean, float* rstd, int64_t rows,
                       int c, float eps, void* stream);
```
